# google-research/rigl

Hardware: AMD Instinct MI355X
Metric: images/sec/node, ResNet-50 80% ERK RigL step (higher is better)
Workload: dtype bf16

## Files before the change

include/rigl_hip.h:

```cpp
#ifndef RIGL_HIP_H_
#define RIGL_HIP_H_

#include <stddef.h>
#include <stdint.h>

#ifdef __cplusplus
extern "C" {
#endif

#define RIGL_ABI_VERSION 2

typedef void* rigl_stream_t;
typedef uint16_t rigl_bf16;

enum {
  RIGL_OK = 0,
  RIGL_EINVAL = -1,
  RIGL_ELAUNCH = -2,
  RIGL_EWORKSPACE = -3,
  RIGL_EUNSUPPORTED = -4
};

int rigl_version(void);
uint32_t rigl_crc32c(const void* data, size_t n, uint32_t crc);
// ... 41 lines not shown
                                         int32_t n_layers);
int rigl_prune_regrow(const RiglPruneRegrowLayer* layers ,
                      int32_t n_layers, const RiglPruneRegrowParams* params,
                      int32_t* out_counts ,
                      void* workspace , size_t workspace_bytes,
                      rigl_stream_t stream);

size_t rigl_prune_regrow_selections_workspace_bytes(int64_t n);
int rigl_prune_regrow_selections(const RiglPruneRegrowLayer* layer ,
                                 const RiglPruneRegrowParams* params,
                                 uint32_t* out_mask1_bits, uint32_t* out_mask2_bits,
                                 int32_t* out_idx1, int32_t* out_idx2,
                                 int32_t* out_counts ,
                                 void* workspace, size_t workspace_bytes,
                                 rigl_stream_t stream);

int rigl_prune_regrow_slots(const RiglPruneRegrowLayer* layers ,
                            float* const* momentum2 ,
                            int32_t n_layers, const RiglPruneRegrowParams* params,
                            int32_t* out_counts ,
                            void* workspace , size_t workspace_bytes,
                            rigl_stream_t stream);
int rigl_prune_regrow_selections_slots(const RiglPruneRegrowLayer* layer ,
                                       float* momentum2 ,
                                       const RiglPruneRegrowParams* params,
                                       uint32_t* out_mask1_bits, uint32_t* out_mask2_bits,
                                       int32_t* out_idx1, int32_t* out_idx2,
                                       int32_t* out_counts ,
                                       void* workspace, size_t workspace_bytes,
                                       rigl_stream_t stream);

int rigl_topk_mask(const float* score, int64_t n, int64_t n_keep,
                   uint32_t* mask_bits, void* workspace,
                   size_t workspace_bytes, rigl_stream_t stream);
typedef struct RiglTopkLayer {
  const float* score;
  int64_t n;
  int64_t n_keep;
  uint32_t* mask_bits;
} RiglTopkLayer;
int rigl_topk_mask_batched(const RiglTopkLayer* layers ,
                           int32_t n_layers, void* workspace,
                           size_t workspace_bytes, rigl_stream_t stream);

typedef struct RiglMagnitudePruneLayer {
  int64_t n;
  const float* w;
  uint32_t* mask_bits;
  float* threshold;
  int64_t k;
} RiglMagnitudePruneLayer;
size_t rigl_magnitude_prune_batched_workspace_bytes(int32_t n_layers);
#define RIGL_MAGPRUNE_COUNTS_PER_LAYER 4
int rigl_magnitude_prune_batched(const RiglMagnitudePruneLayer* layers ,
                                 int32_t n_layers, double threshold_decay,
                                 int32_t* out_counts, void* workspace,
                                 size_t workspace_bytes, rigl_stream_t stream);

int rigl_masked_sgd_momentum(int64_t n, float* w, float* momentum,
                             const float* dense_grad, const uint32_t* mask_bits,
                             float lr, float mu, float weight_decay,
                             float grad_scale, int32_t nesterov,
                             rigl_bf16* w_shadow, rigl_stream_t stream);

int rigl_masked_adam(int64_t n, float* w, float* m, float* v,
                     const float* dense_grad, const uint32_t* mask_bits,
                     const float* beta_powers , float lr,
                     float beta1, float beta2, float epsilon,
                     float weight_decay, float grad_scale,
                     rigl_bf16* w_shadow, rigl_stream_t stream);
int rigl_adam_advance(float* beta_powers , float beta1,
                      float beta2, rigl_stream_t stream);

#define RIGL_LR_MAX_SEGMENTS 32
#define RIGL_LR_DOMAIN_STEP 0
#define RIGL_LR_DOMAIN_EPOCH 1
#define RIGL_LR_CONST 0
#define RIGL_LR_WARMUP 1
#define RIGL_LR_COSINE 2
typedef struct RiglLrSegment {
  int32_t kind;
  int32_t start_step;
  float start;
  float c, d;
  float sum_r, len, m_fac;
} RiglLrSegment;
typedef struct RiglLrSchedule {
  int32_t n_seg;
  int32_t domain;
  float steps_per_epoch;
  int32_t reserved;
  RiglLrSegment seg[RIGL_LR_MAX_SEGMENTS];
} RiglLrSchedule;
int rigl_lr_schedule_step(const RiglLrSchedule* sched ,
                          int32_t* step ,
                          float* lr_out , rigl_stream_t stream);

int rigl_masked_sgd_momentum_dlr(int64_t n, float* w, float* momentum,
                                 const float* dense_grad,
                                 const uint32_t* mask_bits,
                                 const float* lr , float mu,
                                 float weight_decay, float grad_scale,
                                 int32_t nesterov, rigl_bf16* w_shadow,
                                 rigl_stream_t stream);
int rigl_masked_adam_dlr(int64_t n, float* w, float* m, float* v,
                         const float* dense_grad, const uint32_t* mask_bits,
                         const float* beta_powers ,
                         const float* lr , float beta1,
                         float beta2, float epsilon, float weight_decay,
                         float grad_scale, rigl_bf16* w_shadow,
                         rigl_stream_t stream);

int rigl_pack_weights(const float* w, const uint32_t* mask_bits ,
                      int32_t k, int32_t cout, rigl_bf16* hwio, rigl_bf16* ohwi,
                      rigl_stream_t stream);
typedef struct RiglPackLayer {
  const float* w;
  const uint32_t* mask_bits;
  rigl_bf16* hwio;
  rigl_bf16* ohwi;
  int32_t k, cout;
} RiglPackLayer;
int rigl_pack_weights_batched(const RiglPackLayer* layers, int32_t n_layers,
                              rigl_stream_t stream);

typedef struct RiglConvDesc {
  int32_t n, h, w, cin;
  int32_t ho, wo, cout;
  int32_t kh, kw;
  int32_t stride_h, stride_w;
  int32_t pad_top, pad_left;
} RiglConvDesc;

size_t rigl_conv2d_workspace_bytes(const RiglConvDesc* d, int32_t which );
int rigl_masked_conv2d_fwd(const RiglConvDesc* d, const rigl_bf16* x,
                           const rigl_bf16* w_ohwi, rigl_bf16* y,
                           void* workspace, size_t workspace_bytes,
                           rigl_stream_t stream);
int rigl_masked_conv2d_dgrad(const RiglConvDesc* d, const rigl_bf16* dy,
                             const rigl_bf16* w_hwio, rigl_bf16* dx,
                             void* workspace, size_t workspace_bytes,
                             rigl_stream_t stream);
int32_t rigl_conv2d_stats_parts(const RiglConvDesc* d);
int rigl_masked_conv2d_fwd_stats(const RiglConvDesc* d, const rigl_bf16* x,
                                 const rigl_bf16* w_ohwi, rigl_bf16* y,
                                 float* stats, size_t stats_floats,
                                 void* workspace, size_t workspace_bytes,
                                 rigl_stream_t stream);
int32_t rigl_conv2d_fwd_takes_bn_input(const RiglConvDesc* d);
int rigl_masked_conv2d_fwd_bnrelu(const RiglConvDesc* d, const rigl_bf16* x_pre,
                                  const float* scale_shift, rigl_bf16* a_out,
                                  const rigl_bf16* w_ohwi, rigl_bf16* y,
                                  float* stats , size_t stats_floats,
                                  void* workspace, size_t workspace_bytes,
                                  rigl_stream_t stream);
int rigl_masked_conv2d_dgrad_acc(const RiglConvDesc* d, const rigl_bf16* dy,
                                 const rigl_bf16* w_hwio, const rigl_bf16* addend,
                                 rigl_bf16* dx, void* workspace,
                                 size_t workspace_bytes, rigl_stream_t stream);
int rigl_masked_conv2d_wgrad(const RiglConvDesc* d, const rigl_bf16* x,
                             const rigl_bf16* dy, float* dw, void* workspace,
                             size_t workspace_bytes, rigl_stream_t stream);

int rigl_masked_conv2d_bwd(const RiglConvDesc* d, const rigl_bf16* x,
                           const rigl_bf16* dy, const rigl_bf16* w_hwio,
                           const rigl_bf16* addend , float* dw,
                           rigl_bf16* dx , void* workspace,
                           size_t workspace_bytes, rigl_stream_t stream);

int rigl_masked_conv2d_bwd_grid(const RiglConvDesc* d, const rigl_bf16* x,
                                const rigl_bf16* dy, const rigl_bf16* w_hwio,
                                float* dw, rigl_bf16* dx_grid, void* workspace,
                                size_t workspace_bytes, rigl_stream_t stream);
int rigl_masked_conv2d_bwd_sub(const RiglConvDesc* d, const rigl_bf16* x,
                               const rigl_bf16* dy, const rigl_bf16* w_hwio,
                               const rigl_bf16* addend, int32_t sub_h, int32_t sub_w,
                               float* dw, rigl_bf16* dx, void* workspace,
                               size_t workspace_bytes, rigl_stream_t stream);
int32_t rigl_conv2d_bwd_takes_masked_addend(const RiglConvDesc* d);
int rigl_masked_conv2d_bwd_masked(const RiglConvDesc* d, const rigl_bf16* x,
                                  const rigl_bf16* dy, const rigl_bf16* w_hwio,
                                  const rigl_bf16* addend, const uint8_t* addend_bits,
                                  float* dw, rigl_bf16* dx, void* workspace,
                                  size_t workspace_bytes, rigl_stream_t stream);

int32_t rigl_conv2d_bwd_takes_bn_apply(const RiglConvDesc* d);
int rigl_masked_conv2d_bwd_bnapply(const RiglConvDesc* d, const rigl_bf16* x,
                                   const rigl_bf16* dout, const rigl_bf16* w_hwio,
                                   const rigl_bf16* addend , float* dw,
                                   rigl_bf16* dx, void* workspace, size_t workspace_bytes,
                                   const rigl_bf16* y, const uint8_t* relu_bits,
                                   const float* mean, const float* invstd,
                                   const float* coef, rigl_stream_t stream);

typedef struct RiglBnReduceFuse {
  const rigl_bf16* x;
  const uint8_t* relu_bits;
  const float* params;
  int32_t relu;
  float* partial;
  size_t partial_floats;
} RiglBnReduceFuse;
int32_t rigl_conv2d_dgrad_stats_parts(const RiglConvDesc* d);
int rigl_masked_conv2d_bwd_bn(const RiglConvDesc* d, const rigl_bf16* x,
                              const rigl_bf16* dy, const rigl_bf16* w_hwio,
                              const rigl_bf16* addend, float* dw, rigl_bf16* dx,
                              void* workspace, size_t workspace_bytes,
                              const RiglBnReduceFuse* bn ,
                              rigl_stream_t stream);

size_t rigl_depthwise_conv2d_workspace_bytes(const RiglConvDesc* d);
int rigl_depthwise_conv2d_fwd(const RiglConvDesc* d, const rigl_bf16* x,
                              const float* w, rigl_bf16* y, rigl_stream_t stream);
int32_t rigl_depthwise_conv2d_stats_parts(const RiglConvDesc* d);
int rigl_depthwise_conv2d_fwd_stats(const RiglConvDesc* d, const rigl_bf16* x,
                                    const float* w, rigl_bf16* y, float* stats,
                                    size_t stats_floats, rigl_stream_t stream);
int rigl_depthwise_conv2d_dgrad(const RiglConvDesc* d, const rigl_bf16* dy,
                                const float* w, rigl_bf16* dx,
                                rigl_stream_t stream);
int rigl_depthwise_conv2d_wgrad(const RiglConvDesc* d, const rigl_bf16* x,
                                const rigl_bf16* dy, float* dw, void* workspace,
                                size_t workspace_bytes, rigl_stream_t stream);

int rigl_conv2d_fwd_ref(const RiglConvDesc* d, const rigl_bf16* x,
                        const rigl_bf16* w_ohwi, rigl_bf16* y,
                        rigl_stream_t stream);
int rigl_conv2d_dgrad_ref(const RiglConvDesc* d, const rigl_bf16* dy,
                          const rigl_bf16* w_hwio, rigl_bf16* dx,
                          rigl_stream_t stream);
int rigl_conv2d_wgrad_ref(const RiglConvDesc* d, const rigl_bf16* x,
                          const rigl_bf16* dy, float* dw, rigl_stream_t stream);

int rigl_masked_conv2d_fwd_f32(const RiglConvDesc* d, const float* x,
                               const float* w_hwio, const uint32_t* mask_bits ,
                               float* y, rigl_stream_t stream);
int rigl_masked_conv2d_dgrad_f32(const RiglConvDesc* d, const float* dy,
                                 const float* w_hwio, const uint32_t* mask_bits ,
                                 const float* addend ,
                                 float* dx, rigl_stream_t stream);
size_t rigl_conv2d_wgrad_f32_workspace_bytes(const RiglConvDesc* d);
int rigl_masked_conv2d_wgrad_f32(const RiglConvDesc* d, const float* x,
                                 const float* dy, float* dw, void* workspace,
                                 size_t workspace_bytes, rigl_stream_t stream);

size_t rigl_bn_workspace_bytes(int64_t m, int32_t c);
int rigl_bn_fwd(int64_t m, int32_t c, const rigl_bf16* x,
                const rigl_bf16* residual , const float* gamma,
                const float* beta, float* running_mean, float* running_var,
                float momentum, float eps, int32_t relu, rigl_bf16* y,
                float* save_mean, float* save_invstd, float* save_scale,
                float* save_shift, void* workspace, size_t workspace_bytes,
                rigl_stream_t stream);
int rigl_bn_fwd_stats(int64_t m, int32_t c, const rigl_bf16* x,
                      const rigl_bf16* residual ,
                      const float* gamma, const float* beta,
                      float* running_mean, float* running_var, float momentum,
                      float eps, int32_t relu, rigl_bf16* y, float* save_mean,
                      float* save_invstd, float* save_scale, float* save_shift,
                      const float* stats, int32_t stats_parts,
                      uint8_t* relu_bits ,
                      void* workspace, size_t workspace_bytes, rigl_stream_t stream);
int rigl_bn_bwd(int64_t m, int32_t c, const rigl_bf16* x,
                const rigl_bf16* y ,
                const uint8_t* relu_bits , const rigl_bf16* dy,
                const float* gamma, const float* save_mean,
                const float* save_invstd, const float* save_scale,
                const float* save_shift, int32_t relu, rigl_bf16* dx,
                rigl_bf16* dresidual , float* dgamma,
                float* dbeta, void* workspace, size_t workspace_bytes,
                rigl_stream_t stream);
int rigl_bn_bwd_reduce(int64_t m, int32_t c, const rigl_bf16* x,
                       const uint8_t* relu_bits ,
                       const rigl_bf16* dy, const float* gamma, const float* save_mean,
                       const float* save_invstd, int32_t relu, float* dgamma,
                       float* dbeta, float* coef, void* workspace,
                       size_t workspace_bytes, rigl_stream_t stream);
int rigl_bn_bwd_stats(int64_t m, int32_t c, const rigl_bf16* x,
                      const rigl_bf16* y ,
                      const uint8_t* relu_bits , const rigl_bf16* dy,
                      const float* gamma, const float* save_mean,
                      const float* save_invstd, const float* save_scale,
                      const float* save_shift, int32_t relu, rigl_bf16* dx,
                      rigl_bf16* dresidual , float* dgamma,
                      float* dbeta, const float* stats, int32_t stats_parts,
                      void* workspace, size_t workspace_bytes, rigl_stream_t stream);

int rigl_bn_add_bn_fwd(int64_t m, int32_t c, const rigl_bf16* x, const rigl_bf16* x2,
                       const float* scale2, const float* shift2,
                       const float* gamma, const float* beta, float* running_mean,
                       float* running_var, float momentum, float eps, int32_t relu,
                       rigl_bf16* y, float* save_mean, float* save_invstd,
                       float* save_scale, float* save_shift, const float* stats,
                       int32_t stats_parts, uint8_t* relu_bits ,
                       void* workspace, size_t workspace_bytes, rigl_stream_t stream);
size_t rigl_bn_add_bn_bwd_workspace_bytes(int64_t m, int32_t c);
int rigl_bn_add_bn_bwd(int64_t m, int32_t c, const rigl_bf16* x, const rigl_bf16* x2,
                       const uint8_t* relu_bits, const rigl_bf16* dy,
                       const float* gamma, const float* save_mean, const float* save_invstd,
                       const float* gamma2, const float* save_mean2, const float* save_invstd2,
                       rigl_bf16* dx, rigl_bf16* dx2, float* dgamma, float* dbeta,
                       float* dgamma2, float* dbeta2, void* workspace,
                       size_t workspace_bytes, rigl_stream_t stream);

int rigl_stateless_random(float* out, int64_t n, int32_t seed0, int32_t seed1,
                          int32_t dist, float scale, float shift,
                          rigl_stream_t stream);
typedef struct {
  float* out;
  int64_t n;
  int32_t seed0, seed1;
  int32_t dist;
  float scale, shift;
} RiglRandomItem;
int rigl_stateless_random_batched(const RiglRandomItem* items, int32_t n_items,
                                  rigl_stream_t stream);

int rigl_dropout_fwd(const void* x, void* y, uint8_t* keep_bits, int64_t n,
                     int32_t dtype, float rate, int32_t seed0,
                     const int32_t* step , rigl_stream_t stream);
int rigl_dropout_bwd(const void* dy, const uint8_t* keep_bits, void* dx,
                     int64_t n, int32_t dtype, float rate, rigl_stream_t stream);
int rigl_dropout_advance(int32_t* step , rigl_stream_t stream);

int rigl_cifar_batch(const uint8_t* images, const int32_t* labels,
                     int64_t n_images, int32_t batch, int32_t mode,
                     int32_t shard, int32_t n_shards, int32_t seed0,
                     const int32_t* step , void* out, int32_t dtype,
                     int32_t* out_labels, int32_t* out_index ,
                     rigl_stream_t stream);
int rigl_cifar_advance(int32_t* step , rigl_stream_t stream);

int rigl_maxpool_fwd(const RiglConvDesc* d, const rigl_bf16* x, rigl_bf16* y,
                     uint8_t* argmax, rigl_stream_t stream);
int rigl_maxpool_bwd(const RiglConvDesc* d, const rigl_bf16* dy,
                     const uint8_t* argmax, rigl_bf16* dx, rigl_stream_t stream);
int rigl_bn_fwd_statistics(int64_t m, int32_t c, const rigl_bf16* x ,
                           const float* gamma, const float* beta,
                           float* running_mean, float* running_var, float momentum,
                           float eps, float* save_mean, float* save_invstd,
                           float* save_scale, float* save_shift,
                           const float* stats, int32_t stats_parts,
                           void* workspace, size_t workspace_bytes, rigl_stream_t stream);
int rigl_bn_relu_maxpool_fwd(const RiglConvDesc* d, const rigl_bf16* x,
                             const float* scale, const float* shift, rigl_bf16* y,
                             uint8_t* argmax, rigl_stream_t stream);
size_t rigl_bn_relu_maxpool_bwd_workspace_bytes(const RiglConvDesc* d);
int rigl_bn_relu_maxpool_bwd(const RiglConvDesc* d, const rigl_bf16* x,
                             const rigl_bf16* dy, const uint8_t* argmax,
                             const float* gamma, const float* save_mean,
                             const float* save_invstd, const float* save_scale,
                             const float* save_shift, rigl_bf16* dx, float* dgamma,
                             float* dbeta, void* workspace, size_t workspace_bytes,
                             rigl_stream_t stream);

int rigl_global_avgpool_fwd(int32_t n, int32_t pixels, int32_t c, const rigl_bf16* x,
                            rigl_bf16* y, rigl_stream_t stream);
int rigl_global_avgpool_bwd(int32_t n, int32_t pixels, int32_t c, const rigl_bf16* dy,
                            rigl_bf16* dx, rigl_stream_t stream);
int rigl_global_avgpool_bwd_relu(int32_t n, int32_t pixels, int32_t c, const rigl_bf16* dy,
                                 const rigl_bf16* x, rigl_bf16* dx, rigl_stream_t stream);
int rigl_softmax_xent(int32_t rows, int32_t classes, const rigl_bf16* logits,
                      const int64_t* labels, float label_smoothing, float grad_scale,
                      float* row_loss, rigl_bf16* dlogits , rigl_stream_t stream);

int32_t rigl_conv2d_fwd_takes_relu_epilogue(const RiglConvDesc* d);
int32_t rigl_conv2d_bwd_takes_relu_epilogue(const RiglConvDesc* d);
int rigl_masked_conv2d_fwd_relu(const RiglConvDesc* d, const rigl_bf16* x,
                                const rigl_bf16* w_ohwi, rigl_bf16* y, void* workspace,
                                size_t workspace_bytes, rigl_stream_t stream);
int rigl_masked_conv2d_bwd_relu(const RiglConvDesc* d, const rigl_bf16* x,
                                const rigl_bf16* dy, const rigl_bf16* w_hwio, float* dw,
                                rigl_bf16* dx, void* workspace, size_t workspace_bytes,
                                rigl_stream_t stream);
int rigl_relu_fwd(int64_t n, const rigl_bf16* x, rigl_bf16* y, rigl_stream_t stream);
int rigl_relu_bwd(int64_t n, const rigl_bf16* dy, const rigl_bf16* x, rigl_bf16* dx,
                  rigl_stream_t stream);

typedef struct RiglBnInferItem {
  const float* gamma;
  const float* beta;
  const float* moving_mean;
  const float* moving_variance;
  float* scale_shift;
  int32_t c;
  float eps;
} RiglBnInferItem;
int rigl_bn_infer_params_batched(const RiglBnInferItem* items, int32_t n_items,
                                 rigl_stream_t stream);
int rigl_bn_apply(int64_t m, int32_t c, const rigl_bf16* x,
                  const rigl_bf16* residual , const float* scale_shift,
                  int32_t relu, rigl_bf16* y, rigl_stream_t stream);
int rigl_bn_apply_pair(int64_t m, int32_t c, const rigl_bf16* x, const rigl_bf16* x2,
                       const float* scale_shift, const float* scale_shift2,
                       int32_t relu, rigl_bf16* y, rigl_stream_t stream);
int rigl_bn_relu_maxpool_infer(const RiglConvDesc* d, const rigl_bf16* x,
                               const float* scale_shift, rigl_bf16* y,
                               rigl_stream_t stream);
int32_t rigl_conv2d_fwd_takes_bn_epilogue(const RiglConvDesc* d, int32_t bn_on_load,
                                          int32_t residual);
int rigl_masked_conv2d_fwd_bn_infer(const RiglConvDesc* d, const rigl_bf16* x,
                                    const float* in_scale_shift ,
                                    const rigl_bf16* w_ohwi,
                                    const float* scale_shift ,
                                    const rigl_bf16* residual ,
                                    int32_t relu, rigl_bf16* y, rigl_stream_t stream);
int rigl_eval_metrics(int32_t rows, int32_t classes, const rigl_bf16* logits,
                      const int64_t* labels, float label_smoothing, int32_t topk,
                      float* row_loss, int32_t* row_flags,
                      int64_t* counts , rigl_stream_t stream);

#define RIGL_PROF_KINDS 8
int rigl_prof_enable(int32_t on);
int rigl_prof_collect(double* ms_per_kind , int64_t* launches );
#define RIGL_PROF_KINDS_ALL 10
int rigl_prof_collect_kinds(double* ms_per_kind, int64_t* launches, int32_t n_kinds);
typedef struct RiglProfLaunch {
  int32_t kind;
  int32_t tag[6];
  float ms;
} RiglProfLaunch;
int rigl_prof_collect_launches(RiglProfLaunch* out , int64_t cap, int64_t* n_launches);

int rigl_probe_mfma_bf16(int32_t blocks, int32_t iters, float* sink, rigl_stream_t stream);

int rigl_tune_set(const char* key, int32_t value);
int32_t rigl_tune_get(const char* key, int32_t dflt);
int rigl_tune_unset(const char* key);
uint64_t rigl_tune_generation(void);
const volatile uint64_t* rigl_tune_generation_addr(void);

#ifdef __cplusplus
}
#endif
#endif
```

rigl_amd/_lib.py:

```python
import ctypes as C
import os

_HERE = os.path.dirname(os.path.abspath(__file__))
ABI_VERSION = 2
LIB_PATH = os.environ.get('RIGL_HIP_LIB') or os.path.join(_HERE, 'lib', 'librigl_hip.so')

RIGL_OK = 0
RIGL_EINVAL = -1
RIGL_ELAUNCH = -2
RIGL_EWORKSPACE = -3
RIGL_EUNSUPPORTED = -4
COUNTS_PER_LAYER = 8
MAGPRUNE_COUNTS_PER_LAYER = 4
PROF_KINDS = ('conv_fwd', 'conv_dgrad', 'conv_wgrad', 'prune_regrow',
              'sgd_momentum', 'pack_weights', 'conv_bwd', 'depthwise', 'masked_adam', 'magnitude_prune')

GROW_ZEROS, GROW_GRAD_SCALE, GROW_GRAD_SIGN, GROW_EXPLICIT = 0, 1, 2, 3
MOMRESET_ZEROS, MOMRESET_GRAD = 0, 1


class RiglError(RuntimeError):

  def __init__(self, code, msg):
    super().__init__('librigl_hip: error %d: %s' % (code, msg))
    self.code = code


class PruneRegrowLayer(C.Structure):
  _fields_ = [('n', C.c_int64), ('w', C.c_void_p), ('momentum', C.c_void_p),
              ('mask_bits', C.c_void_p), ('dense_grad', C.c_void_p),
              ('drop_noise', C.c_void_p), ('score_drop', C.c_void_p),
              ('score_grow', C.c_void_p), ('grow_values', C.c_void_p)]


class PruneRegrowParams(C.Structure):
  _fields_ = [('drop_fraction', C.c_float), ('grow_init_mode', C.c_int32),
              ('grow_init_div', C.c_float), ('momentum_reset_mode', C.c_int32),
              ('initial_acc_scale', C.c_float), ('reinit_when_same', C.c_int32)]


class TopkLayer(C.Structure):
  _fields_ = [('score', C.c_void_p), ('n', C.c_int64), ('n_keep', C.c_int64),
              ('mask_bits', C.c_void_p)]


class MagnitudePruneLayer(C.Structure):
  _fields_ = [('n', C.c_int64), ('w', C.c_void_p), ('mask_bits', C.c_void_p), ('threshold', C.c_void_p),
              ('k', C.c_int64)]


class PackLayer(C.Structure):
  _fields_ = [('w', C.c_void_p), ('mask_bits', C.c_void_p),
              ('hwio', C.c_void_p), ('ohwi', C.c_void_p), ('k', C.c_int32),
              ('cout', C.c_int32)]


class ConvDesc(C.Structure):
  _fields_ = [('n', C.c_int32), ('h', C.c_int32), ('w', C.c_int32),
              ('cin', C.c_int32), ('ho', C.c_int32), ('wo', C.c_int32),
              ('cout', C.c_int32), ('kh', C.c_int32), ('kw', C.c_int32),
              ('stride_h', C.c_int32), ('stride_w', C.c_int32),
              ('pad_top', C.c_int32), ('pad_left', C.c_int32)]


class BnReduceFuse(C.Structure):
  _fields_ = [('x', C.c_void_p), ('relu_bits', C.c_void_p), ('params', C.c_void_p), ('relu', C.c_int32),
              ('partial', C.c_void_p), ('partial_floats', C.c_size_t)]


class RandomItem(C.Structure):
  _fields_ = [('out', C.c_void_p), ('n', C.c_int64), ('seed0', C.c_int32), ('seed1', C.c_int32),
              ('dist', C.c_int32), ('scale', C.c_float), ('shift', C.c_float)]


class BnInferItem(C.Structure):
  _fields_ = [('gamma', C.c_void_p), ('beta', C.c_void_p), ('moving_mean', C.c_void_p), ('moving_variance', C.c_void_p),
              ('scale_shift', C.c_void_p), ('c', C.c_int32), ('eps', C.c_float)]


LR_MAX_SEGMENTS = 32
LR_DOMAIN_STEP, LR_DOMAIN_EPOCH = 0, 1
LR_CONST, LR_WARMUP, LR_COSINE = 0, 1, 2


class LrSegment(C.Structure):
  _fields_ = [('kind', C.c_int32), ('start_step', C.c_int32), ('start', C.c_float), ('c', C.c_float), ('d', C.c_float),
              ('sum_r', C.c_float), ('len', C.c_float), ('m_fac', C.c_float)]


class LrSchedule(C.Structure):
  _fields_ = [('n_seg', C.c_int32), ('domain', C.c_int32), ('steps_per_epoch', C.c_float), ('reserved', C.c_int32),
              ('seg', LrSegment * LR_MAX_SEGMENTS)]


class ProfLaunch(C.Structure):
  _fields_ = [('kind', C.c_int32), ('tag', C.c_int32 * 6), ('ms', C.c_float)]


_P, _I32, _I64, _F, _SZ = C.c_void_p, C.c_int32, C.c_int64, C.c_float, C.c_size_t
SIGNATURES = {
    'rigl_version': (C.c_int, []),
    'rigl_last_error': (C.c_char_p, []),
    'rigl_mask_pack': (C.c_int, [_P, _P, _I64, _P]),
    'rigl_mask_unpack': (C.c_int, [_P, _P, _I64, _P]),
    'rigl_prune_regrow_workspace_bytes': (_SZ, [C.POINTER(_I64), _I32]),
    'rigl_prune_regrow': (C.c_int, [C.POINTER(PruneRegrowLayer), _I32,
                                    C.POINTER(PruneRegrowParams), _P, _P, _SZ,
                                    _P]),
    'rigl_prune_regrow_slots': (C.c_int, [C.POINTER(PruneRegrowLayer), C.POINTER(_P), _I32,
                                          C.POINTER(PruneRegrowParams), _P, _P, _SZ, _P]),
    'rigl_prune_regrow_selections_workspace_bytes': (_SZ, [_I64]),
    'rigl_prune_regrow_selections': (C.c_int, [C.POINTER(PruneRegrowLayer), C.POINTER(PruneRegrowParams), _P, _P, _P, _P, _P,
                                               _P, _SZ, _P]),
    'rigl_prune_regrow_selections_slots': (C.c_int, [C.POINTER(PruneRegrowLayer), _P, C.POINTER(PruneRegrowParams), _P, _P,
                                                     _P, _P, _P, _P, _SZ, _P]),
    'rigl_topk_mask': (C.c_int, [_P, _I64, _I64, _P, _P, _SZ, _P]),
    'rigl_topk_mask_batched': (C.c_int, [C.POINTER(TopkLayer), _I32, _P, _SZ, _P]),
    'rigl_magnitude_prune_batched_workspace_bytes': (_SZ, [_I32]),
    'rigl_magnitude_prune_batched': (C.c_int, [C.POINTER(MagnitudePruneLayer), _I32, C.c_double, _P, _P, _SZ, _P]),
    'rigl_masked_sgd_momentum': (C.c_int, [_I64, _P, _P, _P, _P, _F, _F, _F, _F,
                                           _I32, _P, _P]),
    'rigl_masked_adam': (C.c_int, [_I64, _P, _P, _P, _P, _P, _P, _F, _F, _F, _F, _F, _F, _P, _P]),
    'rigl_adam_advance': (C.c_int, [_P, _F, _F, _P]),
    'rigl_lr_schedule_step': (C.c_int, [C.POINTER(LrSchedule), _P, _P, _P]),
    'rigl_masked_sgd_momentum_dlr': (C.c_int, [_I64, _P, _P, _P, _P, _P, _F, _F, _F, _I32, _P, _P]),
    'rigl_masked_adam_dlr': (C.c_int, [_I64, _P, _P, _P, _P, _P, _P, _P, _F, _F, _F, _F, _F, _P, _P]),
    'rigl_pack_weights': (C.c_int, [_P, _P, _I32, _I32, _P, _P, _P]),
    'rigl_pack_weights_batched': (C.c_int, [C.POINTER(PackLayer), _I32, _P]),
    'rigl_conv2d_workspace_bytes': (_SZ, [C.POINTER(ConvDesc), _I32]),
    'rigl_masked_conv2d_fwd': (C.c_int, [C.POINTER(ConvDesc), _P, _P, _P, _P,
                                         _SZ, _P]),
    'rigl_masked_conv2d_dgrad': (C.c_int, [C.POINTER(ConvDesc), _P, _P, _P, _P,
                                           _SZ, _P]),
    'rigl_conv2d_stats_parts': (_I32, [C.POINTER(ConvDesc)]),
    'rigl_masked_conv2d_fwd_stats': (C.c_int, [C.POINTER(ConvDesc), _P, _P, _P, _P,
                                               _SZ, _P, _SZ, _P]),
    'rigl_conv2d_fwd_takes_bn_input': (_I32, [C.POINTER(ConvDesc)]),
    'rigl_masked_conv2d_fwd_bnrelu': (C.c_int, [C.POINTER(ConvDesc), _P, _P, _P, _P, _P, _P, _SZ, _P, _SZ, _P]),
    'rigl_masked_conv2d_dgrad_acc': (C.c_int, [C.POINTER(ConvDesc), _P, _P, _P,
                                               _P, _P, _SZ, _P]),
    'rigl_conv2d_dgrad_stats_parts': (_I32, [C.POINTER(ConvDesc)]),
    'rigl_masked_conv2d_bwd_bn': (C.c_int, [C.POINTER(ConvDesc), _P, _P, _P, _P, _P, _P, _P, _SZ,
                                            C.POINTER(BnReduceFuse), _P]),
    'rigl_masked_conv2d_bwd': (C.c_int, [C.POINTER(ConvDesc), _P, _P, _P, _P, _P, _P, _P, _SZ, _P]),
    'rigl_masked_conv2d_bwd_masked': (C.c_int, [C.POINTER(ConvDesc), _P, _P, _P, _P, _P, _P, _P, _P, _SZ, _P]),
    'rigl_conv2d_bwd_takes_masked_addend': (_I32, [C.POINTER(ConvDesc)]),
    'rigl_conv2d_bwd_takes_bn_apply': (_I32, [C.POINTER(ConvDesc)]),
    'rigl_masked_conv2d_bwd_bnapply': (C.c_int, [C.POINTER(ConvDesc), _P, _P, _P, _P, _P, _P, _P, _SZ, _P, _P, _P, _P, _P, _P]),
    'rigl_masked_conv2d_bwd_grid': (C.c_int, [C.POINTER(ConvDesc), _P, _P, _P, _P, _P, _P, _SZ, _P]),
    'rigl_masked_conv2d_bwd_sub': (C.c_int, [C.POINTER(ConvDesc), _P, _P, _P, _P, _I32, _I32, _P, _P, _P, _SZ, _P]),
    'rigl_masked_conv2d_wgrad': (C.c_int, [C.POINTER(ConvDesc), _P, _P, _P, _P,
                                           _SZ, _P]),
    'rigl_conv2d_fwd_ref': (C.c_int, [C.POINTER(ConvDesc), _P, _P, _P, _P]),
    'rigl_conv2d_dgrad_ref': (C.c_int, [C.POINTER(ConvDesc), _P, _P, _P, _P]),
    'rigl_conv2d_wgrad_ref': (C.c_int, [C.POINTER(ConvDesc), _P, _P, _P, _P]),
    'rigl_masked_conv2d_fwd_f32': (C.c_int, [C.POINTER(ConvDesc), _P, _P, _P, _P, _P]),
    'rigl_masked_conv2d_dgrad_f32': (C.c_int, [C.POINTER(ConvDesc), _P, _P, _P, _P, _P, _P]),
    'rigl_conv2d_wgrad_f32_workspace_bytes': (_SZ, [C.POINTER(ConvDesc)]),
    'rigl_masked_conv2d_wgrad_f32': (C.c_int, [C.POINTER(ConvDesc), _P, _P, _P, _P, _SZ, _P]),
    'rigl_depthwise_conv2d_workspace_bytes': (_SZ, [C.POINTER(ConvDesc)]),
    'rigl_depthwise_conv2d_fwd': (C.c_int, [C.POINTER(ConvDesc), _P, _P, _P, _P]),
    'rigl_depthwise_conv2d_stats_parts': (_I32, [C.POINTER(ConvDesc)]),
    'rigl_depthwise_conv2d_fwd_stats': (C.c_int, [C.POINTER(ConvDesc), _P, _P, _P, _P, _SZ, _P]),
    'rigl_depthwise_conv2d_dgrad': (C.c_int, [C.POINTER(ConvDesc), _P, _P, _P, _P]),
    'rigl_depthwise_conv2d_wgrad': (C.c_int, [C.POINTER(ConvDesc), _P, _P, _P, _P, _SZ, _P]),
    'rigl_bn_workspace_bytes': (_SZ, [_I64, _I32]),
    'rigl_bn_fwd': (C.c_int, [_I64, _I32, _P, _P, _P, _P, _P, _P, _F, _F, _I32, _P, _P, _P, _P, _P, _P, _SZ, _P]),
    'rigl_bn_fwd_stats': (C.c_int, [_I64, _I32, _P, _P, _P, _P, _P, _P, _F, _F, _I32, _P, _P, _P, _P, _P, _P, _I32, _P, _P, _SZ, _P]),
    'rigl_bn_bwd': (C.c_int, [_I64, _I32, _P, _P, _P, _P, _P, _P, _P, _P, _P, _I32, _P, _P, _P, _P, _P, _SZ, _P]),
    'rigl_bn_bwd_stats': (C.c_int, [_I64, _I32, _P, _P, _P, _P, _P, _P, _P, _P, _P, _I32, _P, _P, _P, _P, _P, _I32, _P, _SZ, _P]),
    'rigl_bn_bwd_reduce': (C.c_int, [_I64, _I32, _P, _P, _P, _P, _P, _P, _I32, _P, _P, _P, _P, _SZ, _P]),
    'rigl_crc32c': (C.c_uint32, [_P, _SZ, C.c_uint32]),
    'rigl_stateless_random': (C.c_int, [_P, _I64, _I32, _I32, _I32, _F, _F, _P]),
    'rigl_stateless_random_batched': (C.c_int, [C.POINTER(RandomItem), _I32, _P]),
    'rigl_dropout_fwd': (C.c_int, [_P, _P, _P, _I64, _I32, _F, _I32, _P, _P]),
    'rigl_dropout_bwd': (C.c_int, [_P, _P, _P, _I64, _I32, _F, _P]),
    'rigl_dropout_advance': (C.c_int, [_P, _P]),
    'rigl_cifar_batch': (C.c_int, [_P, _P, _I64, _I32, _I32, _I32, _I32, _I32, _P, _P, _I32, _P, _P, _P]),
    'rigl_cifar_advance': (C.c_int, [_P, _P]),
    'rigl_maxpool_fwd': (C.c_int, [C.POINTER(ConvDesc), _P, _P, _P, _P]),
    'rigl_maxpool_bwd': (C.c_int, [C.POINTER(ConvDesc), _P, _P, _P, _P]),
    'rigl_bn_fwd_statistics': (C.c_int, [_I64, _I32, _P, _P, _P, _P, _P, _F, _F, _P, _P, _P, _P, _P, _I32, _P, _SZ, _P]),
    'rigl_bn_add_bn_fwd': (C.c_int, [_I64, _I32, _P, _P, _P, _P, _P, _P, _P, _P, _F, _F, _I32, _P, _P, _P, _P, _P, _P, _I32, _P, _P, _SZ, _P]),
    'rigl_bn_add_bn_bwd_workspace_bytes': (_SZ, [_I64, _I32]),
    'rigl_bn_add_bn_bwd': (C.c_int, [_I64, _I32, _P, _P, _P, _P, _P, _P, _P, _P, _P, _P, _P, _P, _P, _P, _P, _P, _P, _SZ, _P]),
    'rigl_bn_relu_maxpool_fwd': (C.c_int, [C.POINTER(ConvDesc), _P, _P, _P, _P, _P, _P]),
    'rigl_bn_relu_maxpool_bwd_workspace_bytes': (_SZ, [C.POINTER(ConvDesc)]),
    'rigl_bn_relu_maxpool_bwd': (C.c_int, [C.POINTER(ConvDesc), _P, _P, _P, _P, _P, _P, _P, _P, _P, _P, _P, _P, _SZ, _P]),
    'rigl_global_avgpool_fwd': (C.c_int, [_I32, _I32, _I32, _P, _P, _P]),
    'rigl_global_avgpool_bwd': (C.c_int, [_I32, _I32, _I32, _P, _P, _P]),
    'rigl_softmax_xent': (C.c_int, [_I32, _I32, _P, _P, _F, _F, _P, _P, _P]),
    'rigl_global_avgpool_bwd_relu': (C.c_int, [_I32, _I32, _I32, _P, _P, _P, _P]),
    'rigl_conv2d_fwd_takes_relu_epilogue': (C.c_int32, [C.POINTER(ConvDesc)]),
    'rigl_conv2d_bwd_takes_relu_epilogue': (C.c_int32, [C.POINTER(ConvDesc)]),
    'rigl_masked_conv2d_fwd_relu': (C.c_int, [C.POINTER(ConvDesc), _P, _P, _P, _P, _SZ, _P]),
    'rigl_masked_conv2d_bwd_relu': (C.c_int, [C.POINTER(ConvDesc), _P, _P, _P, _P, _P, _P, _SZ, _P]),
    'rigl_relu_fwd': (C.c_int, [_I64, _P, _P, _P]),
    'rigl_relu_bwd': (C.c_int, [_I64, _P, _P, _P, _P]),
    'rigl_bn_infer_params_batched': (C.c_int, [C.POINTER(BnInferItem), _I32, _P]),
    'rigl_bn_apply': (C.c_int, [_I64, _I32, _P, _P, _P, _I32, _P, _P]),
    'rigl_bn_apply_pair': (C.c_int, [_I64, _I32, _P, _P, _P, _P, _I32, _P, _P]),
    'rigl_bn_relu_maxpool_infer': (C.c_int, [C.POINTER(ConvDesc), _P, _P, _P, _P]),
    'rigl_conv2d_fwd_takes_bn_epilogue': (C.c_int32, [C.POINTER(ConvDesc), _I32, _I32]),
    'rigl_masked_conv2d_fwd_bn_infer': (C.c_int, [C.POINTER(ConvDesc), _P, _P, _P, _P, _P, _I32, _P, _P]),
    'rigl_eval_metrics': (C.c_int, [_I32, _I32, _P, _P, _F, _I32, _P, _P, _P, _P]),
    'rigl_prof_enable': (C.c_int, [_I32]),
    'rigl_prof_collect': (C.c_int, [C.POINTER(C.c_double), C.POINTER(_I64)]),
    'rigl_prof_collect_kinds': (C.c_int, [C.POINTER(C.c_double), C.POINTER(_I64), _I32]),
    'rigl_prof_collect_launches': (C.c_int, [C.POINTER(ProfLaunch), _I64, C.POINTER(_I64)]),
    'rigl_probe_mfma_bf16': (C.c_int, [_I32, _I32, _P, _P]),
    'rigl_tune_set': (C.c_int, [C.c_char_p, _I32]),
    'rigl_tune_get': (_I32, [C.c_char_p, _I32]),
    'rigl_tune_generation': (C.c_uint64, []),
    'rigl_tune_generation_addr': (C.c_void_p, []),
    'rigl_tune_unset': (C.c_int, [C.c_char_p]),
}

_lib = None


def load():
  global _lib
  if _lib is not None:
    return _lib
  if not os.path.exists(LIB_PATH):
    raise RiglError(
        RIGL_ELAUNCH, 'HIP extension not built: %s is missing; run '
        '`python -c "import __graft_entry__ as g; g.build()"` or '
        '`make -C rigl_amd/csrc`' % LIB_PATH)
  try:
    import torch
  except ImportError:
    pass
  lib = C.CDLL(LIB_PATH, mode=C.RTLD_GLOBAL)
  for name, (res, args) in SIGNATURES.items():
    fn = getattr(lib, name)
    fn.restype = res
    fn.argtypes = args
  if lib.rigl_version() != ABI_VERSION:
    raise RiglError(RIGL_EINVAL, 'ABI version mismatch')
  _lib = lib
  return lib


def check(rc):
  if rc != RIGL_OK:
    raise RiglError(rc, load().rigl_last_error().decode('utf-8', 'replace'))
```

rigl_amd/csrc/bn.hip:

```cpp
#include "common.hpp"

namespace rigl {
namespace kbn {

constexpr int THREADS = 256;
constexpr int MAX_PARTS = 512;

__device__ __forceinline__ float bf_lo(uint32_t w) { return __uint_as_float(w << 16); }
__device__ __forceinline__ float bf_hi(uint32_t w) { return __uint_as_float(w & 0xFFFF0000u); }
__device__ __forceinline__ uint32_t f2bf(float f) {
  uint32_t u = __float_as_uint(f);
  if ((u & 0x7FFFFFFFu) > 0x7F800000u) return (u >> 16) | 0x40u;
  u += 0x7FFFu + ((u >> 16) & 1u);
  return u >> 16;
}
typedef __attribute__((ext_vector_type(2))) __bf16 bf16x2_t;
typedef __attribute__((ext_vector_type(2))) float f32x2_t;
__device__ __forceinline__ uint32_t pack2(float a, float b) {
  const f32x2_t v = {a, b};
  return __builtin_bit_cast(uint32_t, __builtin_convertvector(v, bf16x2_t));
}
__device__ __forceinline__ void unpack8(const uint4& v, float f[8]) {
  f[0] = bf_lo(v.x); f[1] = bf_hi(v.x); f[2] = bf_lo(v.y); f[3] = bf_hi(v.y);
  f[4] = bf_lo(v.z); f[5] = bf_hi(v.z); f[6] = bf_lo(v.w); f[7] = bf_hi(v.w);
// ... 393 lines not shown
      float xv[8], x2v[8], dv[8];
      unpack8(*reinterpret_cast<const uint4*>(x + off), xv);
      unpack8(*reinterpret_cast<const uint4*>(x2 + off), x2v);
      unpack8(*reinterpret_cast<const uint4*>(dy + off), dv);
      const uint32_t mb = mbits[r * G.cg + cgi];
#pragma unroll
      for (int j = 0; j < 8; ++j) {
        const float dz = ((mb >> j) & 1u) != 0u ? dv[j] : 0.f;
        q0[j] += dz;
        q1[j] = fmaf(dz, (xv[j] - mu[j]) * is[j], q1[j]);
        q2[j] = fmaf(dz, (x2v[j] - mu2[j]) * is2[j], q2[j]);
      }
    }
  }
  float own[24];
#pragma unroll
  for (int j = 0; j < 8; ++j) {
    own[j] = q0[j]; own[8 + j] = q1[j]; own[16 + j] = q2[j];
    red[threadIdx.x][j] = q0[j]; red[threadIdx.x][8 + j] = q1[j]; red[threadIdx.x][16 + j] = q2[j];
  }
  __syncthreads();
  for (int s = G.rpb >> 1; s > 0; s >>= 1) {
    if (ty < s) {
      float oth[24];
#pragma unroll
      for (int j = 0; j < 24; ++j) oth[j] = red[threadIdx.x + s * G.tpr][j];
#pragma unroll
      for (int j = 0; j < 24; ++j) own[j] += oth[j];
      if (s > 1) {
#pragma unroll
        for (int j = 0; j < 24; ++j) red[threadIdx.x][j] = own[j];
      }
    }
    if (s > 1) __syncthreads();
  }
  if (ty == 0 && c_ok) {
    float* p = partial + ((int64_t)blockIdx.x * 2) * G.C + cgi * 8;
    float* p2 = partial2 + ((int64_t)blockIdx.x * 2) * G.C + cgi * 8;
#pragma unroll
    for (int j = 0; j < 8; ++j) {
      p[j] = own[j]; p[G.C + j] = own[8 + j];
      p2[j] = own[j]; p2[G.C + j] = own[16 + j];
    }
  }
}

struct FinSet { const float* partial; const float* gamma; const float* invstd; float* dgamma; float* dbeta; float* coef; };

template <int CL>
__global__ __launch_bounds__(THREADS) void k_bwd_finalize_pair(Geom G, FinSet s0, FinSet s1) {
  const FinSet& f = blockIdx.y == 0 ? s0 : s1;
  double a0, a1; int c; bool leader;
  sum_partials<CL>(G, f.partial, a0, a1, c, leader);
  if (!leader) return;
  f.dbeta[c] = (float)a0;
  f.dgamma[c] = (float)a1;
  f.coef[c] = f.gamma[c] * f.invstd[c];
  f.coef[G.C + c] = (float)(a0 / (double)G.M);
  f.coef[2 * G.C + c] = (float)(a1 / (double)G.M);
}

__global__ __launch_bounds__(THREADS) void k_bwd_apply_pair(Geom G, const uint16_t* __restrict__ x, const uint16_t* __restrict__ x2,
                                                             const uint8_t* __restrict__ mbits, const uint16_t* __restrict__ dy,
                                                             const float* __restrict__ mean, const float* __restrict__ invstd,
                                                             const float* __restrict__ mean2, const float* __restrict__ invstd2,
                                                             const float* __restrict__ coef, const float* __restrict__ coef2,
                                                             uint16_t* __restrict__ dx, uint16_t* __restrict__ dx2) {
  extern __shared__ __attribute__((aligned(16))) float prm[];
  const bool fixed = G.fixed != 0;
  float q[10][8];
  if (fixed) {
    const int c0 = (int)(((int64_t)blockIdx.x * THREADS + threadIdx.x) % G.cg) * 8;
    ld8f(mean + c0, q[0]); ld8f(invstd + c0, q[1]); ld8f(coef + c0, q[2]); ld8f(coef + G.C + c0, q[3]); ld8f(coef + 2 * G.C + c0, q[4]);
    ld8f(mean2 + c0, q[5]); ld8f(invstd2 + c0, q[6]); ld8f(coef2 + c0, q[7]); ld8f(coef2 + G.C + c0, q[8]); ld8f(coef2 + 2 * G.C + c0, q[9]);
  } else {
    for (int i = threadIdx.x; i < G.C; i += THREADS) {
      prm[i] = mean[i]; prm[G.C + i] = invstd[i];
      prm[2 * G.C + i] = coef[i]; prm[3 * G.C + i] = coef[G.C + i]; prm[4 * G.C + i] = coef[2 * G.C + i];
      prm[5 * G.C + i] = mean2[i]; prm[6 * G.C + i] = invstd2[i];
      prm[7 * G.C + i] = coef2[i]; prm[8 * G.C + i] = coef2[G.C + i]; prm[9 * G.C + i] = coef2[2 * G.C + i];
    }
    __syncthreads();
  }
  const int64_t total = G.M * G.cg;
  const int64_t stride = (int64_t)gridDim.x * THREADS;
  for (int64_t i = (int64_t)blockIdx.x * THREADS + threadIdx.x; i < total; i += stride) {
    if (!fixed) {
      const int c0 = (int)(i % G.cg) * 8;
#pragma unroll
      for (int k = 0; k < 10; ++k)
#pragma unroll
        for (int j = 0; j < 8; ++j) q[k][j] = prm[k * G.C + c0 + j];
    }
    float xv[8], x2v[8], dv[8];
    unpack8(ld16(x + i * 8, G.nt), xv);
    unpack8(ld16(x2 + i * 8, G.nt), x2v);
    unpack8(ld16(dy + i * 8, G.nt), dv);
    const uint32_t mb = mbits[i];
    float o[8], o2[8];
#pragma unroll
    for (int j = 0; j < 8; ++j) {
      const float dz = ((mb >> j) & 1u) != 0u ? dv[j] : 0.f;
      const float xh = (xv[j] - q[0][j]) * q[1][j];
      o[j] = q[2][j] * (dz - q[3][j] - xh * q[4][j]);
      const float xh2 = (x2v[j] - q[5][j]) * q[6][j];
      o2[j] = q[7][j] * (dz - q[8][j] - xh2 * q[9][j]);
    }
    uint4 out;
    out.x = pack2(o[0], o[1]); out.y = pack2(o[2], o[3]); out.z = pack2(o[4], o[5]); out.w = pack2(o[6], o[7]);
    st16(dx + i * 8, out, G.nt);
    out.x = pack2(o2[0], o2[1]); out.y = pack2(o2[2], o2[3]); out.z = pack2(o2[4], o2[5]); out.w = pack2(o2[6], o2[7]);
    st16(dx2 + i * 8, out, G.nt);
  }
}

constexpr int INFER_BATCH = 64;
struct InferBatch {
  RiglBnInferItem it[INFER_BATCH];
  int32_t blk_begin[INFER_BATCH + 1];
  int32_t count;
};
__global__ __launch_bounds__(THREADS) void k_infer_params(InferBatch B) {
  int i = 0;
  while (i + 1 < B.count && (int)blockIdx.x >= B.blk_begin[i + 1]) ++i;
  const RiglBnInferItem& t = B.it[i];
  const int c = ((int)blockIdx.x - B.blk_begin[i]) * THREADS + (int)threadIdx.x;
  if (c >= t.c) return;
  const float invstd = (float)(1.0 / sqrt((double)t.moving_variance[c] + (double)t.eps));
  const float sc = t.gamma[c] * invstd;
  t.scale_shift[c] = sc;
  t.scale_shift[t.c + c] = t.beta[c] - t.moving_mean[c] * sc;
}

static Geom make_geom(int64_t m, int c) {
  Geom g;
  g.nt = (int64_t)m * c * 2 >= (int64_t)RIGL_TUNE("bn_nt_mb", 0) * (1 << 20) ? RIGL_TUNE("bn_nt", 2) : 0;
  g.il = RIGL_TUNE("bn_il", 1);
  g.fixed = 0;
  g.M = m; g.C = c; g.cg = c / 8;
  int tpr = 1;
  while (tpr < g.cg && tpr < THREADS) tpr <<= 1;
  g.tpr = tpr; g.rpb = THREADS / tpr;
#ifndef RIGL_BN_ROWS_PER_LANE
#define RIGL_BN_ROWS_PER_LANE 8
#endif
  int64_t parts = (m + (int64_t)g.rpb * RIGL_BN_ROWS_PER_LANE - 1) / ((int64_t)g.rpb * RIGL_BN_ROWS_PER_LANE);
  const int64_t cap = RIGL_TUNE("bn_max_parts", MAX_PARTS);
  if (parts > cap) parts = cap;
  if (parts < 1) parts = 1;
  int64_t rpp = (m + parts - 1) / parts;
  rpp = (rpp + g.rpb - 1) / g.rpb * g.rpb;
  g.rows_per_part = rpp;
  g.parts = (int)((m + rpp - 1) / rpp);
  return g;
}

static unsigned apply_grid(Geom& g) {
#ifndef RIGL_BN_APPLY_PER_THREAD
#define RIGL_BN_APPLY_PER_THREAD 2
#endif
#ifndef RIGL_BN_APPLY_CAP
#define RIGL_BN_APPLY_CAP 16384
#endif
  int64_t b = (g.M * g.cg + THREADS * RIGL_BN_APPLY_PER_THREAD - 1) / (THREADS * RIGL_BN_APPLY_PER_THREAD);
  if (b > RIGL_BN_APPLY_CAP) b = RIGL_BN_APPLY_CAP;
  if (b < 1) b = 1;
  g.fixed = (RIGL_TUNE("bn_regs", 1) != 0 && (b * THREADS) % g.cg == 0) ? 1 : 0;
  return (unsigned)b;
}

void launch_bwd_finalize(int64_t m, int c, const float* partial, int parts, const float* gamma, const float* invstd,
                         float* dgamma, float* dbeta, float* coef, hipStream_t st) {
  Geom g = make_geom(m, c);
  g.parts = parts;
  if (parts > MAX_PARTS)
    hipLaunchKernelGGL(k_bwd_finalize<4>, dim3((unsigned)((c + 3) / 4)), dim3(THREADS), 0, st, g, partial, gamma, invstd,
                       dgamma, dbeta, coef);
  else
    hipLaunchKernelGGL(k_bwd_finalize<16>, dim3((unsigned)((c + 15) / 16)), dim3(THREADS), 0, st, g, partial, gamma, invstd,
                       dgamma, dbeta, coef);
}

static int fwd_statistics(Geom& g, int32_t c, const rigl_bf16* x, const float* gamma, const float* beta,
                          float* running_mean, float* running_var, float momentum, float eps, float* save_mean,
                          float* save_invstd, float* save_scale, float* save_shift, const float* stats,
                          int32_t stats_parts, void* workspace, size_t workspace_bytes, hipStream_t st) {
  const float* partial = stats;
  if (!stats) {
    const size_t need = rigl_bn_workspace_bytes(g.M, c);
    if (!workspace || workspace_bytes < need) return fail(RIGL_EWORKSPACE, "rigl_bn_fwd: workspace %zu < %zu", workspace_bytes, need);
    float* ws_partial = static_cast<float*>(workspace);
    dim3 rgrid((unsigned)g.parts, (unsigned)((g.cg + g.tpr - 1) / g.tpr));
    hipLaunchKernelGGL((k_reduce<0, false, 0>), rgrid, dim3(THREADS), 0, st, g, x, nullptr, nullptr, nullptr, nullptr, nullptr,
                       nullptr, nullptr, ws_partial);
    partial = ws_partial;
  } else {
    g.parts = stats_parts;
  }
  if (g.parts > 1024 && RIGL_TUNE("bn_fin1", 1) != 0)
    hipLaunchKernelGGL(k_fwd_finalize<1>, dim3((unsigned)c), dim3(THREADS), 0, st, g, partial, stats ? nullptr : reinterpret_cast<const uint16_t*>(x), gamma,
                       beta, running_mean, running_var, momentum, eps, save_mean, save_invstd, save_scale, save_shift);
  else if (g.parts > 256)
    hipLaunchKernelGGL(k_fwd_finalize<4>, dim3((unsigned)((c + 3) / 4)), dim3(THREADS), 0, st, g, partial, stats ? nullptr : reinterpret_cast<const uint16_t*>(x), gamma,
                       beta, running_mean, running_var, momentum, eps, save_mean, save_invstd, save_scale, save_shift);
  else
    hipLaunchKernelGGL(k_fwd_finalize<16>, dim3((unsigned)((c + 15) / 16)), dim3(THREADS), 0, st, g, partial, stats ? nullptr : reinterpret_cast<const uint16_t*>(x), gamma,
                       beta, running_mean, running_var, momentum, eps, save_mean, save_invstd, save_scale, save_shift);
  return RIGL_OK;
}

}
}

extern "C" {

size_t rigl_bn_workspace_bytes(int64_t m, int32_t c) {
  if (m <= 0 || c <= 0) return 0;
  rigl::kbn::Geom g = rigl::kbn::make_geom(m, c);
  return rigl::align_up((size_t)g.parts * 2 * c * 4, 256) + rigl::align_up((size_t)3 * c * 4, 256);
}

int rigl_bn_fwd_stats(int64_t m, int32_t c, const rigl_bf16* x, const rigl_bf16* residual, const float* gamma,
                      const float* beta, float* running_mean, float* running_var, float momentum, float eps,
                      int32_t relu, rigl_bf16* y, float* save_mean, float* save_invstd, float* save_scale,
                      float* save_shift, const float* stats, int32_t stats_parts, uint8_t* relu_bits,
                      void* workspace, size_t workspace_bytes, rigl_stream_t stream) {
  using namespace rigl;
  using namespace rigl::kbn;
  if (m <= 0 || c <= 0 || !x || !gamma || !beta || !y || !save_mean || !save_invstd || !save_scale || !save_shift)
    return fail(RIGL_EINVAL, "rigl_bn_fwd: bad arguments");
  if (c % 8) return fail(RIGL_EUNSUPPORTED, "rigl_bn_fwd: channels %% 8 != 0");
  if (2 * (size_t)c * 4 > 65536) return fail(RIGL_EUNSUPPORTED, "rigl_bn_fwd: too many channels for the LDS parameter cache");
  if (stats && stats_parts <= 0) return fail(RIGL_EINVAL, "rigl_bn_fwd_stats: stats_parts must be positive");
  hipStream_t st = as_stream(stream);
  Geom g = make_geom(m, c);
  int rc = fwd_statistics(g, c, x, gamma, beta, running_mean, running_var, momentum, eps, save_mean, save_invstd,
                          save_scale, save_shift, stats, stats_parts, workspace, workspace_bytes, st);
  if (rc) return rc;
  dim3 agrid(apply_grid(g));
  const size_t lds = g.fixed ? 0 : (size_t)2 * c * 4;
  if (relu && residual) hipLaunchKernelGGL((k_fwd_apply<true, true>), agrid, dim3(THREADS), lds, st, g, x, residual, save_scale, save_shift, y, relu_bits);
  else if (relu) hipLaunchKernelGGL((k_fwd_apply<true, false>), agrid, dim3(THREADS), lds, st, g, x, residual, save_scale, save_shift, y, relu_bits);
  else if (residual) hipLaunchKernelGGL((k_fwd_apply<false, true>), agrid, dim3(THREADS), lds, st, g, x, residual, save_scale, save_shift, y, nullptr);
  else hipLaunchKernelGGL((k_fwd_apply<false, false>), agrid, dim3(THREADS), lds, st, g, x, residual, save_scale, save_shift, y, nullptr);
  RIGL_CHECK_LAUNCH("rigl_bn_fwd");
  return RIGL_OK;
}

int rigl_bn_fwd(int64_t m, int32_t c, const rigl_bf16* x, const rigl_bf16* residual, const float* gamma,
                const float* beta, float* running_mean, float* running_var, float momentum, float eps, int32_t relu,
                rigl_bf16* y, float* save_mean, float* save_invstd, float* save_scale, float* save_shift,
                void* workspace, size_t workspace_bytes, rigl_stream_t stream) {
  return rigl_bn_fwd_stats(m, c, x, residual, gamma, beta, running_mean, running_var, momentum, eps, relu, y, save_mean,
                           save_invstd, save_scale, save_shift, nullptr, 0, nullptr, workspace, workspace_bytes, stream);
}

int rigl_bn_fwd_statistics(int64_t m, int32_t c, const rigl_bf16* x, const float* gamma, const float* beta,
                           float* running_mean, float* running_var, float momentum, float eps, float* save_mean,
                           float* save_invstd, float* save_scale, float* save_shift, const float* stats,
                           int32_t stats_parts, void* workspace, size_t workspace_bytes, rigl_stream_t stream) {
  using namespace rigl;
  using namespace rigl::kbn;
  if (m <= 0 || c <= 0 || (!x && !stats) || !gamma || !beta || !save_mean || !save_invstd || !save_scale || !save_shift)
    return fail(RIGL_EINVAL, "rigl_bn_fwd_statistics: bad arguments");
  if (c % 8) return fail(RIGL_EUNSUPPORTED, "rigl_bn_fwd_statistics: channels %% 8 != 0");
  if (stats && stats_parts <= 0) return fail(RIGL_EINVAL, "rigl_bn_fwd_statistics: stats_parts must be positive");
  Geom g = make_geom(m, c);
  int rc = fwd_statistics(g, c, x, gamma, beta, running_mean, running_var, momentum, eps, save_mean, save_invstd,
                          save_scale, save_shift, stats, stats_parts, workspace, workspace_bytes, as_stream(stream));
  if (rc) return rc;
  RIGL_CHECK_LAUNCH("rigl_bn_fwd_statistics");
  return RIGL_OK;
}

int rigl_bn_add_bn_fwd(int64_t m, int32_t c, const rigl_bf16* x, const rigl_bf16* x2, const float* scale2,
                       const float* shift2, const float* gamma, const float* beta, float* running_mean,
                       float* running_var, float momentum, float eps, int32_t relu, rigl_bf16* y, float* save_mean,
                       float* save_invstd, float* save_scale, float* save_shift, const float* stats,
                       int32_t stats_parts, uint8_t* relu_bits, void* workspace, size_t workspace_bytes,
                       rigl_stream_t stream) {
  using namespace rigl;
  using namespace rigl::kbn;
  if (m <= 0 || c <= 0 || !x || !x2 || !scale2 || !shift2 || !gamma || !beta || !y || !save_mean || !save_invstd ||
      !save_scale || !save_shift)
    return fail(RIGL_EINVAL, "rigl_bn_add_bn_fwd: bad arguments");
  if (c % 8) return fail(RIGL_EUNSUPPORTED, "rigl_bn_add_bn_fwd: channels %% 8 != 0");
  if (4 * (size_t)c * 4 > 65536) return fail(RIGL_EUNSUPPORTED, "rigl_bn_add_bn_fwd: too many channels for the LDS parameter cache");
  if (stats && stats_parts <= 0) return fail(RIGL_EINVAL, "rigl_bn_add_bn_fwd: stats_parts must be positive");
  hipStream_t st = as_stream(stream);
  Geom g = make_geom(m, c);
  int rc = fwd_statistics(g, c, x, gamma, beta, running_mean, running_var, momentum, eps, save_mean, save_invstd,
                          save_scale, save_shift, stats, stats_parts, workspace, workspace_bytes, st);
  if (rc) return rc;
  dim3 agrid(apply_grid(g));
  const size_t lds = g.fixed ? 0 : (size_t)4 * c * 4;
  if (relu) hipLaunchKernelGGL(k_fwd_apply_pair<true>, agrid, dim3(THREADS), lds, st, g, x, x2, save_scale, save_shift, scale2, shift2, y, relu_bits);
  else hipLaunchKernelGGL(k_fwd_apply_pair<false>, agrid, dim3(THREADS), lds, st, g, x, x2, save_scale, save_shift, scale2, shift2, y, nullptr);
  RIGL_CHECK_LAUNCH("rigl_bn_add_bn_fwd");
  return RIGL_OK;
}

size_t rigl_bn_add_bn_bwd_workspace_bytes(int64_t m, int32_t c) { return 2 * rigl_bn_workspace_bytes(m, c); }

int rigl_bn_add_bn_bwd(int64_t m, int32_t c, const rigl_bf16* x, const rigl_bf16* x2, const uint8_t* relu_bits,
                       const rigl_bf16* dy, const float* gamma, const float* save_mean, const float* save_invstd,
                       const float* gamma2, const float* save_mean2, const float* save_invstd2, rigl_bf16* dx,
                       rigl_bf16* dx2, float* dgamma, float* dbeta, float* dgamma2, float* dbeta2, void* workspace,
                       size_t workspace_bytes, rigl_stream_t stream) {
  using namespace rigl;
  using namespace rigl::kbn;
  if (m <= 0 || c <= 0 || !x || !x2 || !relu_bits || !dy || !gamma || !save_mean || !save_invstd || !gamma2 || !save_mean2 ||
      !save_invstd2 || !dx || !dx2 || !dgamma || !dbeta || !dgamma2 || !dbeta2)
    return fail(RIGL_EINVAL, "rigl_bn_add_bn_bwd: bad arguments");
  if (c % 8) return fail(RIGL_EUNSUPPORTED, "rigl_bn_add_bn_bwd: channels %% 8 != 0");
  const size_t lds = (size_t)10 * c * 4;
  if (lds > 160 * 1024 - 1024) return fail(RIGL_EUNSUPPORTED, "rigl_bn_add_bn_bwd: too many channels for the LDS parameter cache");
  const size_t need = rigl_bn_add_bn_bwd_workspace_bytes(m, c);
  if (!workspace || workspace_bytes < need) return fail(RIGL_EWORKSPACE, "rigl_bn_add_bn_bwd: workspace %zu < %zu", workspace_bytes, need);
  static const bool big_lds = hipFuncSetAttribute(reinterpret_cast<const void*>(&k_bwd_apply_pair),
                                                  hipFuncAttributeMaxDynamicSharedMemorySize, 159 * 1024) == hipSuccess;
  if (lds > 65536 && !big_lds) return fail(RIGL_ELAUNCH, "rigl_bn_add_bn_bwd: cannot raise the dynamic LDS limit");
  hipStream_t st = as_stream(stream);
  Geom g = make_geom(m, c);
  const size_t half = rigl_bn_workspace_bytes(m, c);
  const size_t part_bytes = align_up((size_t)g.parts * 2 * c * 4, 256);
  char* w0 = static_cast<char*>(workspace);
  float* partial = reinterpret_cast<float*>(w0);
  float* coef = reinterpret_cast<float*>(w0 + part_bytes);
  float* partial2 = reinterpret_cast<float*>(w0 + half);
  float* coef2 = reinterpret_cast<float*>(w0 + half + part_bytes);
  dim3 rgrid((unsigned)g.parts, (unsigned)((g.cg + g.tpr - 1) / g.tpr));
  hipLaunchKernelGGL(k_reduce_pair, rgrid, dim3(THREADS), 0, st, g, x, x2, relu_bits, dy, save_mean, save_invstd, save_mean2,
                     save_invstd2, partial, partial2);
  const FinSet f0 = {partial, gamma, save_invstd, dgamma, dbeta, coef};
  const FinSet f1 = {partial2, gamma2, save_invstd2, dgamma2, dbeta2, coef2};
  hipLaunchKernelGGL(k_bwd_finalize_pair<16>, dim3((unsigned)((c + 15) / 16), 2), dim3(THREADS), 0, st, g, f0, f1);
  const dim3 pgrid(apply_grid(g));
  hipLaunchKernelGGL(k_bwd_apply_pair, pgrid, dim3(THREADS), g.fixed ? 0 : lds, st, g, x, x2, relu_bits, dy, save_mean, save_invstd,
                     save_mean2, save_invstd2, coef, coef2, dx, dx2);
  RIGL_CHECK_LAUNCH("rigl_bn_add_bn_bwd");
  return RIGL_OK;
}

static int bn_bwd_impl(int64_t m, int32_t c, const rigl_bf16* x, const rigl_bf16* y, const uint8_t* relu_bits,
                       const rigl_bf16* dy, const float* gamma,
                       const float* save_mean, const float* save_invstd, const float* save_scale, const float* save_shift,
                       int32_t relu, rigl_bf16* dx, rigl_bf16* dresidual, float* dgamma, float* dbeta,
                       const float* stats, int32_t stats_parts, float* coef_out, void* workspace,
                       size_t workspace_bytes, rigl_stream_t stream) {
  using namespace rigl;
  using namespace rigl::kbn;
  if (m <= 0 || c <= 0 || !x || !dy || !gamma || !save_mean || !save_invstd || (!dx && !coef_out) || !dgamma || !dbeta)
    return fail(RIGL_EINVAL, "rigl_bn_bwd: bad arguments");
  if (c % 8) return fail(RIGL_EUNSUPPORTED, "rigl_bn_bwd: channels %% 8 != 0");
  if (relu && !y && !relu_bits && (!save_scale || !save_shift))
    return fail(RIGL_EINVAL, "rigl_bn_bwd: relu needs y, relu_bits or scale/shift");
  if (7 * (size_t)c * 4 > 65536) return fail(RIGL_EUNSUPPORTED, "rigl_bn_bwd: too many channels for the LDS parameter cache");
  if (stats && stats_parts <= 0) return fail(RIGL_EINVAL, "rigl_bn_bwd_stats: stats_parts must be positive");
  const size_t need = rigl_bn_workspace_bytes(m, c);
  if (!workspace || workspace_bytes < need) return fail(RIGL_EWORKSPACE, "rigl_bn_bwd: workspace %zu < %zu", workspace_bytes, need);
  hipStream_t st = as_stream(stream);
  Geom g = make_geom(m, c);
  float* partial = static_cast<float*>(workspace);
  float* coef = coef_out ? coef_out : reinterpret_cast<float*>(static_cast<char*>(workspace) + align_up((size_t)g.parts * 2 * c * 4, 256));
  dim3 rgrid((unsigned)g.parts, (unsigned)((g.cg + g.tpr - 1) / g.tpr));
  const int msk = relu_bits ? 2 : (y ? 1 : 0);
  const float* red = partial;
  if (stats) {
    red = stats;
    g.parts = stats_parts;
  } else {
#define RIGL_BWD_REDUCE(R, K) hipLaunchKernelGGL((k_reduce<1, R, K>), rgrid, dim3(THREADS), 0, st, g, x, y, relu_bits, dy, save_mean, save_invstd, save_scale, save_shift, partial)
    if (!relu) RIGL_BWD_REDUCE(false, 0);
    else if (msk == 2) RIGL_BWD_REDUCE(true, 2);
    else if (msk == 1) RIGL_BWD_REDUCE(true, 1);
    else RIGL_BWD_REDUCE(true, 0);
#undef RIGL_BWD_REDUCE
  }
  if (g.parts > MAX_PARTS)
    hipLaunchKernelGGL(k_bwd_finalize<4>, dim3((unsigned)((c + 3) / 4)), dim3(THREADS), 0, st, g, red, gamma,
                       save_invstd, dgamma, dbeta, coef);
  else
    hipLaunchKernelGGL(k_bwd_finalize<16>, dim3((unsigned)((c + 15) / 16)), dim3(THREADS), 0, st, g, red, gamma,
                       save_invstd, dgamma, dbeta, coef);
  if (coef_out) {
    RIGL_CHECK_LAUNCH("rigl_bn_bwd_reduce");
    return RIGL_OK;
  }
  dim3 agrid(apply_grid(g));
  const size_t lds = g.fixed ? 0 : (size_t)7 * c * 4;
#define RIGL_BWD_APPLY(R, K, D) hipLaunchKernelGGL((k_bwd_apply<R, K, D>), agrid, dim3(THREADS), lds, st, g, x, y, relu_bits, dy, save_mean, save_invstd, save_scale, save_shift, coef, dx, dresidual)
  const bool dres = dresidual != nullptr;
  if (!relu) { if (dres) RIGL_BWD_APPLY(false, 0, true); else RIGL_BWD_APPLY(false, 0, false); }
  else if (msk == 2) { if (dres) RIGL_BWD_APPLY(true, 2, true); else RIGL_BWD_APPLY(true, 2, false); }
  else if (msk == 1) { if (dres) RIGL_BWD_APPLY(true, 1, true); else RIGL_BWD_APPLY(true, 1, false); }
  else { if (dres) RIGL_BWD_APPLY(true, 0, true); else RIGL_BWD_APPLY(true, 0, false); }
#undef RIGL_BWD_APPLY
  RIGL_CHECK_LAUNCH("rigl_bn_bwd");
  return RIGL_OK;
}

int rigl_bn_bwd_stats(int64_t m, int32_t c, const rigl_bf16* x, const rigl_bf16* y, const uint8_t* relu_bits,
                      const rigl_bf16* dy, const float* gamma,
                      const float* save_mean, const float* save_invstd, const float* save_scale, const float* save_shift,
                      int32_t relu, rigl_bf16* dx, rigl_bf16* dresidual, float* dgamma, float* dbeta,
                      const float* stats, int32_t stats_parts, void* workspace,
                      size_t workspace_bytes, rigl_stream_t stream) {
  return bn_bwd_impl(m, c, x, y, relu_bits, dy, gamma, save_mean, save_invstd, save_scale, save_shift, relu, dx, dresidual, dgamma,
                     dbeta, stats, stats_parts, nullptr, workspace, workspace_bytes, stream);
}

int rigl_bn_bwd_reduce(int64_t m, int32_t c, const rigl_bf16* x, const uint8_t* relu_bits, const rigl_bf16* dy, const float* gamma,
                       const float* save_mean, const float* save_invstd, int32_t relu, float* dgamma, float* dbeta, float* coef,
                       void* workspace, size_t workspace_bytes, rigl_stream_t stream) {
  if (!coef) return rigl::fail(RIGL_EINVAL, "rigl_bn_bwd_reduce: coef is required");
  if (relu && !relu_bits) return rigl::fail(RIGL_EINVAL, "rigl_bn_bwd_reduce: relu needs relu_bits");
  return bn_bwd_impl(m, c, x, nullptr, relu ? relu_bits : nullptr, dy, gamma, save_mean, save_invstd, nullptr, nullptr, relu, nullptr,
                     nullptr, dgamma, dbeta, nullptr, 0, coef, workspace, workspace_bytes, stream);
}

int rigl_bn_bwd(int64_t m, int32_t c, const rigl_bf16* x, const rigl_bf16* y, const uint8_t* relu_bits,
                const rigl_bf16* dy, const float* gamma,
                const float* save_mean, const float* save_invstd, const float* save_scale, const float* save_shift,
                int32_t relu, rigl_bf16* dx, rigl_bf16* dresidual, float* dgamma, float* dbeta, void* workspace,
                size_t workspace_bytes, rigl_stream_t stream) {
  return rigl_bn_bwd_stats(m, c, x, y, relu_bits, dy, gamma, save_mean, save_invstd, save_scale, save_shift, relu, dx,
                           dresidual, dgamma, dbeta, nullptr, 0, workspace, workspace_bytes, stream);
}

int rigl_bn_infer_params_batched(const RiglBnInferItem* items, int32_t n_items, rigl_stream_t stream) {
  using namespace rigl;
  using namespace rigl::kbn;
  if (n_items < 0 || (n_items > 0 && !items)) return fail(RIGL_EINVAL, "rigl_bn_infer_params_batched: bad arguments");
  for (int i = 0; i < n_items; ++i) {
    const RiglBnInferItem& t = items[i];
    if (t.c < 0 || (t.c > 0 && (!t.gamma || !t.beta || !t.moving_mean || !t.moving_variance || !t.scale_shift)))
      return fail(RIGL_EINVAL, "rigl_bn_infer_params_batched: item %d: bad channels / NULL tensor", i);
  }
  hipStream_t st = as_stream(stream);
  for (int b = 0; b < n_items; b += INFER_BATCH) {
    InferBatch B;
    B.count = 0;
    int32_t blk = 0;
    for (int i = b; i < n_items && i < b + INFER_BATCH; ++i) {
      if (items[i].c == 0) continue;
      B.it[B.count] = items[i];
      B.blk_begin[B.count] = blk;
      blk += (items[i].c + THREADS - 1) / THREADS;
      ++B.count;
    }
    B.blk_begin[B.count] = blk;
    if (B.count) hipLaunchKernelGGL(k_infer_params, dim3((unsigned)blk), dim3(THREADS), 0, st, B);
  }
  RIGL_CHECK_LAUNCH("rigl_bn_infer_params_batched");
  return RIGL_OK;
}

int rigl_bn_apply(int64_t m, int32_t c, const rigl_bf16* x, const rigl_bf16* residual, const float* scale_shift, int32_t relu,
                  rigl_bf16* y, rigl_stream_t stream) {
  using namespace rigl;
  using namespace rigl::kbn;
  if (m <= 0 || c <= 0 || !x || !scale_shift || !y) return fail(RIGL_EINVAL, "rigl_bn_apply: bad arguments");
  if (c % 8) return fail(RIGL_EUNSUPPORTED, "rigl_bn_apply: channels %% 8 != 0");
  if (2 * (size_t)c * 4 > 65536) return fail(RIGL_EUNSUPPORTED, "rigl_bn_apply: too many channels for the LDS parameter cache");
  hipStream_t st = as_stream(stream);
  Geom g = make_geom(m, c);
  dim3 agrid(apply_grid(g));
  const size_t lds = g.fixed ? 0 : (size_t)2 * c * 4;
  const float* sc = scale_shift;
  const float* sh = scale_shift + c;
  if (relu && residual) hipLaunchKernelGGL((k_fwd_apply<true, true>), agrid, dim3(THREADS), lds, st, g, x, residual, sc, sh, y, nullptr);
  else if (relu) hipLaunchKernelGGL((k_fwd_apply<true, false>), agrid, dim3(THREADS), lds, st, g, x, residual, sc, sh, y, nullptr);
  else if (residual) hipLaunchKernelGGL((k_fwd_apply<false, true>), agrid, dim3(THREADS), lds, st, g, x, residual, sc, sh, y, nullptr);
  else hipLaunchKernelGGL((k_fwd_apply<false, false>), agrid, dim3(THREADS), lds, st, g, x, residual, sc, sh, y, nullptr);
  RIGL_CHECK_LAUNCH("rigl_bn_apply");
  return RIGL_OK;
}

int rigl_bn_apply_pair(int64_t m, int32_t c, const rigl_bf16* x, const rigl_bf16* x2, const float* scale_shift,
                       const float* scale_shift2, int32_t relu, rigl_bf16* y, rigl_stream_t stream) {
  using namespace rigl;
  using namespace rigl::kbn;
  if (m <= 0 || c <= 0 || !x || !x2 || !scale_shift || !scale_shift2 || !y) return fail(RIGL_EINVAL, "rigl_bn_apply_pair: bad arguments");
  if (c % 8) return fail(RIGL_EUNSUPPORTED, "rigl_bn_apply_pair: channels %% 8 != 0");
  if (4 * (size_t)c * 4 > 65536) return fail(RIGL_EUNSUPPORTED, "rigl_bn_apply_pair: too many channels for the LDS parameter cache");
  hipStream_t st = as_stream(stream);
  Geom g = make_geom(m, c);
  dim3 agrid(apply_grid(g));
  const size_t lds = g.fixed ? 0 : (size_t)4 * c * 4;
  if (relu) hipLaunchKernelGGL(k_fwd_apply_pair<true>, agrid, dim3(THREADS), lds, st, g, x, x2, scale_shift, scale_shift + c, scale_shift2, scale_shift2 + c, y, nullptr);
  else hipLaunchKernelGGL(k_fwd_apply_pair<false>, agrid, dim3(THREADS), lds, st, g, x, x2, scale_shift, scale_shift + c, scale_shift2, scale_shift2 + c, y, nullptr);
  RIGL_CHECK_LAUNCH("rigl_bn_apply_pair");
  return RIGL_OK;
}

}
```

rigl_amd/csrc/bwd1x1.hpp:

```cpp
#pragma once

struct Bwd1x1Args {
  const uint16_t* X;
  const uint16_t* DY;
  const uint16_t* W;
  const uint16_t* ADD;
  uint16_t* DX;
  float* SLAB;
  int M, splits, interleave;
  uint32_t x_bytes, dy_bytes;
  const uint16_t* Y3;
  const uint8_t* BITS;
  const float* MEAN;
  const float* INVSTD;
  const float* COEF;
};

template <int ROWB>
__device__ __forceinline__ int dual_swz(int row) {
  if (ROWB == 512) return ((row & 1) << 1) | (((row >> 1) & 1) << 2) | (((row ^ (row >> 2)) & 1) << 3);
  return (((row >> 1) & 1) << 1) | ((((row >> 1) ^ (row >> 2)) & 1) << 2);
}

typedef __attribute__((ext_vector_type(4))) float f32x4;

template <int CI, int CO, bool DO_W, int NST, bool BNA = false>
struct Bwd1x1Smem {
  static constexpr int BYTES = NST * (32 * ((DO_W ? CI : 0) + CO) * 2 + (BNA ? 32 * CO * 2 + 32 * (CO / 8) : 0)) + (CI <= 64 ? 2 : 1) * 32 * (CI * 2 + 16);
};
template <int CI, int CO, bool DO_W, int NST, bool BNA = false>
__global__ __launch_bounds__(THREADS) void k_bwd1x1(Bwd1x1Args P) {
  constexpr int PX = 32;
  constexpr int YROWB = CO * 2, XROWB = CI * 2;
  constexpr int Y_BYTES = PX * YROWB, X_BYTES = DO_W ? PX * XROWB : 0;
  constexpr int B_BYTES = BNA ? PX * (CO / 8) : 0;
  constexpr int Y3_OFF = Y_BYTES + X_BYTES, B_OFF = Y3_OFF + (BNA ? Y_BYTES : 0), STAGE = B_OFF + B_BYTES;
  static_assert(!BNA || (YROWB == 512 && B_BYTES == 4 * 256), "BNA: 256 output channels (a lane's pieces share one channel chunk)");
  constexpr int YI = YROWB / 32, XI = XROWB / 32;
  constexpr int YPW = YI / 4 > 0 ? YI / 4 : 1, XPW = XI / 4 > 0 ? XI / 4 : 1;
  static_assert(YI % 4 == 0 && XI % 4 == 0, "tiles are whole rounds of four waves");
  constexpr int L = YPW + (DO_W ? XPW : 0) + (BNA ? YPW + 1 : 0);
  constexpr int CF = CI / 16, CFW = CF / 2;
  constexpr int KSD = CO / 32;
  constexpr int NFI = CI / 32, NFO = CO / 32;
  constexpr bool WIDE_O = NFO >= NFI;
  constexpr int WF = NFI * NFO / 4 > 0 ? NFI * NFO / 4 : 1;
  static_assert(CFW * KSD * 4 <= 96, "W fragments stay in registers");
  constexpr bool DXDB = CI <= 64;
  constexpr int NDX = DXDB ? 2 : 1;
  constexpr int DXROWB = XROWB + 16, DX_BYTES = PX * DXROWB;
  static_assert(NST * STAGE + NDX * DX_BYTES == Bwd1x1Smem<CI, CO, DO_W, NST, BNA>::BYTES, "host and device agree on the LDS size");
  extern __shared__ __attribute__((aligned(1024))) unsigned char smem[];
  unsigned char* const dxs = smem + NST * STAGE;

  const int tid = threadIdx.x, lane = tid & 63;
  const int wave = __builtin_amdgcn_readfirstlane(tid >> 6);
  const int split = blockIdx.x;
  const int KT_all = (P.M + PX - 1) / PX;
  const int kt_begin = P.interleave ? split : (int)((int64_t)KT_all * split / P.splits);
  const int kt_step = P.interleave ? P.splits : 1;
  const int KT = P.interleave ? (split < KT_all ? (KT_all - split + P.splits - 1) / P.splits : 0)
                              : (int)((int64_t)KT_all * (split + 1) / P.splits) - kt_begin;
  const __amdgpu_buffer_rsrc_t rsrcY = make_rsrc(P.DY, P.dy_bytes), rsrcX = make_rsrc(P.X, P.x_bytes);
  const u32x4 rsrcY4 = make_rsrc4(P.DY, P.dy_bytes), rsrcX4 = make_rsrc4(P.X, P.x_bytes);
  (void)rsrcY4; (void)rsrcX4; (void)rsrcY; (void)rsrcX;
  const u32x4 rsrcZ4 = make_rsrc4(BNA ? P.Y3 : P.DY, BNA ? P.dy_bytes : 0u);
  const u32x4 rsrcB4 = make_rsrc4(BNA ? (const void*)P.BITS : (const void*)P.DY, BNA ? P.dy_bytes >> 4 : 0u);
  (void)rsrcZ4; (void)rsrcB4;

  int y_row[YPW], y_col[YPW], x_row[XPW], x_col[XPW];
#pragma unroll
  for (int q = 0; q < YPW; ++q) {
    const int i = q * 4 + wave, row = i * (1024 / YROWB) + lane / (YROWB / 16), slot = lane % (YROWB / 16);
    y_row[q] = row; y_col[q] = (slot ^ dual_swz<YROWB>(row)) * 8;
  }
#pragma unroll
  for (int q = 0; q < XPW; ++q) {
    const int i = q * 4 + wave, row = i * (1024 / XROWB) + lane / (XROWB / 16), slot = lane % (XROWB / 16);
    x_row[q] = row; x_col[q] = (slot ^ dual_swz<XROWB>(row)) * 8;
  }
  const int b_row = (((lane >> 4) * 4 + wave) << 1) | ((lane >> 3) & 1), b_col = (lane & 7) * 4;
  float pm[8], pis[8], pa[8], pb[8], pc[8];
  (void)pm; (void)pis; (void)pa; (void)pb; (void)pc; (void)b_row; (void)b_col;
  if constexpr (BNA) {
    const int c0 = y_col[0];
#pragma unroll
    for (int j = 0; j < 8; ++j) {
      pm[j] = P.MEAN[c0 + j]; pis[j] = P.INVSTD[c0 + j];
      pa[j] = P.COEF[c0 + j]; pb[j] = P.COEF[CO + c0 + j]; pc[j] = P.COEF[2 * CO + c0 + j];
    }
  }
#if !defined(RIGL_B1_NO_NT) && !defined(RIGL_DMA_BUILTIN)
#define B1_DMA16(r_, lds_, off_) lds_dma16_nt(r_##4, lds_, off_)
#else
#define B1_DMA16(r_, lds_, off_) RIGL_DMA16(r_, lds_, off_)
#endif
#define B1_ISSUE(kt_, stage_)                                                                            \
  {                                                                                                      \
    const int p0_ = (kt_begin + (kt_) * kt_step) * PX;                                                             \
    _Pragma("unroll") for (int q = 0; q < YPW; ++q) {                                                    \
      const int p_ = p0_ + y_row[q];                                                                     \
      const int off_ = p_ < P.M ? (int)((uint32_t)(p_ * CO + y_col[q]) * 2u) : (int)OOB;                 \
      B1_DMA16(rsrcY, smem + (stage_) * STAGE + (q * 4 + wave) * 1024, off_); \
      if (BNA) lds_dma16_nt(rsrcZ4, smem + (stage_) * STAGE + Y3_OFF + (q * 4 + wave) * 1024, off_);       \
    }                                                                                                    \
    if (BNA) {                                                                                           \
      const int p_ = p0_ + b_row;                                                                        \
      lds_dma4(rsrcB4, smem + (stage_) * STAGE + B_OFF + wave * 256, p_ < P.M ? p_ * (CO / 8) + b_col : (int)OOB); \
    }                                                                                                    \
    if (DO_W) {                                                                                          \
      _Pragma("unroll") for (int q = 0; q < XPW; ++q) {                                                  \
        const int p_ = p0_ + x_row[q];                                                                   \
        const int off_ = p_ < P.M ? (int)((uint32_t)(p_ * CI + x_col[q]) * 2u) : (int)OOB;               \
        B1_DMA16(rsrcX, smem + (stage_) * STAGE + Y_BYTES + (q * 4 + wave) * 1024, off_); \
      }                                                                                                  \
    }                                                                                                    \
  }

  const int pf = wave & 1, chalf = wave >> 1;
  bf16x8 wfr[CFW][KSD];
#pragma unroll
  for (int c = 0; c < CFW; ++c)
#pragma unroll
    for (int ks = 0; ks < KSD; ++ks) {
      const int ci = (chalf * CFW + c) * 16 + (lane & 15), co = ks * 32 + (lane >> 4) * 8;
      wfr[c][ks] = *reinterpret_cast<const bf16x8*>(P.W + (int64_t)ci * CO + co);
    }
  const int d_row = 16 * pf + (lane & 15);
  const int d_base = d_row * YROWB, d_swz = dual_swz<YROWB>(d_row), d_hi = lane >> 4;

  const int g = lane >> 4, j16 = lane & 15;
  const int t_row = 8 * (g >> 1) + (j16 >> 2);
  const int t_low = 2 * (g & 1) + ((j16 >> 1) & 1), t_half = (j16 & 1) * 8;
  f32x16 acc2[DO_W ? WF : 1];
  if (DO_W) {
#pragma unroll
    for (int f = 0; f < WF; ++f)
#pragma unroll
      for (int e = 0; e < 16; ++e) acc2[f][e] = 0.f;
  }
  const int w_fix = WIDE_O ? wave % NFI : wave % NFO;
  const int w_var0 = WIDE_O ? (wave / NFI) * WF : (wave / NFO) * WF;
#define B1_TR_OFF(ROWB_, chunk_, plus4_) \
  ((t_row + (plus4_)) * (ROWB_) + ((((chunk_) + t_low) ^ dual_swz<ROWB_>(t_row + (plus4_))) << 4) + t_half)

  constexpr int DXP = PX * (CI / 8) / THREADS;
  static_assert(PX * (CI / 8) % THREADS == 0, "whole pieces per thread");
  constexpr int W_N = L * (NST - 2), W_A = W_N + DXP * (NST - 1);
  uint4 addv[DXP];
#define B1_FLUSH(ktp_, second_barrier_)                                                                    \
  {                                                                                                        \
    const int p0_ = (kt_begin + (ktp_) * kt_step) * PX;                                                              \
    const unsigned char* src_ = dxs + ((ktp_) & (NDX - 1)) * DX_BYTES;                                     \
    uint4 v_[DXP];                                                                                         \
    _Pragma("unroll") for (int q = 0; q < DXP; ++q) {                                                      \
      const int idx = q * THREADS + tid, row = idx / (CI / 8), ch = idx % (CI / 8);                        \
      v_[q] = *reinterpret_cast<const uint4*>(src_ + row * DXROWB + ch * 16);                              \
    }                                                                                                      \
    if (second_barrier_) __syncthreads();                                                                  \
    _Pragma("unroll") for (int q = 0; q < DXP; ++q) {                                                      \
      const int idx = q * THREADS + tid, row = idx / (CI / 8), ch = idx % (CI / 8);                        \
      if (p0_ + row < P.M) {                                                                               \
        uint4 v = v_[q];                                                                                   \
        if (P.ADD) {                                                                                       \
          const uint4 a = addv[q];                                                                         \
          v.x = add_bf16x2(v.x, a.x); v.y = add_bf16x2(v.y, a.y); v.z = add_bf16x2(v.z, a.z); v.w = add_bf16x2(v.w, a.w); \
        }                                                                                                  \
        *reinterpret_cast<uint4*>(P.DX + (int64_t)(p0_ + row) * CI + ch * 8) = v;                          \
      }                                                                                                    \
    }                                                                                                      \
  }
  for (int t = 0; t < NST - 1; ++t)
    if (t < KT) B1_ISSUE(t, t);
  for (int kt = 0; kt < KT; ++kt) {
    if (kt + NST - 1 <= KT) {
      if (P.ADD && kt >= NST - 1) wait_vmcnt<W_A>();
      else wait_vmcnt<W_N>();
    } else {
      wait_vmcnt<0>();
    }
    if constexpr (BNA) {
      unsigned char* const Yw = smem + (kt % NST) * STAGE;
      const int p0 = (kt_begin + kt * kt_step) * PX;
#pragma unroll
      for (int q = 0; q < YPW; ++q) {
        unsigned char* const pd = Yw + (q * 4 + wave) * 1024 + lane * 16;
        const uint4 d4 = *reinterpret_cast<const uint4*>(pd), x4 = *reinterpret_cast<const uint4*>(pd + Y3_OFF);
        const uint32_t mb = Yw[B_OFF + wave * 256 + (2 * q + (lane >> 5)) * 32 + (y_col[q] >> 3)];
        const bool rowok = p0 + y_row[q] < P.M;
        uint32_t o4[4];
#pragma unroll
        for (int dd = 0; dd < 4; ++dd) {
          const uint32_t dw_ = dword_of(d4, dd), xw_ = dword_of(x4, dd);
          const float dz0 = (mb >> (2 * dd)) & 1u ? __uint_as_float(dw_ << 16) : 0.f;
          const float dz1 = (mb >> (2 * dd + 1)) & 1u ? __uint_as_float(dw_ & 0xFFFF0000u) : 0.f;
          const f32x2 o = {bn_bwd_dx(dz0, __uint_as_float(xw_ << 16), pm[2 * dd], pis[2 * dd], pa[2 * dd], pb[2 * dd], pc[2 * dd]),
                           bn_bwd_dx(dz1, __uint_as_float(xw_ & 0xFFFF0000u), pm[2 * dd + 1], pis[2 * dd + 1], pa[2 * dd + 1],
                                     pb[2 * dd + 1], pc[2 * dd + 1])};
          o4[dd] = rowok ? __builtin_bit_cast(uint32_t, __builtin_convertvector(o, bf16x2)) : 0u;
        }
        *reinterpret_cast<uint4*>(pd) = make_uint4(o4[0], o4[1], o4[2], o4[3]);
      }
    }
    asm volatile("s_waitcnt lgkmcnt(0)" ::: "memory");
    __builtin_amdgcn_s_barrier();
    asm volatile("" ::: "memory");
    if (kt + NST - 1 < KT) B1_ISSUE(kt + NST - 1, (kt + NST - 1) % NST);
    asm volatile("" ::: "memory");
    __builtin_amdgcn_sched_barrier(0);
    if (kt > 0) B1_FLUSH(kt - 1, !DXDB);
    asm volatile("" ::: "memory");
    __builtin_amdgcn_sched_barrier(0);
    const unsigned char* Ys = smem + (kt % NST) * STAGE;
    const unsigned char* Xs = Ys + Y_BYTES;
    if (P.ADD) {
      const int p0 = (kt_begin + kt * kt_step) * PX;
#pragma unroll
      for (int q = 0; q < DXP; ++q) {
        const int idx = q * THREADS + tid, row = idx / (CI / 8), ch = idx % (CI / 8);
        addv[q] = p0 + row < P.M ? *reinterpret_cast<const uint4*>(P.ADD + (int64_t)(p0 + row) * CI + ch * 8) : make_uint4(0u, 0u, 0u, 0u);
      }
    }
    asm volatile("" ::: "memory");
    __builtin_amdgcn_sched_barrier(0);
    f32x4 acc1[CFW];
#pragma unroll
    for (int c = 0; c < CFW; ++c) acc1[c] = (f32x4){0.f, 0.f, 0.f, 0.f};
#pragma unroll
    for (int ks = 0; ks < KSD; ++ks) {
      const bf16x8 yf = *reinterpret_cast<const bf16x8*>(Ys + d_base + (((4 * ks + d_hi) ^ d_swz) << 4));
#pragma unroll
      for (int c = 0; c < CFW; ++c) acc1[c] = __builtin_amdgcn_mfma_f32_16x16x32_bf16(wfr[c][ks], yf, acc1[c], 0, 0, 0);
    }
    if (DO_W) {
#pragma unroll
      for (int k2 = 0; k2 < 2; ++k2) {
        bf16x8 fa[WIDE_O ? 1 : WF], fb[WIDE_O ? WF : 1];
        if (WIDE_O) {
          fa[0] = lds_read_tr_pair(Xs + k2 * 16 * XROWB + B1_TR_OFF(XROWB, w_fix * 4, 0), Xs + k2 * 16 * XROWB + B1_TR_OFF(XROWB, w_fix * 4, 4));
#pragma unroll
          for (int f = 0; f < WF; ++f)
            fb[f] = lds_read_tr_pair(Ys + k2 * 16 * YROWB + B1_TR_OFF(YROWB, (w_var0 + f) * 4, 0),
                                     Ys + k2 * 16 * YROWB + B1_TR_OFF(YROWB, (w_var0 + f) * 4, 4));
#pragma unroll
          for (int f = 0; f < WF; ++f) acc2[f] = __builtin_amdgcn_mfma_f32_32x32x16_bf16(fa[0], fb[f], acc2[f], 0, 0, 0);
        } else {
          fb[0] = lds_read_tr_pair(Ys + k2 * 16 * YROWB + B1_TR_OFF(YROWB, w_fix * 4, 0), Ys + k2 * 16 * YROWB + B1_TR_OFF(YROWB, w_fix * 4, 4));
#pragma unroll
          for (int f = 0; f < WF; ++f)
            fa[f] = lds_read_tr_pair(Xs + k2 * 16 * XROWB + B1_TR_OFF(XROWB, (w_var0 + f) * 4, 0),
                                     Xs + k2 * 16 * XROWB + B1_TR_OFF(XROWB, (w_var0 + f) * 4, 4));
#pragma unroll
          for (int f = 0; f < WF; ++f) acc2[f] = __builtin_amdgcn_mfma_f32_32x32x16_bf16(fa[f], fb[0], acc2[f], 0, 0, 0);
        }
      }
    }
    {
      const int prow = 16 * pf + (lane & 15);
      unsigned char* const dst = dxs + (kt & (NDX - 1)) * DX_BYTES;
#pragma unroll
      for (int c = 0; c < CFW; ++c) {
        const f32x2 lo = {acc1[c][0], acc1[c][1]}, hi2 = {acc1[c][2], acc1[c][3]};
        uint2 pk;
        pk.x = __builtin_bit_cast(uint32_t, __builtin_convertvector(lo, bf16x2));
        pk.y = __builtin_bit_cast(uint32_t, __builtin_convertvector(hi2, bf16x2));
        *reinterpret_cast<uint2*>(dst + prow * DXROWB + ((chalf * CFW + c) * 16 + (lane >> 4) * 4) * 2) = pk;
      }
    }
  }
  if (KT > 0) {
    __syncthreads();
    B1_FLUSH(KT - 1, false);
  }
#undef B1_FLUSH
#undef B1_ISSUE
#undef B1_TR_OFF
  if (DO_W) {
    float* const out = P.SLAB + (int64_t)split * CI * CO;
#pragma unroll
    for (int f = 0; f < WF; ++f) {
      const int fi = WIDE_O ? w_fix : w_var0 + f, fo = WIDE_O ? w_var0 + f : w_fix;
#pragma unroll
      for (int e = 0; e < 16; ++e) {
        const int ci = fi * 32 + (e & 3) + 8 * (e >> 2) + 4 * (lane >> 5), co = fo * 32 + (lane & 31);
        out[(int64_t)ci * CO + co] = acc2[f][e];
      }
    }
  }
}

static inline int bwd1x1_kind(const RiglConvDesc* d) {
  if (d->kh != 1 || d->kw != 1 || d->stride_h != 1 || d->stride_w != 1 || d->pad_top || d->pad_left) return 0;
  if (d->ho != d->h || d->wo != d->w) return 0;
  const int knob = RIGL_TUNE("bwd1x1", 1);
  if (knob == 0 || (int64_t)d->n * d->h * d->w < (knob == 2 ? 8192 : 65536)) return 0;
  if (d->cin == 64 && d->cout == 256) return 1;
  if (d->cin == 64 && d->cout == 64) return 3;
  return 0;
}
static inline int bwd1x1_splits() { return 2 * num_cus(); }
static inline size_t bwd1x1_workspace(const RiglConvDesc* d) {
  return bwd1x1_kind(d) ? (size_t)2 * num_cus() * d->cin * d->cout * 4 : 0;
}
template <int CI, int CO, bool DO_W, int NST>
static bool bwd1x1_ready_i() {
  constexpr int SMEM = Bwd1x1Smem<CI, CO, DO_W, NST>::BYTES;
  static_assert(SMEM <= 160 * 1024 / 2, "the rings of the two workgroups resident on a CU fit its LDS");
  static const bool ready = hipFuncSetAttribute(reinterpret_cast<const void*>(&k_bwd1x1<CI, CO, DO_W, NST>),
                                                hipFuncAttributeMaxDynamicSharedMemorySize, SMEM) == hipSuccess;
  return ready;
}
static bool bwd1x1_ready(const RiglConvDesc* d) {
  switch (bwd1x1_kind(d)) {
    case 1: return bwd1x1_ready_i<64, 256, true, 3>();
    case 3: return bwd1x1_ready_i<64, 64, true, 3>();
    default: return false;
  }
}
template <int CI, int CO, bool DO_W, int NST>
static bool launch_bwd1x1_i(const Bwd1x1Args& a, hipStream_t st) {
  constexpr int SMEM = Bwd1x1Smem<CI, CO, DO_W, NST>::BYTES;
  if (!bwd1x1_ready_i<CI, CO, DO_W, NST>()) return false;
  RIGL_K_LAUNCH((k_bwd1x1<CI, CO, DO_W, NST>), dim3((unsigned)a.splits), dim3(THREADS), SMEM, st, a);
  return true;
}
template <int CI, int CO>
static bool launch_bwd1x1_t(const Bwd1x1Args& a, bool w, hipStream_t st) {
  return w ? launch_bwd1x1_i<CI, CO, true, 3>(a, st) : launch_bwd1x1_i<CI, CO, false, 3>(a, st);
}
static bool launch_bwd1x1(const RiglConvDesc* d, const rigl_bf16* x, const rigl_bf16* dy, const rigl_bf16* w_hwio,
                          const rigl_bf16* addend, rigl_bf16* dx, float* slab, hipStream_t st) {
  Bwd1x1Args a = {};
  a.X = x; a.DY = dy; a.W = w_hwio; a.ADD = addend; a.DX = dx; a.SLAB = slab;
  a.M = d->n * d->h * d->w; a.splits = bwd1x1_splits(); a.interleave = RIGL_TUNE("bwd1x1_il", 1);
  a.x_bytes = (uint32_t)((size_t)a.M * d->cin * 2); a.dy_bytes = (uint32_t)((size_t)a.M * d->cout * 2);
  const bool w = slab != nullptr;
  switch (bwd1x1_kind(d)) {
    case 1: return launch_bwd1x1_t<64, 256>(a, w, st);
    case 3: return launch_bwd1x1_t<64, 64>(a, w, st);
    default: return false;
  }
}

static bool bwd1x1_bna_ready(const RiglConvDesc* d) {
  if (!RIGL_TUNE("bn_bwd_on_load", 1) || bwd1x1_kind(d) != 1 || !bwd1x1_ready(d)) return false;
  constexpr int SMEM = Bwd1x1Smem<64, 256, true, 4, true>::BYTES;
  static_assert(SMEM <= 160 * 1024, "the ring fits a CU's LDS");
  static const bool ready = hipFuncSetAttribute(reinterpret_cast<const void*>(&k_bwd1x1<64, 256, true, 4, true>),
                                                hipFuncAttributeMaxDynamicSharedMemorySize, SMEM) == hipSuccess;
  return ready;
}
static bool launch_bwd1x1_bna(const RiglConvDesc* d, const rigl_bf16* x, const rigl_bf16* dout, const rigl_bf16* w_hwio,
                              const rigl_bf16* addend, rigl_bf16* dx, float* slab, const rigl_bf16* y3, const uint8_t* bits,
                              const float* mean, const float* invstd, const float* coef, hipStream_t st) {
  if (!bwd1x1_bna_ready(d)) return false;
  Bwd1x1Args a = {};
  a.X = x; a.DY = dout; a.W = w_hwio; a.ADD = addend; a.DX = dx; a.SLAB = slab;
  a.M = d->n * d->h * d->w; a.splits = bwd1x1_splits(); a.interleave = RIGL_TUNE("bwd1x1_il", 1);
  a.x_bytes = (uint32_t)((size_t)a.M * d->cin * 2); a.dy_bytes = (uint32_t)((size_t)a.M * d->cout * 2);
  a.Y3 = y3; a.BITS = bits; a.MEAN = mean; a.INVSTD = invstd; a.COEF = coef;
  RIGL_K_LAUNCH((k_bwd1x1<64, 256, true, 4, true>), dim3((unsigned)a.splits), dim3(THREADS),
                (Bwd1x1Smem<64, 256, true, 4, true>::BYTES), st, a);
  return true;
}
```

rigl_amd/ops.py:

```python
import ctypes as C
import os

import torch

from rigl_amd import _lib
from rigl_amd._lib import (ConvDesc, PackLayer, PruneRegrowLayer,
                           PruneRegrowParams, RiglError, check)

_workspaces = {}


_raw_stream = getattr(torch._C, '_cuda_getCurrentRawStream', None)
_cur_device = getattr(torch._C, '_cuda_getDevice', None)


def _stream():
  if _raw_stream is not None and _cur_device is not None:
    return C.c_void_p(_raw_stream(_cur_device()))
  return C.c_void_p(torch.cuda.current_stream().cuda_stream)


def _ptr(t):
  return C.c_void_p(t.data_ptr()) if t is not None else C.c_void_p(0)

# ... 218 lines not shown
      _ptr(w_shadow), _stream()))


def masked_adam(w, grad, m, v, beta_powers, lr=None, beta1=0.9, beta2=0.999, epsilon=1e-8, mask_bits=None,
                weight_decay=0.0, grad_scale=1.0, w_shadow=None, lr_device=None):
  _lr_device(lr, lr_device)
  _req(w, torch.float32, 'w')
  _req(grad, torch.float32, 'grad')
  _req(m, torch.float32, 'm')
  _req(v, torch.float32, 'v')
  _req(beta_powers, torch.float32, 'beta_powers')
  _req(mask_bits, torch.int32, 'mask_bits', allow_none=True)
  _req(w_shadow, torch.bfloat16, 'w_shadow', allow_none=True)
  n = w.numel()
  if grad.numel() != n or m.numel() != n or v.numel() != n or beta_powers.numel() != 2:
    raise ValueError('size mismatch')
  if mask_bits is not None and mask_bits.numel() < n_mask_words(n):
    raise ValueError('mask_bits too small')
  if w_shadow is not None and w_shadow.numel() != n:
    raise ValueError('w_shadow size mismatch')
  if lr_device is not None:
    check(_lib.load().rigl_masked_adam_dlr(
        n, _ptr(w), _ptr(m), _ptr(v), _ptr(grad), _ptr(mask_bits), _ptr(beta_powers), _ptr(lr_device), float(beta1),
        float(beta2), float(epsilon), float(weight_decay), float(grad_scale), _ptr(w_shadow), _stream()))
    return
  check(_lib.load().rigl_masked_adam(
      n, _ptr(w), _ptr(m), _ptr(v), _ptr(grad), _ptr(mask_bits), _ptr(beta_powers), float(lr), float(beta1),
      float(beta2), float(epsilon), float(weight_decay), float(grad_scale), _ptr(w_shadow), _stream()))


def adam_advance(beta_powers, beta1=0.9, beta2=0.999):
  _req(beta_powers, torch.float32, 'beta_powers')
  if beta_powers.numel() != 2:
    raise ValueError('beta_powers must hold 2 floats')
  check(_lib.load().rigl_adam_advance(_ptr(beta_powers), float(beta1), float(beta2), _stream()))


def lr_schedule_step(sched, step, lr_out):
  if not isinstance(sched, _lib.LrSchedule):
    raise TypeError('sched: expected an LrSchedule descriptor, got %s' % type(sched).__name__)
  _req(step, torch.int32, 'step')
  _req(lr_out, torch.float32, 'lr_out')
  if step.numel() != 1 or lr_out.numel() != 1:
    raise ValueError('step and lr_out must hold 1 element each')
  check(_lib.load().rigl_lr_schedule_step(C.byref(sched), _ptr(step), _ptr(lr_out), _stream()))


def pack_weights_batched(layers):
  nl = len(layers)
  if nl == 0:
    return
  arr = (PackLayer * nl)()
  for i, (w, bits, k, cout, hwio, ohwi) in enumerate(layers):
    _req(w, torch.float32, 'w')
    _req(bits, torch.int32, 'mask_bits', allow_none=True)
    _req(hwio, torch.bfloat16, 'hwio', allow_none=True)
    _req(ohwi, torch.bfloat16, 'ohwi', allow_none=True)
    if w.numel() != k * cout:
      raise ValueError('pack_weights: w has %d elements, k*cout=%d' %
                       (w.numel(), k * cout))
    arr[i].w = w.data_ptr()
    arr[i].mask_bits = bits.data_ptr() if bits is not None else None
    arr[i].hwio = hwio.data_ptr() if hwio is not None else None
    arr[i].ohwi = ohwi.data_ptr() if ohwi is not None else None
    arr[i].k = k
    arr[i].cout = cout
  check(_lib.load().rigl_pack_weights_batched(arr, nl, _stream()))


def pack_weights(w, mask_bits, k, cout, hwio=None, ohwi=None):
  pack_weights_batched([(w, mask_bits, k, cout, hwio, ohwi)])


WORK = {'fwd_macs': 0, 'dgrad_macs': 0, 'wgrad_macs': 0, 'depthwise_bytes': 0}
_work_on = False


def work_count(on=True):
  global _work_on
  _work_on = bool(on)
  if on:
    for k in WORK:
      WORK[k] = 0


def _count_macs(kind, d):
  if _work_on:
    WORK[kind] += d.n * d.ho * d.wo * d.kh * d.kw * d.cin * d.cout


def _count_depthwise(d):
  if _work_on:
    WORK['depthwise_bytes'] += 2 * d.n * (d.h * d.w + d.ho * d.wo) * d.cin




_GEN_WORD = None


def _plan_cached(d, name, fn):
  global _GEN_WORD
  if _GEN_WORD is None:
    _GEN_WORD = C.c_uint64.from_address(_lib.load().rigl_tune_generation_addr())
  gen = _GEN_WORD.value
  c = getattr(d, '_plan', None)
  if c is None or c[0] != gen:
    c = (gen, {})
    d._plan = c
  v = c[1].get(name)
  if v is None:
    v = c[1][name] = fn()
  return v


def conv_desc(n, h, w, cin, cout, kh, kw, stride, pad_top, pad_left, ho, wo):
  sh, sw = (stride, stride) if isinstance(stride, int) else stride
  return ConvDesc(n, h, w, cin, ho, wo, cout, kh, kw, sh, sw, pad_top,
                  pad_left)


def mfma_supported(d):
  return d.cout % 8 == 0


def mfma_dgrad_supported(d):
  return d.cout % 8 == 0 and d.cin % 8 == 0


def conv_fwd(d, x, w_ohwi, y=None, force_ref=False, stats=False, *, scale_shift=None, residual=None, relu=False, part=None):
  if scale_shift is not None or residual is not None or relu:
    if scale_shift is None or stats or force_ref:
      raise ValueError('conv_fwd: residual / relu need scale_shift, and the eval epilogue leaves no statistics')
    return _conv_fwd_infer(d, x, None, w_ohwi, scale_shift, residual, relu, y)
  _req(x, torch.bfloat16, 'x')
  _req(w_ohwi, torch.bfloat16, 'w_ohwi')
  _count_macs('fwd_macs', d)
  y = _out(y, (d.n, d.ho, d.wo, d.cout), torch.bfloat16, x.device, 'y')
  lib = _lib.load()
  if force_ref or not mfma_supported(d):
    check(lib.rigl_conv2d_fwd_ref(C.byref(d), _ptr(x), _ptr(w_ohwi), _ptr(y),
                                  _stream()))
    return (y, None) if stats else y
  need = _plan_cached(d, 'ws_fwd', lambda: lib.rigl_conv2d_workspace_bytes(C.byref(d), 0))
  d._stats_parts = _plan_cached(d, 'stats_parts', lambda: lib.rigl_conv2d_stats_parts(C.byref(d)))
  ws = workspace(need, x.device) if need else None
  if stats:
    part = _stats_out(part, d._stats_parts, d.cout, x.device)
  else:
    part = None
  check(lib.rigl_masked_conv2d_fwd_stats(
      C.byref(d), _ptr(x), _ptr(w_ohwi), _ptr(y), _ptr(part),
      part.numel() if part is not None else 0, _ptr(ws),
      ws.numel() if ws is not None else 0, _stream()))
  return (y, part) if stats else y


def _stats_out(part, parts, c, device):
  if part is None:
    return torch.empty((parts, 2, c), dtype=torch.float32, device=device)
  _req(part, torch.float32, 'part')
  if tuple(part.shape) != (parts, 2, c):
    raise ValueError('part must be [%d, 2, %d]' % (parts, c))
  return part


def _out(t, shape, dtype, device, name):
  if t is None:
    return torch.empty(shape, dtype=dtype, device=device)
  _req(t, dtype, name)
  n = 1
  for s in shape:
    n *= s
  if t.numel() != n:
    raise ValueError('%s must hold %d elements (%s)' % (name, n, 'x'.join(map(str, shape))))
  return t


def conv_fwd_takes_bn_input(d):
  if not mfma_supported(d):
    return False
  return bool(_plan_cached(d, 'fwd_bn_input', lambda: int(_lib.load().rigl_conv2d_fwd_takes_bn_input(C.byref(d)))))


def conv_fwd_bnrelu(d, x_pre, saved, w_ohwi, a_out, y=None, stats=False, *, scale_shift=None, residual=None, relu=False, part=None):
  if a_out is None:
    if stats:
      raise ValueError('conv_fwd_bnrelu: the eval form leaves no statistics')
    if scale_shift is None and (residual is not None or relu):
      raise ValueError('conv_fwd_bnrelu: residual / relu need scale_shift')
    return _conv_fwd_infer(d, x_pre, saved, w_ohwi, scale_shift, residual, relu, y)
  if scale_shift is not None or residual is not None or relu:
    raise ValueError('conv_fwd_bnrelu: the epilogue arguments belong to the eval form (a_out None)')
  _req(x_pre, torch.bfloat16, 'x_pre')
  _req(a_out, torch.bfloat16, 'a_out')
  _req(w_ohwi, torch.bfloat16, 'w_ohwi')
  _req(saved, torch.float32, 'saved')
  if saved.numel() != 4 * d.cin or a_out.numel() != x_pre.numel() or x_pre.numel() != d.n * d.h * d.w * d.cin:
    raise ValueError('saved must be [4, Cin]; x_pre and a_out [n, h, w, Cin]')
  _count_macs('fwd_macs', d)
  y = _out(y, (d.n, d.ho, d.wo, d.cout), torch.bfloat16, x_pre.device, 'y')
  lib = _lib.load()
  if stats:
    parts = _plan_cached(d, 'stats_parts', lambda: lib.rigl_conv2d_stats_parts(C.byref(d)))
    part = _stats_out(part, parts, d.cout, x_pre.device)
  else:
    part = None
  check(lib.rigl_masked_conv2d_fwd_bnrelu(C.byref(d), _ptr(x_pre), _ptr(saved[2]), _ptr(a_out), _ptr(w_ohwi), _ptr(y), _ptr(part),
                                          part.numel() if part is not None else 0, None, 0, _stream()))
  return (y, part) if stats else y


def conv_fwd_takes_bn_epilogue(d, bn_on_load=False, residual=False):
  if not mfma_supported(d):
    return False
  a, r = int(bool(bn_on_load)), int(bool(residual))
  return bool(_plan_cached(d, 'fwd_bn_epilogue%d%d' % (a, r),
                           lambda: int(_lib.load().rigl_conv2d_fwd_takes_bn_epilogue(C.byref(d), a, r))))


def _conv_fwd_infer(d, x, in_ss, w_ohwi, ss, residual, relu, y):
  _req(x, torch.bfloat16, 'x')
  _req(w_ohwi, torch.bfloat16, 'w_ohwi')
  for t, nm, c in ((in_ss, 'in_scale_shift', d.cin), (ss, 'scale_shift', d.cout)):
    if t is not None:
      _req(t, torch.float32, nm)
      if t.dim() != 2 or t.shape[0] not in (2, 4) or t.shape[1] != c:
        raise ValueError('%s must be [2, %d] (or a [4, %d] saved block)' % (nm, c, c))
  if x.numel() != d.n * d.h * d.w * d.cin:
    raise ValueError('x must be [n, h, w, Cin] of the descriptor')
  _req(residual, torch.bfloat16, 'residual', allow_none=True)
  if residual is not None and residual.numel() != d.n * d.ho * d.wo * d.cout:
    raise ValueError('residual must have the shape of the output')
  y = _out(y, (d.n, d.ho, d.wo, d.cout), torch.bfloat16, x.device, 'y')
  if conv_fwd_takes_bn_epilogue(d, in_ss is not None, residual is not None):
    _count_macs('fwd_macs', d)
    check(_lib.load().rigl_masked_conv2d_fwd_bn_infer(
        C.byref(d), _ptr(x), _ptr(in_ss[-2] if in_ss is not None else None), _ptr(w_ohwi),
        _ptr(ss[-2] if ss is not None else None), _ptr(residual), int(bool(relu)), _ptr(y), _stream()))
    return y
  if in_ss is not None:
    x = bn_apply(x, in_ss, relu=True)
    if ss is not None and conv_fwd_takes_bn_epilogue(d, False, residual is not None):
      return _conv_fwd_infer(d, x, None, w_ohwi, ss, residual, relu, y)
  if ss is None:
    return conv_fwd(d, x, w_ohwi, y)
  return bn_apply(conv_fwd(d, x, w_ohwi), ss, relu=relu, residual=residual, y=y)


def conv_dgrad(d, dy, w_hwio, dx=None, force_ref=False, addend=None):
  _count_macs('dgrad_macs', d)
  _req(dy, torch.bfloat16, 'dy')
  _req(w_hwio, torch.bfloat16, 'w_hwio')
  dx = _out(dx, (d.n, d.h, d.w, d.cin), torch.bfloat16, dy.device, 'dx')
  if addend is not None:
    _req(addend, torch.bfloat16, 'addend')
    if addend.numel() != dx.numel():
      raise ValueError('addend must have the shape of dx')
  lib = _lib.load()
  if force_ref or not mfma_dgrad_supported(d):
    check(lib.rigl_conv2d_dgrad_ref(C.byref(d), _ptr(dy), _ptr(w_hwio),
                                    _ptr(dx), _stream()))
    if addend is not None:
      dx += addend.view_as(dx)
    return dx
  check(lib.rigl_masked_conv2d_dgrad_acc(C.byref(d), _ptr(dy), _ptr(w_hwio),
                                         _ptr(addend), _ptr(dx), None, 0,
                                         _stream()))
  return dx


def conv_wgrad(d, x, dy, dw=None, force_ref=False):
  _count_macs('wgrad_macs', d)
  _req(x, torch.bfloat16, 'x')
  _req(dy, torch.bfloat16, 'dy')
  dw = _out(dw, (d.kh * d.kw * d.cin * d.cout,), torch.float32, x.device, 'dw')
  lib = _lib.load()
  if force_ref or not mfma_supported(d):
    check(lib.rigl_conv2d_wgrad_ref(C.byref(d), _ptr(x), _ptr(dy), _ptr(dw),
                                    _stream()))
    return dw
  need = _plan_cached(d, 'ws_wgrad', lambda: lib.rigl_conv2d_workspace_bytes(C.byref(d), 2))
  ws = workspace(need, x.device) if need else None
  check(lib.rigl_masked_conv2d_wgrad(C.byref(d), _ptr(x), _ptr(dy), _ptr(dw),
                                     _ptr(ws),
                                     ws.numel() if ws is not None else 0,
                                     _stream()))
  return dw


def dgrad_stats_parts(d):
  v = _plan_cached(d, 'dgrad_parts', lambda: int(_lib.load().rigl_conv2d_dgrad_stats_parts(C.byref(d))))
  return v


def conv_bwd_takes_masked_addend(d):
  return bool(_plan_cached(d, 'masked_addend', lambda: int(_lib.load().rigl_conv2d_bwd_takes_masked_addend(C.byref(d)))))


def conv_bwd_takes_bn_apply(d):
  if not (mfma_supported(d) and mfma_dgrad_supported(d)):
    return False
  return bool(_plan_cached(d, 'bwd_bn_apply', lambda: int(_lib.load().rigl_conv2d_bwd_takes_bn_apply(C.byref(d)))))


def _conv_bwd(d, x, dy, w_hwio, dw, dx, on_dw_ready, launch, need_dx=True, dx_shape=None, dgrad_desc=None, f32=False):
  act = torch.float32 if f32 else torch.bfloat16
  _req(x, act, 'x')
  _req(dy, act, 'dy')
  _req(dw, torch.float32, 'dw')
  lib = _lib.load()
  _count_macs('wgrad_macs', d)
  if f32:
    need = _plan_cached(d, 'ws_wgrad_f32', lambda: lib.rigl_conv2d_wgrad_f32_workspace_bytes(C.byref(d)))
  else:
    need = _plan_cached(d, 'ws_wgrad', lambda: lib.rigl_conv2d_workspace_bytes(C.byref(d), 2))
  ws = workspace(need, x.device, 'wg32' if f32 else 'wg') if need else None
  if need_dx:
    _req(w_hwio, act, 'w_hwio')
    _count_macs('dgrad_macs', dgrad_desc if dgrad_desc is not None else d)
    dx = _out(dx, dx_shape or (d.n, d.h, d.w, d.cin), act, dy.device, 'dx')
  else:
    dx = None
  check(launch(lib, _ptr(dx), _ptr(ws), ws.numel() if ws is not None else 0))
  if on_dw_ready is not None:
    on_dw_ready()
  return dx


def conv_bwd_bnapply(d, x, dout, w_hwio, dw, y, relu_bits, saved, coef, addend=None, on_dw_ready=None, dx=None):
  if not conv_bwd_takes_bn_apply(d):
    raise ValueError('this layer\'s backward does not take the batch-norm apply (conv_bwd_takes_bn_apply)')
  _req(dout, torch.bfloat16, 'dout')
  _req(y, torch.bfloat16, 'y')
  _req(addend, torch.bfloat16, 'addend', allow_none=True)
  _req(saved, torch.float32, 'saved'); _req(coef, torch.float32, 'coef')
  _req(relu_bits, torch.uint8, 'relu_bits')
  n_out = d.n * d.ho * d.wo * d.cout
  if dout.numel() != n_out or y.numel() != n_out or relu_bits.numel() * 8 != n_out:
    raise ValueError('dout and y must have the shape of the conv output and relu_bits one bit per element of it')
  if saved.numel() != 4 * d.cout or coef.numel() != 3 * d.cout:
    raise ValueError('saved must be [4, Cout] and coef [3, Cout]')
  if addend is not None and addend.numel() != d.n * d.h * d.w * d.cin:
    raise ValueError('addend must have the shape of dx')
  return _conv_bwd(d, x, dout, w_hwio, dw, dx, on_dw_ready, lambda lib, pdx, ws, nws: lib.rigl_masked_conv2d_bwd_bnapply(
      C.byref(d), _ptr(x), _ptr(dout), _ptr(w_hwio), _ptr(addend), _ptr(dw), pdx, ws, nws, _ptr(y), _ptr(relu_bits),
      _ptr(saved[0]), _ptr(saved[1]), _ptr(coef), _stream()))


def conv_bwd(d, x, dy, w_hwio, dw, need_dx=True, addend=None, on_dw_ready=None, bn_fuse=None, addend_sub=None,
             addend_bits=None, dx=None):
  if addend_sub is not None and tuple(addend_sub) == (1, 1):
    addend_sub = None
  n_in = d.n * d.h * d.w * d.cin
  both = mfma_supported(d) and mfma_dgrad_supported(d)
  if addend_bits is not None:
    if addend is None or not need_dx or bn_fuse is not None or addend_sub is not None:
      raise ValueError('addend_bits needs an addend and dX, and combines with neither bn_fuse nor addend_sub')
    _req(addend, torch.bfloat16, 'addend'); _req(addend_bits, torch.uint8, 'addend_bits')
    if addend.numel() != n_in or addend_bits.numel() * 8 != n_in:
      raise ValueError('addend must have the shape of dx and addend_bits one bit per element of it')
    return _conv_bwd(d, x, dy, w_hwio, dw, dx, on_dw_ready, lambda lib, pdx, ws, nws: lib.rigl_masked_conv2d_bwd_masked(
        C.byref(d), _ptr(x), _ptr(dy), _ptr(w_hwio), _ptr(addend), _ptr(addend_bits), _ptr(dw), pdx, ws, nws, _stream()))
  if addend_sub is not None:
    if addend is None or not need_dx or bn_fuse is not None:
      raise ValueError('addend_sub needs an addend and dX, and does not combine with bn_fuse')
    if not both:
      raise ValueError('addend_sub needs cin % 8 == cout % 8 == 0')
  if bn_fuse is not None:
    bn_fuse.pop('partials', None)
    if not (need_dx and both and dgrad_stats_parts(d) > 0):
      bn_fuse = None
  if not (mfma_supported(d) and (not need_dx or mfma_dgrad_supported(d))):
    conv_wgrad(d, x, dy, dw)
    if on_dw_ready is not None:
      on_dw_ready()
    return conv_dgrad(d, dy, w_hwio, dx=dx, addend=addend) if need_dx else None
  _req(addend, torch.bfloat16, 'addend', allow_none=True)
  if addend_sub is not None:
    sh, sw = addend_sub
    if addend.numel() != d.n * (-(-d.h // sh)) * (-(-d.w // sw)) * d.cin:
      raise ValueError('addend must be [n, ceil(h / sh), ceil(w / sw), cin]')
    return _conv_bwd(d, x, dy, w_hwio, dw, dx, on_dw_ready, lambda lib, pdx, ws, nws: lib.rigl_masked_conv2d_bwd_sub(
        C.byref(d), _ptr(x), _ptr(dy), _ptr(w_hwio), _ptr(addend), int(sh), int(sw), _ptr(dw), pdx, ws, nws, _stream()))
  if need_dx and addend is not None and addend.numel() != n_in:
    raise ValueError('addend must have the shape of dx')
  bn = None
  if bn_fuse is not None:
    bx, saved = bn_fuse['x'], bn_fuse['saved']
    _req(bx, torch.bfloat16, 'bn x')
    _req(saved, torch.float32, 'bn saved')
    bits = bn_fuse.get('relu_bits')
    _req(bits, torch.uint8, 'bn relu_bits', allow_none=True)
    if bx.numel() != n_in or saved.numel() != 4 * d.cin:
      raise ValueError('bn_fuse: x must have the shape of dx and saved must be [4, Cin]')
    part = torch.empty((dgrad_stats_parts(d), 2, d.cin), dtype=torch.float32, device=dy.device)
    bn = C.byref(_lib.BnReduceFuse(bx.data_ptr(), bits.data_ptr() if bits is not None else None, saved.data_ptr(),
                                   int(bool(bn_fuse['relu'])), part.data_ptr(), part.numel()))
    bn_fuse['partials'] = part
  return _conv_bwd(d, x, dy, w_hwio, dw, dx, on_dw_ready, lambda lib, pdx, ws, nws: lib.rigl_masked_conv2d_bwd_bn(
      C.byref(d), _ptr(x), _ptr(dy), _ptr(w_hwio), _ptr(addend), _ptr(dw), pdx, ws, nws, bn, _stream()), need_dx=need_dx)


def conv_bwd_grid(d, x, dy, w_hwio, dw, on_dw_ready=None, dx=None):
  grid = ConvDesc(d.n, d.ho, d.wo, d.cin, d.ho, d.wo, d.cout, 1, 1, 1, 1, 0, 0)
  return _conv_bwd(d, x, dy, w_hwio, dw, dx, on_dw_ready, lambda lib, pdx, ws, nws: lib.rigl_masked_conv2d_bwd_grid(
      C.byref(d), _ptr(x), _ptr(dy), _ptr(w_hwio), _ptr(dw), pdx, ws, nws, _stream()),
                   dx_shape=(d.n, d.ho, d.wo, d.cin), dgrad_desc=grid)


def conv_fwd_takes_relu_epilogue(d):
  return bool(_plan_cached(d, 'fwd_relu_epi', lambda: int(_lib.load().rigl_conv2d_fwd_takes_relu_epilogue(C.byref(d)))))


def conv_bwd_takes_relu_epilogue(d):
  return bool(_plan_cached(d, 'bwd_relu_epi', lambda: int(_lib.load().rigl_conv2d_bwd_takes_relu_epilogue(C.byref(d)))))


def conv_fwd_relu(d, x, w_ohwi, y=None):
  _req(x, torch.bfloat16, 'x')
  _req(w_ohwi, torch.bfloat16, 'w_ohwi')
  if x.numel() != d.n * d.h * d.w * d.cin:
    raise ValueError('x must be [n, h, w, Cin] of the descriptor')
  _count_macs('fwd_macs', d)
  y = _out(y, (d.n, d.ho, d.wo, d.cout), torch.bfloat16, x.device, 'y')
  lib = _lib.load()
  need = _plan_cached(d, 'ws_fwd', lambda: lib.rigl_conv2d_workspace_bytes(C.byref(d), 0))
  ws = workspace(need, x.device) if need else None
  check(lib.rigl_masked_conv2d_fwd_relu(C.byref(d), _ptr(x), _ptr(w_ohwi), _ptr(y), _ptr(ws),
                                        ws.numel() if ws is not None else 0, _stream()))
  return y


def conv_bwd_relu(d, x, dy, w_hwio, dw, on_dw_ready=None, dx=None):
  _req(x, torch.bfloat16, 'x')
  _req(dy, torch.bfloat16, 'dy')
  if x.numel() != d.n * d.h * d.w * d.cin or dy.numel() != d.n * d.ho * d.wo * d.cout:
    raise ValueError('x / dy must have the shapes of the descriptor')
  return _conv_bwd(d, x, dy, w_hwio, dw, dx, on_dw_ready, lambda lib, pdx, ws, nws: lib.rigl_masked_conv2d_bwd_relu(
      C.byref(d), _ptr(x), _ptr(dy), _ptr(w_hwio), _ptr(dw), pdx, ws, nws, _stream()))


def relu_fwd(x, y=None):
  _req(x, torch.bfloat16, 'x')
  if y is None:
    y = torch.empty_like(x)
  _req(y, torch.bfloat16, 'y')
  if y.numel() != x.numel():
    raise ValueError('y must have the shape of x')
  check(_lib.load().rigl_relu_fwd(x.numel(), _ptr(x), _ptr(y), _stream()))
  return y


def relu_bwd(dy, x, dx=None):
  _req(dy, torch.bfloat16, 'dy')
  _req(x, torch.bfloat16, 'x')
  if dx is None:
    dx = torch.empty_like(dy)
  _req(dx, torch.bfloat16, 'dx')
  if not dy.numel() == x.numel() == dx.numel():
    raise ValueError('dy, x and dx must have one shape')
  check(_lib.load().rigl_relu_bwd(dy.numel(), _ptr(dy), _ptr(x), _ptr(dx), _stream()))
  return dx


def conv_fwd_f32(d, x, w_hwio, mask_bits=None, y=None):
  _req(x, torch.float32, 'x')
  _req(w_hwio, torch.float32, 'w_hwio')
  _req(mask_bits, torch.int32, 'mask_bits', allow_none=True)
  _count_macs('fwd_macs', d)
  if y is None:
    y = torch.empty((d.n, d.ho, d.wo, d.cout), dtype=torch.float32, device=x.device)
  _req(y, torch.float32, 'y')
  check(_lib.load().rigl_masked_conv2d_fwd_f32(C.byref(d), _ptr(x), _ptr(w_hwio), _ptr(mask_bits), _ptr(y), _stream()))
  return y


def conv_bwd_f32(d, x, dy, w_hwio, mask_bits, dw, need_dx=True, addend=None, on_dw_ready=None, dx=None):
  _req(addend, torch.float32, 'addend', allow_none=True)
  _req(mask_bits, torch.int32, 'mask_bits', allow_none=True)
  if need_dx and addend is not None and addend.numel() != d.n * d.h * d.w * d.cin:
    raise ValueError('addend must have the shape of dx')
  dx = _conv_bwd(d, x, dy, w_hwio, dw, dx, on_dw_ready, lambda lib, pdx, ws, nws: lib.rigl_masked_conv2d_wgrad_f32(
      C.byref(d), _ptr(x), _ptr(dy), _ptr(dw), ws, nws, _stream()), need_dx=need_dx, f32=True)
  if need_dx:
    check(_lib.load().rigl_masked_conv2d_dgrad_f32(C.byref(d), _ptr(dy), _ptr(w_hwio), _ptr(mask_bits), _ptr(addend), _ptr(dx),
                                                   _stream()))
  return dx


def depthwise_fwd(d, x, w, stats=False, y=None, part=None):
  _count_depthwise(d)
  _req(x, torch.bfloat16, 'x')
  _req(w, torch.float32, 'w')
  y = _out(y, (d.n, d.ho, d.wo, d.cout), torch.bfloat16, x.device, 'y')
  lib = _lib.load()
  if stats:
    parts = _plan_cached(d, 'dw_parts', lambda: int(lib.rigl_depthwise_conv2d_stats_parts(C.byref(d))))
    if parts > 0:
      part = _stats_out(part, parts, d.cout, x.device)
      check(lib.rigl_depthwise_conv2d_fwd_stats(C.byref(d), _ptr(x), _ptr(w), _ptr(y), _ptr(part), part.numel(), _stream()))
      return y, part
  check(lib.rigl_depthwise_conv2d_fwd(C.byref(d), _ptr(x), _ptr(w), _ptr(y), _stream()))
  return (y, None) if stats else y


def depthwise_dgrad(d, dy, w, dx=None):
  _count_depthwise(d)
  _req(dy, torch.bfloat16, 'dy')
  _req(w, torch.float32, 'w')
  dx = _out(dx, (d.n, d.h, d.w, d.cin), torch.bfloat16, dy.device, 'dx')
  check(_lib.load().rigl_depthwise_conv2d_dgrad(C.byref(d), _ptr(dy), _ptr(w), _ptr(dx), _stream()))
  return dx


def depthwise_wgrad(d, x, dy, dw):
  _count_depthwise(d)
  _req(x, torch.bfloat16, 'x')
  _req(dy, torch.bfloat16, 'dy')
  _req(dw, torch.float32, 'dw')
  lib = _lib.load()
  ws = workspace(lib.rigl_depthwise_conv2d_workspace_bytes(C.byref(d)), x.device)
  check(lib.rigl_depthwise_conv2d_wgrad(C.byref(d), _ptr(x), _ptr(dy), _ptr(dw), _ptr(ws), ws.numel(), _stream()))
  return dw


def _bn_plan(x, partials=None, need_ws=False):
  _req(x, torch.bfloat16, 'x')
  c = x.shape[-1]
  m = x.numel() // c
  parts = 0
  if partials is not None:
    _req(partials, torch.float32, 'partials')
    if partials.dim() != 3 or partials.shape[1] != 2 or partials.shape[2] != c:
      raise ValueError('partials must be [parts, 2, %d]' % c)
    parts = partials.shape[0]
  ws = workspace(_lib.load().rigl_bn_workspace_bytes(m, c), x.device) if (need_ws or partials is None) else None
  return m, c, ws, parts


def bn_fwd(x, gamma, beta, running_mean, running_var, momentum, eps, relu,
           residual=None, partials=None, want_relu_bits=False):
  _req(residual, torch.bfloat16, 'residual', allow_none=True)
  for t, nm in ((gamma, 'gamma'), (beta, 'beta')):
    _req(t, torch.float32, nm)
  m, c, ws, parts = _bn_plan(x, partials)
  y = torch.empty_like(x)
  saved = torch.empty((4, c), dtype=torch.float32, device=x.device)
  bits = torch.empty(x.numel() // 8, dtype=torch.uint8, device=x.device) \
      if (want_relu_bits and relu) else None
  check(_lib.load().rigl_bn_fwd_stats(
      m, c, _ptr(x), _ptr(residual), _ptr(gamma), _ptr(beta),
      _ptr(running_mean), _ptr(running_var), float(momentum), float(eps),
      int(bool(relu)), _ptr(y), _ptr(saved[0]), _ptr(saved[1]), _ptr(saved[2]),
      _ptr(saved[3]), _ptr(partials), parts, _ptr(bits), _ptr(ws),
      ws.numel() if ws is not None else 0, _stream()))
  return (y, saved, bits) if want_relu_bits else (y, saved)


def bn_bwd(x, y, dy, gamma, saved, relu, dgamma, dbeta, want_dres=False,
           relu_bits=None, partials=None):
  _req(relu_bits, torch.uint8, 'relu_bits', allow_none=True)
  _req(dy, torch.bfloat16, 'dy')
  _req(y, torch.bfloat16, 'y', allow_none=True)
  m, c, ws, parts = _bn_plan(x, partials, need_ws=True)
  dx = torch.empty_like(x)
  dres = torch.empty_like(x) if want_dres else None
  check(_lib.load().rigl_bn_bwd_stats(m, c, _ptr(x), _ptr(y), _ptr(relu_bits), _ptr(dy), _ptr(gamma),
                                      _ptr(saved[0]), _ptr(saved[1]), _ptr(saved[2]),
                                      _ptr(saved[3]), int(bool(relu)), _ptr(dx), _ptr(dres),
                                      _ptr(dgamma), _ptr(dbeta), _ptr(partials), parts, _ptr(ws), ws.numel(),
                                      _stream()))
  return dx, dres


def bn_bwd_reduce(x, dy, gamma, saved, relu, relu_bits, dgamma, dbeta):
  _req(dy, torch.bfloat16, 'dy')
  _req(relu_bits, torch.uint8, 'relu_bits', allow_none=not relu)
  m, c, ws, _ = _bn_plan(x)
  if dy.numel() != x.numel() or (relu and relu_bits.numel() * 8 != x.numel()):
    raise ValueError('dy must have the shape of x and relu_bits one bit per element of it')
  coef = torch.empty((3, c), dtype=torch.float32, device=x.device)
  check(_lib.load().rigl_bn_bwd_reduce(m, c, _ptr(x), _ptr(relu_bits) if relu else None, _ptr(dy), _ptr(gamma), _ptr(saved[0]),
                                       _ptr(saved[1]), int(bool(relu)), _ptr(dgamma), _ptr(dbeta), _ptr(coef), _ptr(ws),
                                       ws.numel(), _stream()))
  return coef


def _i32(v):
  v = int(v) & 0xFFFFFFFF
  return v - (1 << 32) if v >= 1 << 31 else v


def stateless_random(n, seed0, seed1, dist, scale=1.0, shift=0.0, device=None,
                     out=None):
  if dist not in ('uniform', 'normal'):
    raise ValueError('dist must be "uniform" or "normal"')
  if out is None:
    out = torch.empty(int(n), dtype=torch.float32, device=device)
  _req(out, torch.float32, 'out')
  check(_lib.load().rigl_stateless_random(_ptr(out), out.numel(), _i32(seed0), _i32(seed1),
                                          1 if dist == 'normal' else 0,
                                          float(scale), float(shift), _stream()))
  return out


def stateless_random_batched(items, device):
  if not items:
    return []
  offs, total = [], 0
  for it in items:
    offs.append(total)
    total += (int(it[0]) + 63) // 64 * 64
  buf = torch.empty(max(total, 1), dtype=torch.float32, device=device)
  arr = (_lib.RandomItem * len(items))()
  outs = []
  for i, (n, s0, s1, dist, scale, shift) in enumerate(items):
    if dist not in ('uniform', 'normal'):
      raise ValueError('dist must be "uniform" or "normal"')
    t = buf[offs[i]:offs[i] + int(n)]
    outs.append(t)
    arr[i].out = t.data_ptr() if int(n) else None
    arr[i].n = int(n)
    arr[i].seed0, arr[i].seed1 = _i32(s0), _i32(s1)
    arr[i].dist = 1 if dist == 'normal' else 0
    arr[i].scale, arr[i].shift = float(scale), float(shift)
  check(_lib.load().rigl_stateless_random_batched(arr, len(items), _stream()))
  return outs


_DROPOUT_DTYPES = {torch.bfloat16: 0, torch.float32: 1}


def _dropout_dtype(t, name):
  _req(t, getattr(t, 'dtype', None), name)
  if t.dtype not in _DROPOUT_DTYPES:
    raise TypeError('%s: expected bfloat16 or float32, got %s' % (name, t.dtype))
  return _DROPOUT_DTYPES[t.dtype]


def dropout_fwd(x, rate, seed0, step, y=None, bits=None):
  dt = _dropout_dtype(x, 'x')
  _req(step, torch.int32, 'step')
  if step.numel() != 1:
    raise ValueError('step must hold one int32')
  n = x.numel()
  if y is None:
    y = torch.empty_like(x)
  if bits is None:
    bits = torch.empty((n + 7) // 8, dtype=torch.uint8, device=x.device)
  _req(y, x.dtype, 'y')
  _req(bits, torch.uint8, 'bits')
  if y.numel() != n or bits.numel() < (n + 7) // 8:
    raise ValueError('y must have the shape of x and bits ceil(n / 8) bytes')
  check(_lib.load().rigl_dropout_fwd(_ptr(x), _ptr(y), _ptr(bits), n, dt, float(rate), _i32(seed0), _ptr(step), _stream()))
  return y, bits


def dropout_bwd(dy, bits, rate, dx=None):
  dt = _dropout_dtype(dy, 'dy')
  _req(bits, torch.uint8, 'bits')
  n = dy.numel()
  if dx is None:
    dx = torch.empty_like(dy)
  _req(dx, dy.dtype, 'dx')
  if dx.numel() != n or bits.numel() < (n + 7) // 8:
    raise ValueError('dx must have the shape of dy and bits ceil(n / 8) bytes')
  check(_lib.load().rigl_dropout_bwd(_ptr(dy), _ptr(bits), _ptr(dx), n, dt, float(rate), _stream()))
  return dx


def dropout_advance(step):
  _req(step, torch.int32, 'step')
  if step.numel() != 1:
    raise ValueError('step must hold one int32')
  check(_lib.load().rigl_dropout_advance(_ptr(step), _stream()))


def cifar_batch(images, labels, batch, step, out, out_labels, out_index=None, train=True, seed0=0, shard=0, n_shards=1):
  _req(images, torch.uint8, 'images')
  _req(labels, torch.int32, 'labels')
  _req(step, torch.int32, 'step')
  dt = _dropout_dtype(out, 'out')
  _req(out_labels, torch.int32, 'out_labels')
  _req(out_index, torch.int32, 'out_index', allow_none=True)
  if step.numel() != 1:
    raise ValueError('step must hold one int32')
  if images.dim() != 4 or tuple(images.shape[1:]) != (32, 32, 3):
    raise ValueError('images must be [N, 32, 32, 3] uint8 (HWC), got %s' % (tuple(images.shape),))
  n = images.shape[0]
  batch = int(batch)
  if labels.numel() != n:
    raise ValueError('labels must hold one int32 per image')
  if batch > 0 and (out.numel() != batch * 3072 or out_labels.numel() != batch or
                    (out_index is not None and out_index.numel() != batch)):
    raise ValueError('out must be [batch, 32, 32, 3] and out_labels / out_index [batch]')
  check(_lib.load().rigl_cifar_batch(_ptr(images), _ptr(labels), n, batch, 0 if train else 1, int(shard), int(n_shards),
                                     _i32(seed0), _ptr(step), _ptr(out), dt, _ptr(out_labels), _ptr(out_index), _stream()))


def cifar_advance(step):
  _req(step, torch.int32, 'step')
  if step.numel() != 1:
    raise ValueError('step must hold one int32')
  check(_lib.load().rigl_cifar_advance(_ptr(step), _stream()))


def maxpool_fwd(d, x):
  _req(x, torch.bfloat16, 'x')
  y = torch.empty((d.n, d.ho, d.wo, d.cout), dtype=torch.bfloat16, device=x.device)
  arg = torch.empty((d.n, d.ho, d.wo, d.cout), dtype=torch.uint8, device=x.device)
  check(_lib.load().rigl_maxpool_fwd(C.byref(d), _ptr(x), _ptr(y), _ptr(arg), _stream()))
  return y, arg


def maxpool_bwd(d, dy, arg):
  _req(dy, torch.bfloat16, 'dy')
  _req(arg, torch.uint8, 'argmax')
  dx = torch.empty((d.n, d.h, d.w, d.cin), dtype=torch.bfloat16, device=dy.device)
  check(_lib.load().rigl_maxpool_bwd(C.byref(d), _ptr(dy), _ptr(arg), _ptr(dx), _stream()))
  return dx


def bn_statistics(x, gamma, beta, running_mean, running_var, momentum, eps, partials=None):
  m, c, ws, parts = _bn_plan(x, partials)
  saved = torch.empty((4, c), dtype=torch.float32, device=x.device)
  check(_lib.load().rigl_bn_fwd_statistics(
      m, c, _ptr(x), _ptr(gamma), _ptr(beta), _ptr(running_mean), _ptr(running_var), float(momentum), float(eps),
      _ptr(saved[0]), _ptr(saved[1]), _ptr(saved[2]), _ptr(saved[3]), _ptr(partials), parts, _ptr(ws),
      ws.numel() if ws is not None else 0, _stream()))
  return saved


def bn_add_bn_fwd(x, x2, saved2, gamma, beta, running_mean, running_var, momentum, eps, relu, partials=None):
  _req(x2, torch.bfloat16, 'x2')
  if x2.shape != x.shape:
    raise ValueError('x2 must have the shape of x')
  m, c, ws, parts = _bn_plan(x, partials)
  y = torch.empty_like(x)
  saved = torch.empty((4, c), dtype=torch.float32, device=x.device)
  bits = torch.empty(x.numel() // 8, dtype=torch.uint8, device=x.device) if relu else None
  check(_lib.load().rigl_bn_add_bn_fwd(
      m, c, _ptr(x), _ptr(x2), _ptr(saved2[2]), _ptr(saved2[3]), _ptr(gamma), _ptr(beta), _ptr(running_mean),
      _ptr(running_var), float(momentum), float(eps), int(bool(relu)), _ptr(y), _ptr(saved[0]), _ptr(saved[1]),
      _ptr(saved[2]), _ptr(saved[3]), _ptr(partials), parts, _ptr(bits),
      _ptr(ws), ws.numel() if ws is not None else 0, _stream()))
  return y, saved, bits


def bn_add_bn_bwd(x, x2, relu_bits, dy, gamma, saved, gamma2, saved2, dgamma, dbeta, dgamma2, dbeta2):
  _req(x, torch.bfloat16, 'x')
  _req(x2, torch.bfloat16, 'x2')
  _req(dy, torch.bfloat16, 'dy')
  _req(relu_bits, torch.uint8, 'relu_bits')
  c = x.shape[-1]
  m = x.numel() // c
  lib = _lib.load()
  ws = workspace(lib.rigl_bn_add_bn_bwd_workspace_bytes(m, c), x.device)
  dx, dx2 = torch.empty_like(x), torch.empty_like(x2)
  check(lib.rigl_bn_add_bn_bwd(m, c, _ptr(x), _ptr(x2), _ptr(relu_bits), _ptr(dy), _ptr(gamma), _ptr(saved[0]), _ptr(saved[1]),
                               _ptr(gamma2), _ptr(saved2[0]), _ptr(saved2[1]), _ptr(dx), _ptr(dx2), _ptr(dgamma), _ptr(dbeta),
                               _ptr(dgamma2), _ptr(dbeta2), _ptr(ws), ws.numel(), _stream()))
  return dx, dx2


def bn_relu_maxpool_fwd(d, x, gamma, beta, running_mean, running_var, momentum, eps, partials=None):
  saved = bn_statistics(x, gamma, beta, running_mean, running_var, momentum, eps, partials=partials)
  lib = _lib.load()
  y = torch.empty((d.n, d.ho, d.wo, d.cout), dtype=torch.bfloat16, device=x.device)
  arg = torch.empty((d.n, d.ho, d.wo, d.cout), dtype=torch.uint8, device=x.device)
  check(lib.rigl_bn_relu_maxpool_fwd(C.byref(d), _ptr(x), _ptr(saved[2]), _ptr(saved[3]), _ptr(y), _ptr(arg), _stream()))
  return y, arg, saved


def bn_relu_maxpool_bwd(d, x, dy, arg, gamma, saved, dgamma, dbeta):
  _req(x, torch.bfloat16, 'x')
  _req(dy, torch.bfloat16, 'dy')
  _req(arg, torch.uint8, 'argmax')
  lib = _lib.load()
  ws = workspace(lib.rigl_bn_relu_maxpool_bwd_workspace_bytes(C.byref(d)), x.device)
  dx = torch.empty_like(x)
  check(lib.rigl_bn_relu_maxpool_bwd(C.byref(d), _ptr(x), _ptr(dy), _ptr(arg), _ptr(gamma), _ptr(saved[0]), _ptr(saved[1]),
                                     _ptr(saved[2]), _ptr(saved[3]), _ptr(dx), _ptr(dgamma), _ptr(dbeta), _ptr(ws),
                                     ws.numel(), _stream()))
  return dx


def global_avgpool_fwd(x):
  _req(x, torch.bfloat16, 'x')
  n, h, w, c = x.shape
  y = torch.empty((n, c), dtype=torch.bfloat16, device=x.device)
  check(_lib.load().rigl_global_avgpool_fwd(n, h * w, c, _ptr(x), _ptr(y), _stream()))
  return y


def global_avgpool_bwd(dy, h, w):
  _req(dy, torch.bfloat16, 'dy')
  n, c = dy.shape
  dx = torch.empty((n, h, w, c), dtype=torch.bfloat16, device=dy.device)
  check(_lib.load().rigl_global_avgpool_bwd(n, h * w, c, _ptr(dy), _ptr(dx), _stream()))
  return dx


def global_avgpool_bwd_relu(dy, x):
  _req(dy, torch.bfloat16, 'dy')
  _req(x, torch.bfloat16, 'x')
  n, h, w, c = x.shape
  if tuple(dy.shape) != (n, c):
    raise ValueError('dy must be [N, C] of x')
  dx = torch.empty_like(x)
  check(_lib.load().rigl_global_avgpool_bwd_relu(n, h * w, c, _ptr(dy), _ptr(x), _ptr(dx), _stream()))
  return dx


def softmax_xent(logits, labels, label_smoothing=0.0, grad_scale=None, want_grad=True):
  _req(logits, torch.bfloat16, 'logits')
  _req(labels, torch.int64, 'labels')
  rows, k = logits.shape
  if labels.numel() != rows:
    raise ValueError('softmax_xent: %d labels for %d rows' % (labels.numel(), rows))
  loss = torch.empty(rows, dtype=torch.float32, device=logits.device)
  dz = torch.empty_like(logits) if want_grad else None
  check(_lib.load().rigl_softmax_xent(rows, k, _ptr(logits), _ptr(labels), float(label_smoothing),
                                      1.0 / rows if grad_scale is None else float(grad_scale), _ptr(loss), _ptr(dz),
                                      _stream()))
  return loss, dz


def bn_infer_params(bns, out=None):
  bns = list(bns)
  if not bns:
    return []
  total = sum(2 * b.moving_mean.numel() for b in bns)
  dev = bns[0].moving_mean.device
  if out is None:
    out = torch.empty(total, dtype=torch.float32, device=dev)
  _req(out, torch.float32, 'out')
  if out.numel() < total:
    raise ValueError('bn_infer_params: out holds %d floats < %d' % (out.numel(), total))
  arr = (_lib.BnInferItem * len(bns))()
  views, off = [], 0
  for i, b in enumerate(bns):
    c = b.moving_mean.numel()
    for t, nm in ((b.gamma.data, 'gamma'), (b.beta.data, 'beta'), (b.moving_mean, 'moving_mean'),
                  (b.moving_variance, 'moving_variance')):
      _req(t, torch.float32, nm)
      if t.numel() != c:
        raise ValueError('bn_infer_params: %s has %d channels, not %d' % (nm, t.numel(), c))
    v = out[off:off + 2 * c].view(2, c)
    arr[i] = _lib.BnInferItem(b.gamma.data.data_ptr(), b.beta.data.data_ptr(), b.moving_mean.data_ptr(),
                              b.moving_variance.data_ptr(), v.data_ptr(), c, float(b.eps))
    views.append(v)
    off += 2 * c
  check(_lib.load().rigl_bn_infer_params_batched(arr, len(bns), _stream()))
  return views


def _req_ss(ss, c, name='scale_shift'):
  _req(ss, torch.float32, name)
  if ss.dim() != 2 or ss.shape[0] not in (2, 4) or ss.shape[1] != c:
    raise ValueError('%s must be [2, %d] (or a [4, %d] saved block)' % (name, c, c))
  return ss[-2]


def bn_apply(x, scale_shift, relu=False, residual=None, y=None):
  _req(x, torch.bfloat16, 'x')
  _req(residual, torch.bfloat16, 'residual', allow_none=True)
  c = x.shape[-1]
  row = _req_ss(scale_shift, c)
  if residual is not None and residual.shape != x.shape:
    raise ValueError('residual must have the shape of x')
  if y is None:
    y = torch.empty_like(x)
  _req(y, torch.bfloat16, 'y')
  check(_lib.load().rigl_bn_apply(x.numel() // c, c, _ptr(x), _ptr(residual), _ptr(row), int(bool(relu)), _ptr(y), _stream()))
  return y


def bn_apply_pair(x, x2, scale_shift, scale_shift2, relu=True):
  _req(x, torch.bfloat16, 'x')
  _req(x2, torch.bfloat16, 'x2')
  if x2.shape != x.shape:
    raise ValueError('x2 must have the shape of x')
  c = x.shape[-1]
  r1, r2 = _req_ss(scale_shift, c), _req_ss(scale_shift2, c, 'scale_shift2')
  y = torch.empty_like(x)
  check(_lib.load().rigl_bn_apply_pair(x.numel() // c, c, _ptr(x), _ptr(x2), _ptr(r1), _ptr(r2), int(bool(relu)), _ptr(y),
                                       _stream()))
  return y


def bn_relu_maxpool_infer(d, x, scale_shift):
  _req(x, torch.bfloat16, 'x')
  row = _req_ss(scale_shift, d.cin)
  y = torch.empty((d.n, d.ho, d.wo, d.cout), dtype=torch.bfloat16, device=x.device)
  check(_lib.load().rigl_bn_relu_maxpool_infer(C.byref(d), _ptr(x), _ptr(row), _ptr(y), _stream()))
  return y


def eval_metrics(logits, labels, label_smoothing=0.0, topk=5, counts=None):
  _req(logits, torch.bfloat16, 'logits')
  _req(labels, torch.int64, 'labels')
  _req(counts, torch.int64, 'counts', allow_none=True)
  if counts is not None and counts.numel() != 3:
    raise ValueError('counts must be int64 [3]')
  rows, k = logits.shape
  if labels.numel() != rows:
    raise ValueError('eval_metrics: %d labels for %d rows' % (labels.numel(), rows))
  loss = torch.empty(rows, dtype=torch.float32, device=logits.device)
  flags = torch.empty(rows, dtype=torch.int32, device=logits.device)
  check(_lib.load().rigl_eval_metrics(rows, k, _ptr(logits), _ptr(labels), float(label_smoothing), int(topk), _ptr(loss),
                                      _ptr(flags), _ptr(counts), _stream()))
  return loss, flags


def tune_set(key, value):
  check(_lib.load().rigl_tune_set(key.encode(), int(value)))


def tune_unset(key):
  check(_lib.load().rigl_tune_unset(key.encode()))


def tune_get(key, default=-1):
  return int(_lib.load().rigl_tune_get(key.encode(), int(default)))


def mfma_peak_probe(device='cuda:0', blocks=2048, iters=2000, reps=5):
  lib = _lib.load()
  sink = torch.zeros(blocks * 256, dtype=torch.float32, device=device)
  best = 0.0
  for r in range(reps + 1):
    s, e = torch.cuda.Event(enable_timing=True), torch.cuda.Event(enable_timing=True)
    s.record()
    check(lib.rigl_probe_mfma_bf16(blocks, iters, _ptr(sink), _stream()))
    e.record()
    e.synchronize()
    if r:
      best = max(best, blocks * 4 * iters * 8 * 32768.0 / (s.elapsed_time(e) * 1e-3) / 1e12)
  return best


def prof_enable(on=True):
  check(_lib.load().rigl_prof_enable(int(bool(on))))


def prof_collect_launches(cap=1 << 16):
  arr = (_lib.ProfLaunch * cap)()
  n = C.c_int64(0)
  check(_lib.load().rigl_prof_collect_launches(arr, cap, C.byref(n)))
  if n.value > cap:
    raise RuntimeError('prof_collect_launches: %d timed dispatches, room for %d (the rest were consumed and dropped): '
                       'collect more often or pass a larger cap' % (n.value, cap))
  return [(_lib.PROF_KINDS[arr[i].kind], tuple(arr[i].tag), float(arr[i].ms)) for i in range(min(n.value, cap))]


def prof_collect():
  ms = (C.c_double * len(_lib.PROF_KINDS))()
  cnt = (C.c_int64 * len(_lib.PROF_KINDS))()
  check(_lib.load().rigl_prof_collect_kinds(ms, cnt, len(_lib.PROF_KINDS)))
  return {k: (ms[i], cnt[i]) for i, k in enumerate(_lib.PROF_KINDS)}
```

rigl_amd/pruning_layers.py:

```python
import math
import os

import numpy as np
import torch

from rigl_amd import ops
from rigl_amd import variables as V


def _same_pad(size, k, stride):
  out = -(-size // stride)
  total = max((out - 1) * stride + k - size, 0)
  return out, total // 2


def _valid_out(size, k, stride):
  return (size - k) // stride + 1


_BN_FUSE_BWD = os.environ.get('RIGL_BN_FUSE_BWD', '0') == '1'
_CONV_PAIR = os.environ.get('RIGL_CONV_PAIR', '1') != '0'
_BN_FUSE_MAX_BYTES = float(os.environ.get('RIGL_BN_FUSE_MAX_MB', '1e9')) * 1e6


def _bn_source(x):
  h = getattr(x, 'bn_ctx', None) if _BN_FUSE_BWD else None
  if h is not None:
    h.attached += 1
  return h


def _bn_fuse_request(holder, need_dx):
  if holder is None or not need_dx or holder.attached != 1 or holder.x is None:
    return None
  if holder.x.numel() * 2 > _BN_FUSE_MAX_BYTES:
    return None
  return dict(x=holder.x, saved=holder.saved, relu=holder.relu, relu_bits=holder.bits)


def _bn_fuse_publish(holder, req, dx):
  if req is not None and req.get('partials') is not None and dx is not None:
    holder.partials, holder.dx_ptr = req['partials'], dx.data_ptr()


class _HandOver:
  __slots__ = ('armed', 'grad', 'payload')
  knob = did = None

  def __init__(self):
    self.armed = False
    self.grad = self.payload = None

  def fill(self, grad, *payload):
    self.grad, self.payload = grad, payload

  def take(self, grad):
    filled, payload = self.grad, self.payload
    self.grad = self.payload = None
    if self.armed != (filled is not None):
      raise RuntimeError('%s: the batch norm %s but the forward had decided otherwise' % (self.knob, self.did[filled is None]))
    if filled is None:
      return None
    if grad is not filled and (grad is None or grad.data_ptr() != filled.data_ptr() or grad.shape != filled.shape
                               or not grad.is_contiguous()):
      raise RuntimeError('%s: the gradient that reached the conv is not the one the batch norm handed over' % self.knob)
    return payload


class BnApplyHolder(_HandOver):
  __slots__ = ()
  knob, did = 'bn_bwd_on_load', ('skipped its apply pass', 'ran its apply pass')


class MaskedAddendHolder(_HandOver):
  __slots__ = ()
  knob, did = 'lazy_res_grad', ('handed the shortcut gradient over unmasked', 'wrote the masked shortcut gradient')


def _conv_forward(lv, desc, x, want_stats):
  if x.dtype == torch.float32:
    return ops.conv_fwd_f32(desc, x, lv.weights.data.view(-1), _mask_bits(lv)), None
  return ops.conv_fwd(desc, x, lv.ohwi, stats=True) if want_stats else (ops.conv_fwd(desc, x, lv.ohwi), None)


def stats_outputs(ctx, want_stats, outs, parts, device):
  if not want_stats:
    return outs if len(outs) > 1 else outs[0]
  parts = tuple(p if p is not None else torch.empty(0, device=device) for p in parts)
  ctx.mark_non_differentiable(*parts)
  ctx.set_materialize_grads(False)
  return outs + parts


def _dw_ready(lv):
  sync = getattr(lv.weights.graph, 'grad_sync', None)
  return (lambda: sync.notify_layer_grad_ready(lv.weights)) if sync is not None else None


def _dy_or_zeros(dy, d, x):
  if dy is None:
    return torch.zeros((d.n, d.ho, d.wo, d.cout), dtype=x.dtype, device=x.device)
  return dy.contiguous()


def _mask_bits(lv):
  return lv.mask.bits if lv.mask is not None else None


class _MaskedConvFn(torch.autograd.Function):

  @staticmethod
  def forward(ctx, x, lv, desc, need_dx, want_stats=False, bn_holder=None, pending=None, apply_holder=None):
    ctx.lv, ctx.desc, ctx.need_dx = lv, desc, need_dx
    ctx.bn_holder, ctx.apply_holder = bn_holder, apply_holder
    ctx.save_for_backward(x)
    if pending is not None:
      out = ops.conv_fwd_bnrelu(desc, pending.x, pending.saved, lv.ohwi, x, stats=want_stats)
      y, part = out if want_stats else (out, None)
    else:
      y, part = _conv_forward(lv, desc, x, want_stats)
    return stats_outputs(ctx, want_stats, (y,), (part,), x.device)

  @staticmethod
  def backward(ctx, dy, _dpart=None):
    (x,) = ctx.saved_tensors
    lv, d = ctx.lv, ctx.desc
    dy = _dy_or_zeros(dy, d, x)
    ready = _dw_ready(lv)
    if x.dtype == torch.float32:
      dx = ops.conv_bwd_f32(d, x, dy, lv.weights.data.view(-1), _mask_bits(lv), lv.weights.grad.view(-1),
                            need_dx=ctx.need_dx, on_dw_ready=ready)
      return (dx,) + (None,) * 7
    got = ctx.apply_holder.take(dy) if ctx.apply_holder is not None else None
    if got is not None:
      dx = ops.conv_bwd_bnapply(d, x, dy, lv.hwio, lv.weights.grad.view(-1), *got, on_dw_ready=ready)
      return (dx,) + (None,) * 7
    req = _bn_fuse_request(ctx.bn_holder, ctx.need_dx)
    dx = ops.conv_bwd(d, x, dy, lv.hwio, lv.weights.grad.view(-1), need_dx=ctx.need_dx, on_dw_ready=ready, bn_fuse=req)
    _bn_fuse_publish(ctx.bn_holder, req, dx)
    return (dx,) + (None,) * 7


class _MaskedConvReluFn(torch.autograd.Function):

  @staticmethod
  def forward(ctx, x, lv, desc, need_dx, gate_input):
    ctx.lv, ctx.desc, ctx.need_dx, ctx.gate_input = lv, desc, need_dx, gate_input
    ctx.save_for_backward(x)
    return ops.conv_fwd_relu(desc, x, lv.ohwi)

  @staticmethod
  def backward(ctx, dy):
    (x,) = ctx.saved_tensors
    lv, d = ctx.lv, ctx.desc
    dy, ready = _dy_or_zeros(dy, d, x), _dw_ready(lv)
    if ctx.need_dx and ctx.gate_input:
      dx = ops.conv_bwd_relu(d, x, dy, lv.hwio, lv.weights.grad.view(-1), on_dw_ready=ready)
    else:
      dx = ops.conv_bwd(d, x, dy, lv.hwio, lv.weights.grad.view(-1), need_dx=ctx.need_dx, on_dw_ready=ready)
    return dx, None, None, None, None


class _MaskedConvForkFn(torch.autograd.Function):

  @staticmethod
  def forward(ctx, x, lv, desc, want_stats=False, bn_holder=None, addend_holder=None):
    ctx.lv, ctx.desc = lv, desc
    ctx.bn_holder, ctx.addend_holder = bn_holder, addend_holder
    ctx.save_for_backward(x)
    y, part = _conv_forward(lv, desc, x, want_stats)
    return stats_outputs(ctx, want_stats, (y, x.view_as(x)), (part,), x.device)

  @staticmethod
  def backward(ctx, dy, dalias, _dpart=None):
    (x,) = ctx.saved_tensors
    lv, d = ctx.lv, ctx.desc
    dy, ready = _dy_or_zeros(dy, d, x), _dw_ready(lv)
    if dalias is not None:
      dalias = dalias.contiguous()
    if x.dtype == torch.float32:
      dx = ops.conv_bwd_f32(d, x, dy, lv.weights.data.view(-1), _mask_bits(lv), lv.weights.grad.view(-1),
                            need_dx=True, addend=dalias, on_dw_ready=ready)
      return (dx,) + (None,) * 5
    got = ctx.addend_holder.take(dalias) if ctx.addend_holder is not None else None
    if got is not None:
      dx = ops.conv_bwd(d, x, dy, lv.hwio, lv.weights.grad.view(-1), need_dx=True, addend=dalias, addend_bits=got[0],
                        on_dw_ready=ready)
      return (dx,) + (None,) * 5
    req = _bn_fuse_request(ctx.bn_holder, True)
    dx = ops.conv_bwd(d, x, dy, lv.hwio, lv.weights.grad.view(-1), need_dx=True, addend=dalias, on_dw_ready=ready, bn_fuse=req)
    _bn_fuse_publish(ctx.bn_holder, req, dx)
    return (dx,) + (None,) * 5


class _MaskedConvPairFn(torch.autograd.Function):

  @staticmethod
  def forward(ctx, x, lv_s, d_s, lv_m, d_m, want_stats):
    ctx.lv_s, ctx.d_s, ctx.lv_m, ctx.d_m = lv_s, d_s, lv_m, d_m
    ctx.save_for_backward(x)
    ys, ps = _conv_forward(lv_s, d_s, x, want_stats)
    ym, pm = _conv_forward(lv_m, d_m, x, want_stats)
    return stats_outputs(ctx, want_stats, (ys, ym), (ps, pm), x.device)

  @staticmethod
  def backward(ctx, dys, dym, _dps=None, _dpm=None):
    (x,) = ctx.saved_tensors
    lv_s, d_s, lv_m, d_m = ctx.lv_s, ctx.d_s, ctx.lv_m, ctx.d_m
    dys, dym = _dy_or_zeros(dys, d_s, x), _dy_or_zeros(dym, d_m, x)
    dxs = ops.conv_bwd_grid(d_s, x, dys, lv_s.hwio, lv_s.weights.grad.view(-1), on_dw_ready=_dw_ready(lv_s))
    dx = ops.conv_bwd(d_m, x, dym, lv_m.hwio, lv_m.weights.grad.view(-1), need_dx=True, addend=dxs,
                      addend_sub=(d_s.stride_h, d_s.stride_w), on_dw_ready=_dw_ready(lv_m))
    return dx, None, None, None, None, None


def conv_pair(conv_sub, conv_main, x, bn_stats=False):
  n, h, w, c = x.shape
  ok = (x.dtype == torch.bfloat16 and x.requires_grad and conv_sub.need_input_grad and conv_main.need_input_grad
        and conv_sub.kh == conv_sub.kw == 1 and max(conv_sub.strides) > 1
        and conv_sub.cin % 8 == 0 and conv_sub.units % 8 == 0 and conv_main.units % 8 == 0
        and _CONV_PAIR and not (_BN_FUSE_BWD and getattr(x, 'bn_ctx', None) is not None))
  d_s = conv_sub.desc_for(n, h, w) if ok else None
  if ok and (d_s.pad_top or d_s.pad_left or d_s.ho != -(-h // d_s.stride_h) or d_s.wo != -(-w // d_s.stride_w)):
    ok = False
  if not ok:
    ys, alias = conv_sub.fork(x, bn_stats)
    return ys, conv_main(alias, bn_stats)
  if c != conv_sub.cin or c != conv_main.cin:
    raise ValueError('expected [N,H,W,%d], got %s' % (conv_sub.cin, tuple(x.shape)))
  conv_sub.graph.refresh_shadows()
  d_m = conv_main.desc_for(n, h, w)
  if not bn_stats:
    return _MaskedConvPairFn.apply(x.contiguous(), conv_sub.vars, d_s, conv_main.vars, d_m, False)
  ys, ym, ps, pm = _MaskedConvPairFn.apply(x.contiguous(), conv_sub.vars, d_s, conv_main.vars, d_m, True)
  if ps.numel():
    ys.bn_partials = ps
  if pm.numel():
    ym.bn_partials = pm
  return ys, ym


class _Layer:

  def __init__(self, graph, scope, shape, sparsity_technique, weight_decay,
               kernel_initializer):
    if sparsity_technique not in ('threshold', 'baseline'):
      raise ValueError(
          'Unsupported sparsity technique {}'.format(sparsity_technique))
    self.graph = graph
    self.scope = scope
    self.masked = sparsity_technique == 'threshold'
    init = kernel_initializer(shape) if kernel_initializer is not None else \
        variance_scaling_initializer()(shape)
    self.vars = graph.add_masked_layer(scope, shape, self.masked, weight_decay,
                                       init)
    self.bias = None

  @property
  def weights(self):
    return self.vars.weights

  @property
  def mask(self):
    return self.vars.mask


class MaskedConv2d(_Layer):

  def __init__(self, graph, scope, cin, units, kernel_size, strides=(1, 1),
               padding='SAME', sparsity_technique='baseline', weight_decay=0.0,
               kernel_initializer=None, need_input_grad=True):
    kh, kw = kernel_size
    super().__init__(graph, scope, (kh, kw, cin, units), sparsity_technique,
                     weight_decay, kernel_initializer)
    if padding not in ('SAME', 'VALID'):
      raise ValueError('padding must be SAME or VALID')
    self.cin, self.units, self.kh, self.kw = cin, units, kh, kw
    self.strides = tuple(strides)
    self.padding = padding
    self.need_input_grad = need_input_grad
    self._descs = {}

  def desc_for(self, n, h, w):
    key = (n, h, w)
    d = self._descs.get(key)
    if d is None:
      sh, sw = self.strides
      if self.padding == 'SAME':
        ho, pt = _same_pad(h, self.kh, sh)
        wo, pl = _same_pad(w, self.kw, sw)
      else:
        ho, pt = _valid_out(h, self.kh, sh), 0
        wo, pl = _valid_out(w, self.kw, sw), 0
      d = ops.conv_desc(n, h, w, self.cin, self.units, self.kh, self.kw,
                        (sh, sw), pt, pl, ho, wo)
      self._descs[key] = d
    return d

  def __call__(self, x, bn_stats=False):
    if x.dim() != 4:
      raise ValueError('Rank not supported {}'.format(x.dim()))
    if x.shape[-1] != self.cin:
      raise ValueError('expected %d input channels, got %d' %
                       (self.cin, x.shape[-1]))
    self.graph.refresh_shadows()
    n, h, w, _ = x.shape
    d = self.desc_for(n, h, w)
    need_dx = self.need_input_grad and x.requires_grad
    holder = _bn_source(x) if need_dx else None
    pending = getattr(x, 'bn_pending', None)
    if pending is not None and (pending.x is None or not x.is_contiguous()):
      raise RuntimeError('a deferred batch-norm output must reach its consumer conv as it was returned')
    if not x.requires_grad:
      x = x.detach().requires_grad_(True)
    apply_holder = BnApplyHolder() if (need_dx and x.dtype == torch.bfloat16 and x.is_cuda and ops.conv_bwd_takes_bn_apply(d)) else None
    if not bn_stats:
      y = _MaskedConvFn.apply(x.contiguous(), self.vars, d, need_dx, False, holder, pending, apply_holder)
    else:
      y, part = _MaskedConvFn.apply(x.contiguous(), self.vars, d, need_dx, True, holder, pending, apply_holder)
      if part.numel():
        y.bn_partials = part
    if apply_holder is not None and y.grad_fn is not None:
      y.bn_apply = apply_holder
    return y

  def conv_relu(self, x, gate_input=True):
    if x.dim() != 4 or x.shape[-1] != self.cin:
      raise ValueError('expected [N,H,W,%d], got %s' % (self.cin, tuple(x.shape)))
    if x.dtype != torch.bfloat16:
      raise NotImplementedError('conv_relu: bf16 activations only')
    self.graph.refresh_shadows()
    n, h, w, _ = x.shape
    d = self.desc_for(n, h, w)
    need_dx = self.need_input_grad and x.requires_grad
    if not x.requires_grad:
      x = x.detach().requires_grad_(True)
    return _MaskedConvReluFn.apply(x.contiguous(), self.vars, d, need_dx, bool(gate_input))

  def takes_bn_input(self, x):
    if not (x.is_cuda and x.dtype == torch.bfloat16 and x.dim() == 4 and x.shape[-1] == self.cin):
      return False
    n, h, w, _ = x.shape
    return ops.conv_fwd_takes_bn_input(self.desc_for(n, h, w))

  def takes_masked_addend(self, x):
    if not (self.need_input_grad and x.requires_grad and x.dtype == torch.bfloat16 and x.dim() == 4) or _BN_FUSE_BWD:
      return False
    n, h, w, _ = x.shape
    return ops.conv_bwd_takes_masked_addend(self.desc_for(n, h, w))

  def fork(self, x, bn_stats=False):
    if x.dim() != 4 or x.shape[-1] != self.cin:
      raise ValueError('expected [N,H,W,%d], got %s' % (self.cin, tuple(x.shape)))
    if not (self.need_input_grad and x.requires_grad):
      return self(x, bn_stats), x
    self.graph.refresh_shadows()
    n, h, w, _ = x.shape
    holder = _bn_source(x)
    addend_holder = MaskedAddendHolder() if self.takes_masked_addend(x) else None
    y, alias, *part = _MaskedConvForkFn.apply(x.contiguous(), self.vars, self.desc_for(n, h, w), bn_stats, holder, addend_holder)
    if part and part[0].numel():
      y.bn_partials = part[0]
    if addend_holder is not None:
      alias.masked_addend = addend_holder
    return y, alias


class MaskedDense(_Layer):

  def __init__(self, graph, scope, n_in, units, use_bias=True,
               sparsity_technique='baseline', weight_decay=0.0,
               kernel_initializer=None, activation=None):
    super().__init__(graph, scope, (n_in, units), sparsity_technique,
                     weight_decay, kernel_initializer)
    self.n_in, self.units = n_in, units
    self.activation = activation
    self._descs = {}
    if use_bias:
      self.bias = graph.add_variable(scope + '/biases', (units,), V.KIND_OTHER, 0.0)

  def __call__(self, x):
    if x.shape[-1] != self.n_in:
      raise ValueError('expected %d inputs, got %d' % (self.n_in, x.shape[-1]))
    self.graph.refresh_shadows()
    lead = x.shape[:-1]
    x2 = x.reshape(-1, 1, 1, self.n_in)
    b = x2.shape[0]
    d = self._descs.get(b)
    if d is None:
      d = ops.conv_desc(b, 1, 1, self.n_in, self.units, 1, 1, 1, 0, 0, 1, 1)
      self._descs[b] = d
    need_dx = x2.requires_grad
    if not x2.requires_grad:
      x2 = x2.detach().requires_grad_(True)
    y = _MaskedConvFn.apply(x2.contiguous(), self.vars, d, need_dx)
    y = y.reshape(*lead, self.units)
    if self.bias is not None:
      y = y + bias_tensor(self.bias).to(y.dtype)
    if self.activation is not None:
      y = self.activation(y)
    return y


def bias_tensor(var):
  leaf = getattr(var, '_leaf', None)
  if leaf is None or leaf.data_ptr() != var.data.data_ptr():
    leaf = var.data.detach().requires_grad_(True)
    var._leaf = leaf
  if leaf.grad is None or leaf.grad.data_ptr() != var.grad.data_ptr():
    leaf.grad = var.grad
  return leaf


_init_rng = np.random.RandomState(0)


def set_init_seed(seed):
  global _init_rng
  _init_rng = np.random.RandomState(seed)


def variance_scaling_initializer(scale=1.0):

  def init(shape):
    fan_in = int(np.prod(shape[:-1]))
    std = math.sqrt(scale / max(1.0, fan_in)) / .87962566103423978
    v = _init_rng.randn(*shape)
    bad = np.abs(v) > 2
    while bad.any():
      v[bad] = _init_rng.randn(int(bad.sum()))
      bad = np.abs(v) > 2
    return (v * std).astype(np.float32)

  return init


def random_normal_initializer(stddev=0.01):
  return lambda shape: (_init_rng.randn(*shape) * stddev).astype(np.float32)


def _regularizer_scale(reg):
  if reg is None:
    return 0.0
  if isinstance(reg, (int, float)):
    return float(reg)
  return float(getattr(reg, 'scale'))


class l2_regularizer:

  def __init__(self, scale):
    self.scale = float(scale)


def sparse_conv2d(x, units, kernel_size, activation=None, use_bias=False,
                  kernel_initializer=None, kernel_regularizer=None,
                  bias_initializer=None, biases_regularizer=None,
                  sparsity_technique='baseline', normalizer_fn=None,
                  strides=(1, 1), padding='SAME', data_format='channels_last',
                  name=None, graph=None):
  del bias_initializer, biases_regularizer
  if data_format == 'channels_last':
    pass
  elif data_format == 'channels_first':
    raise ValueError('channels_first is not supported by the NHWC kernels')
  else:
    raise ValueError('Not a valid channel string:', data_format)
  if x.dim() != 4:
    raise ValueError('Rank not supported {}'.format(x.dim()))
  if sparsity_technique not in ('threshold', 'baseline'):
    raise ValueError(
        'Unsupported sparsity technique {}'.format(sparsity_technique))
  if use_bias:
    raise ValueError('use_bias=True is not used by the reference models')
  g = graph or V.get_default_graph()
  key = name
  layer = g.modules.get(key) if key is not None else None
  if layer is None:
    scope = g.unique_scope(name, 'Conv')
    layer = MaskedConv2d(g, scope, x.shape[-1], units, tuple(kernel_size),
                         tuple(strides), padding, sparsity_technique,
                         _regularizer_scale(kernel_regularizer),
                         kernel_initializer)
    g.modules[scope] = layer
  y = layer(x)
  if normalizer_fn is not None:
    y = normalizer_fn(y)
  if activation is not None:
    y = activation(y)
  return y


def sparse_fully_connected(x, units, activation=None, use_bias=True,
                           kernel_initializer=None, kernel_regularizer=None,
                           bias_initializer=None, biases_regularizer=None,
                           sparsity_technique='baseline', name=None,
                           graph=None):
  del bias_initializer, biases_regularizer
  if sparsity_technique not in ('threshold', 'baseline'):
    raise ValueError(
        'Unsupported sparsity technique {}'.format(sparsity_technique))
  g = graph or V.get_default_graph()
  layer = g.modules.get(name) if name is not None else None
  if layer is None:
    scope = g.unique_scope(name, 'Dense')
    layer = MaskedDense(g, scope, x.shape[-1], units, use_bias,
                        sparsity_technique,
                        _regularizer_scale(kernel_regularizer),
                        kernel_initializer, activation)
    g.modules[scope] = layer
  return layer(x)
```

rigl_amd/workloads/nn.py:

```python
import os

import torch
import torch.nn.functional as F

from rigl_amd import variables as V
from rigl_amd.pruning_layers import bias_tensor, stats_outputs

BATCH_NORM_DECAY = 0.9
BATCH_NORM_EPSILON = 1e-5
_DW_STATS = os.environ.get('RIGL_DW_STATS', '1') != '0'


def activation_dtype(precision=None):
  if precision is None:
    from rigl_amd import ops
    precision = 'float32' if ops.tune_get('k1_fp32', 0) == 1 else 'bfloat16'
  if precision not in ('bfloat16', 'float32'):
    raise ValueError('precision must be bfloat16 or float32, got %r' % (precision,))
  return torch.float32 if precision == 'float32' else torch.bfloat16


def nchw_view(x):
  return x.permute(0, 3, 1, 2)


def nhwc_view(x):
  return x.permute(0, 2, 3, 1)


class _BnBwdHolder:
  __slots__ = ('x', 'saved', 'bits', 'relu', 'attached', 'partials', 'dx_ptr')

  def __init__(self, relu):
    self.x = self.saved = self.bits = self.partials = self.dx_ptr = None
    self.relu = relu
    self.attached = 0


_LAZY_RES_GRAD = os.environ.get('RIGL_LAZY_RES_GRAD', '1') != '0'
_BN_ON_LOAD = os.environ.get('RIGL_BN_ON_LOAD', '0') == '1'


class _FusedBNFn(torch.autograd.Function):

  @staticmethod
  def forward(ctx, x, residual, bn, relu, partials=None, holder=None, addend_holder=None, defer=False, apply_holder=None):
    from rigl_amd import ops
    x_in = x
    x = x.contiguous()
    res = residual.contiguous() if residual is not None else None
    ctx.bn, ctx.relu, ctx.has_res = bn, relu, res is not None
    ctx.holder = holder
    ctx.addend_holder = addend_holder if (_LAZY_RES_GRAD and relu and res is not None and ctx.needs_input_grad[1]) else None
    if ctx.addend_holder is not None:
      addend_holder.armed = True
    ctx.apply_holder = None
    if apply_holder is not None and ctx.addend_holder is not None and not defer and x is x_in and ctx.needs_input_grad[0]:
      ctx.apply_holder = apply_holder
      apply_holder.armed = True
    if defer:
      saved = ops.bn_statistics(x, bn.gamma.data, bn.beta.data, bn.moving_mean, bn.moving_variance, 1.0 - bn.decay, bn.eps,
                                partials=partials)
      ctx.save_for_backward(x, saved)
      holder.x, holder.saved, holder.bits = x, saved, None
      return torch.empty_like(x)
    if relu and res is not None:
      y, saved, bits = ops.bn_fwd(x, bn.gamma.data, bn.beta.data, bn.moving_mean,
                                  bn.moving_variance, 1.0 - bn.decay, bn.eps, relu, res,
                                  partials=partials, want_relu_bits=True)
      ctx.save_for_backward(x, saved, bits)
    else:
      bits = None
      y, saved = ops.bn_fwd(x, bn.gamma.data, bn.beta.data, bn.moving_mean,
                            bn.moving_variance, 1.0 - bn.decay, bn.eps, relu, res,
                            partials=partials)
      ctx.save_for_backward(x, saved)
    if holder is not None:
      holder.x, holder.saved, holder.bits = x, saved, bits
    return y

  @staticmethod
  def backward(ctx, dy):
    from rigl_amd import ops
    bn = ctx.bn
    if ctx.relu and ctx.has_res:
      x, saved, bits = ctx.saved_tensors
    else:
      (x, saved), bits = ctx.saved_tensors, None
    dy = dy.contiguous()
    h, part = ctx.holder, None
    if h is not None:
      if h.partials is not None and h.dx_ptr == dy.data_ptr():
        part = h.partials
      h.partials = h.x = h.saved = h.bits = None
    if ctx.apply_holder is not None:
      coef = ops.bn_bwd_reduce(x, dy, bn.gamma.data, saved, True, bits, bn.gamma.grad, bn.beta.grad)
      ctx.apply_holder.fill(dy, x, bits, saved, coef)
      ctx.addend_holder.fill(dy, bits)
      return dy, dy, None, None, None, None, None, None, None
    if ctx.addend_holder is not None:
      dx, _ = ops.bn_bwd(x, None, dy, bn.gamma.data, saved, ctx.relu, bn.gamma.grad, bn.beta.grad, want_dres=False,
                         relu_bits=bits, partials=part)
      ctx.addend_holder.fill(dy, bits)
      return dx, dy, None, None, None, None, None, None, None
    dx, dres = ops.bn_bwd(x, None, dy, bn.gamma.data, saved, ctx.relu,
                          bn.gamma.grad, bn.beta.grad,
                          want_dres=ctx.has_res and ctx.needs_input_grad[1],
                          relu_bits=bits, partials=part)
    return dx, dres, None, None, None, None, None, None, None


class _BnAddBnFn(torch.autograd.Function):

  @staticmethod
  def forward(ctx, x, x2, bn, bn2, partials, partials2):
    from rigl_amd import ops
    x, x2 = x.contiguous(), x2.contiguous()
    saved2 = ops.bn_statistics(x2, bn2.gamma.data, bn2.beta.data, bn2.moving_mean, bn2.moving_variance,
                               1.0 - bn2.decay, bn2.eps, partials=partials2)
    y, saved, bits = ops.bn_add_bn_fwd(x, x2, saved2, bn.gamma.data, bn.beta.data, bn.moving_mean, bn.moving_variance,
                                       1.0 - bn.decay, bn.eps, True, partials=partials)
    ctx.bn, ctx.bn2 = bn, bn2
    ctx.save_for_backward(x, x2, saved, saved2, bits)
    return y

  @staticmethod
  def backward(ctx, dy):
    from rigl_amd import ops
    x, x2, saved, saved2, bits = ctx.saved_tensors
    bn, bn2 = ctx.bn, ctx.bn2
    dx, dx2 = ops.bn_add_bn_bwd(x, x2, bits, dy.contiguous(), bn.gamma.data, saved, bn2.gamma.data, saved2,
                                bn.gamma.grad, bn.beta.grad, bn2.gamma.grad, bn2.beta.grad)
    return dx, dx2, None, None, None, None


_BN_PAIR_FUSED = os.environ.get('RIGL_BN_PAIR', '1') != '0'


def bn_add_bn_relu(bn, x, bn2, x2, is_training=True):
  c = x.shape[-1]
  if (_BN_PAIR_FUSED and bn.fused and bn2.fused and is_training and x.is_cuda and x.dtype == torch.bfloat16
      and x2.dtype == torch.bfloat16 and x2.shape == x.shape and c % 8 == 0 and c <= 3968):
    px, px2 = getattr(x, 'bn_partials', None), getattr(x2, 'bn_partials', None)
    if not x.requires_grad:
      x = x.detach().requires_grad_(True)
    if not x2.requires_grad:
      x2 = x2.detach().requires_grad_(True)
    return _BnAddBnFn.apply(x, x2, bn, bn2, px, px2)
  return bn(x, is_training, relu=True, residual=bn2(x2, is_training, relu=False))


class BatchNorm:

  def __init__(self, graph, scope, channels, init_zero=False,
               decay=BATCH_NORM_DECAY, eps=BATCH_NORM_EPSILON, fused=True):
    self.gamma = graph.add_variable(scope + '/gamma', (channels,), V.KIND_OTHER,
                                    0.0, init=None)
    if not init_zero:
      self.gamma.data.fill_(1.0)
    self.beta = graph.add_variable(scope + '/beta', (channels,), V.KIND_OTHER)
    self.moving_mean = torch.zeros(channels, device=graph.device)
    self.moving_variance = torch.ones(channels, device=graph.device)
    self.decay, self.eps = decay, eps
    self.channels = channels
    self.fused = fused
    self.scope = scope
    graph.modules[scope] = self

  def __call__(self, x, is_training=True, relu=False, residual=None, consumer=None):
    if (self.fused and is_training and x.is_cuda and self.channels % 8 == 0
        and x.dtype == torch.bfloat16):
      partials = getattr(x, 'bn_partials', None)
      if not x.requires_grad:
        x = x.detach().requires_grad_(True)
      holder = _BnBwdHolder(relu)
      defer = bool(_BN_ON_LOAD and consumer is not None and relu and residual is None and consumer.takes_bn_input(x))
      apply_holder = getattr(x, 'bn_apply', None)
      addend_holder = getattr(residual, 'masked_addend', None)
      y = _FusedBNFn.apply(x, residual, self, relu, partials, holder, addend_holder, defer, apply_holder)
      y.bn_ctx = holder
      if defer:
        y.bn_pending = holder
      return y
    y = F.batch_norm(nchw_view(x), self.moving_mean, self.moving_variance,
                     bias_tensor(self.gamma), bias_tensor(self.beta),
                     is_training, 1.0 - self.decay, self.eps)
    y = nhwc_view(y)
    if residual is not None:
      y = y + residual
    if relu:
      y = F.relu(y)
    return y


class DropoutState:

  def __init__(self, device):
    self.step = torch.zeros(1, dtype=torch.int32, device=device)
    self.bits_hook = None


class _DropoutFn(torch.autograd.Function):

  @staticmethod
  def forward(ctx, x, rate, seed0, state):
    from rigl_amd import ops
    y, bits = ops.dropout_fwd(x.contiguous(), rate, seed0, state.step)
    ctx.rate = rate
    ctx.save_for_backward(bits)
    if state.bits_hook is not None:
      state.bits_hook(seed0, bits)
    return y

  @staticmethod
  def backward(ctx, dy):
    from rigl_amd import ops
    (bits,) = ctx.saved_tensors
    return ops.dropout_bwd(dy.contiguous(), bits, ctx.rate), None, None, None


def dropout(x, rate, seed0, state, is_training=True):
  if not is_training or rate == 0:
    return x
  if not 0.0 < rate < 1.0:
    raise ValueError('dropout: rate must be in [0, 1), got %r' % (rate,))
  return _DropoutFn.apply(x, float(rate), int(seed0), state)


def eval_fused():
  from rigl_amd import ops
  return ops.tune_get('eval_fuse', 1) != 0


def infer_params(graph):
  from rigl_amd import ops
  bns = [m for m in graph.modules.values() if isinstance(m, BatchNorm)]
  return dict(zip(bns, ops.bn_infer_params(bns)))


def conv_infer(conv, x, desc=None, **epilogue):
  from rigl_amd import ops
  n, h, w, _ = x.shape
  d = desc if desc is not None else conv.desc_for(n, h, w)
  return ops.conv_fwd(d, x.contiguous(), conv.vars.ohwi, **epilogue)


def conv_bn_infer(conv, x, bn_in, **epilogue):
  from rigl_amd import ops
  n, h, w, _ = x.shape
  return ops.conv_fwd_bnrelu(conv.desc_for(n, h, w), x.contiguous(), bn_in, conv.vars.ohwi, None, **epilogue)


def dense_infer(layer, x):
  from rigl_amd import ops
  lead = x.shape[:-1]
  x2 = x.reshape(-1, 1, 1, layer.n_in).contiguous()
  b = x2.shape[0]
  d = layer._descs.get(b)
  if d is None:
    d = ops.conv_desc(b, 1, 1, layer.n_in, layer.units, 1, 1, 1, 0, 0, 1, 1)
    layer._descs[b] = d
  y = ops.conv_fwd(d, x2, layer.vars.ohwi).reshape(*lead, layer.units)
  if layer.bias is not None:
    y = y + layer.bias.data.to(y.dtype)
  if layer.activation is not None:
    y = layer.activation(y)
  return y


def bn_relu_max_pool_infer(x, scale_shift):
  from rigl_amd import ops
  if eval_fused():
    return ops.bn_relu_maxpool_infer(_pool_desc(x), x.contiguous(), scale_shift)
  return max_pool_3x3_s2_same(ops.bn_apply(x.contiguous(), scale_shift, relu=True))


class _DepthwiseFn(torch.autograd.Function):

  @staticmethod
  def forward(ctx, x, layer, desc, want_stats=False):
    from rigl_amd import ops
    x = x.contiguous()
    ctx.layer, ctx.desc = layer, desc
    ctx.save_for_backward(x)
    out = ops.depthwise_fwd(desc, x, layer.weights.data.view(-1), stats=want_stats)
    y, part = out if want_stats else (out, None)
    return stats_outputs(ctx, want_stats, (y,), (part,), x.device)

  @staticmethod
  def backward(ctx, dy, _dpart=None):
    from rigl_amd import ops
    (x,) = ctx.saved_tensors
    dy = dy.contiguous()
    w = ctx.layer.weights
    ops.depthwise_wgrad(ctx.desc, x, dy, w.grad.view(-1))
    return ops.depthwise_dgrad(ctx.desc, dy, w.data.view(-1)), None, None, None


class DepthwiseConv2d:

  def __init__(self, graph, scope, channels, kernel_size=3, stride=1):
    from rigl_amd import pruning_layers as PL
    self.k, self.stride, self.channels = kernel_size, stride, channels
    init = PL.variance_scaling_initializer()((kernel_size, kernel_size, channels, 1))
    self.weights = graph.add_variable(scope + '/depthwise_weights', (kernel_size, kernel_size, channels, 1),
                                      V.KIND_OTHER, 0.0, init)
    self._descs = {}

  def _desc(self, x):
    from rigl_amd import ops
    n, h, w, c = x.shape
    d = self._descs.get((n, h, w))
    if d is None:
      pad = (self.k - 1) // 2
      ho, wo = (h - 1) // self.stride + 1, (w - 1) // self.stride + 1
      d = ops.conv_desc(n, h, w, c, c, self.k, self.k, self.stride, pad, pad, ho, wo)
      self._descs[(n, h, w)] = d
    return d

  def infer(self, x):
    from rigl_amd import ops
    return ops.depthwise_fwd(self._desc(x), x.contiguous(), self.weights.data.view(-1))

  def __call__(self, x, bn_stats=False):
    d = self._desc(x)
    if not x.requires_grad:
      x = x.detach().requires_grad_(True)
    if not (bn_stats and _DW_STATS):
      return _DepthwiseFn.apply(x, self, d)
    y, part = _DepthwiseFn.apply(x, self, d, True)
    if part.numel():
      y.bn_partials = part
    return y


class _MaxPoolFn(torch.autograd.Function):

  @staticmethod
  def forward(ctx, x, desc):
    from rigl_amd import ops
    y, arg = ops.maxpool_fwd(desc, x.contiguous())
    ctx.desc = desc
    ctx.save_for_backward(arg)
    return y

  @staticmethod
  def backward(ctx, dy):
    from rigl_amd import ops
    (arg,) = ctx.saved_tensors
    return ops.maxpool_bwd(ctx.desc, dy.contiguous(), arg), None


class _BnReluMaxPoolFn(torch.autograd.Function):

  @staticmethod
  def forward(ctx, x, bn, desc, partials=None):
    from rigl_amd import ops
    x = x.contiguous()
    y, arg, saved = ops.bn_relu_maxpool_fwd(desc, x, bn.gamma.data, bn.beta.data, bn.moving_mean, bn.moving_variance,
                                            1.0 - bn.decay, bn.eps, partials=partials)
    ctx.bn, ctx.desc = bn, desc
    ctx.save_for_backward(x, arg, saved)
    return y

  @staticmethod
  def backward(ctx, dy):
    from rigl_amd import ops
    x, arg, saved = ctx.saved_tensors
    bn = ctx.bn
    dx = ops.bn_relu_maxpool_bwd(ctx.desc, x, dy.contiguous(), arg, bn.gamma.data, saved, bn.gamma.grad, bn.beta.grad)
    return dx, None, None, None


_STEM_TAIL_FUSED = os.environ.get('RIGL_STEM_TAIL', '1') != '0'


def _pool_desc(x):
  from rigl_amd import ops
  n, h, w, c = x.shape
  key = (n, h, w, c)
  d = _POOL_DESCS.get(key)
  if d is None:
    ho, wo = -(-h // 2), -(-w // 2)
    ph = max((ho - 1) * 2 + 3 - h, 0)
    pw = max((wo - 1) * 2 + 3 - w, 0)
    d = ops.conv_desc(n, h, w, c, c, 3, 3, 2, ph // 2, pw // 2, ho, wo)
    _POOL_DESCS[key] = d
  return d


def bn_relu_max_pool_3x3_s2_same(bn, x, is_training=True):
  c = x.shape[-1]
  if (_STEM_TAIL_FUSED and bn.fused and is_training and x.is_cuda and x.dtype == torch.bfloat16 and x.dim() == 4
      and c % 8 == 0 and c <= 256 and 64 % (c // 4) == 0 and x.numel() // 4 < (1 << 31)):
    partials = getattr(x, 'bn_partials', None)
    if not x.requires_grad:
      x = x.detach().requires_grad_(True)
    return _BnReluMaxPoolFn.apply(x, bn, _pool_desc(x), partials)
  return max_pool_3x3_s2_same(bn(x, is_training, relu=True))


_POOL_DESCS = {}


def max_pool_3x3_s2_same(x):
  if x.is_cuda and x.dtype == torch.bfloat16 and x.dim() == 4 and x.shape[-1] % 8 == 0:
    return _MaxPoolFn.apply(x, _pool_desc(x))
  xn = nchw_view(x)
  h, w = xn.shape[2], xn.shape[3]
  if h % 2 == 0 and w % 2 == 0:
    return nhwc_view(F.max_pool2d(xn, 3, 2, padding=0, ceil_mode=True))
  ph = max((-(-h // 2) - 1) * 2 + 3 - h, 0)
  pw = max((-(-w // 2) - 1) * 2 + 3 - w, 0)
  xn = F.pad(xn, (pw // 2, pw - pw // 2, ph // 2, ph - ph // 2),
             value=float('-inf'))
  return nhwc_view(F.max_pool2d(xn, 3, 2))


_HEAD_KERNELS = os.environ.get('RIGL_HEAD_TORCH', '0') != '1'


class _GlobalAvgPoolFn(torch.autograd.Function):

  @staticmethod
  def forward(ctx, x):
    from rigl_amd import ops
    ctx.hw = (x.shape[1], x.shape[2])
    return ops.global_avgpool_fwd(x.contiguous())

  @staticmethod
  def backward(ctx, dy):
    from rigl_amd import ops
    return ops.global_avgpool_bwd(dy.contiguous(), *ctx.hw)


def global_avg_pool(x):
  if _HEAD_KERNELS and x.is_cuda and x.dtype == torch.bfloat16 and x.shape[-1] % 2 == 0:
    return _GlobalAvgPoolFn.apply(x)
  return x.float().mean(dim=(1, 2)).to(x.dtype)


class _GlobalAvgPoolReluFn(torch.autograd.Function):

  @staticmethod
  def forward(ctx, x):
    from rigl_amd import ops
    ctx.save_for_backward(x)
    return ops.global_avgpool_fwd(x)

  @staticmethod
  def backward(ctx, dy):
# ... 37 lines not shown
```

Baseline: 13110.

## Fuse paired BN-add-BN backward apply into downstream 1x1 conv backward loads

Splits the paired BN+add+BN backward into a reduce-only entry that produces per-channel coefficients. The elementwise BN apply is then deferred into the fused 1x1 conv backward (bn-apply-on-load) for both the main and shortcut convolutions, which skips writing and re-reading dx/dx2. The 1x1 backward kernel also gains an ADDL variant that stages the residual addend through LDS via DMA instead of register loads. The bn_bwd_on_load default is raised to 2 to enable the pair path. This adds holder plumbing complexity and more LDS use per block.

```diff
diff --git a/include/rigl_hip.h b/include/rigl_hip.h
--- a/include/rigl_hip.h
+++ b/include/rigl_hip.h
@@ -367,6 +367,13 @@
                        rigl_bf16* dx, rigl_bf16* dx2, float* dgamma, float* dbeta,
                        float* dgamma2, float* dbeta2, void* workspace,
                        size_t workspace_bytes, rigl_stream_t stream);
+int rigl_bn_add_bn_bwd_reduce(int64_t m, int32_t c, const rigl_bf16* x, const rigl_bf16* x2,
+                              const uint8_t* relu_bits, const rigl_bf16* dy,
+                              const float* gamma, const float* save_mean, const float* save_invstd,
+                              const float* gamma2, const float* save_mean2, const float* save_invstd2,
+                              float* dgamma, float* dbeta, float* dgamma2, float* dbeta2,
+                              float* coef, float* coef2, void* workspace,
+                              size_t workspace_size, rigl_stream_t stream);
 
 int rigl_stateless_random(float* out, int64_t n, int32_t seed0, int32_t seed1,
                           int32_t dist, float scale, float shift,
diff --git a/rigl_amd/_lib.py b/rigl_amd/_lib.py
--- a/rigl_amd/_lib.py
+++ b/rigl_amd/_lib.py
@@ -184,6 +184,7 @@
     'rigl_bn_add_bn_fwd': (C.c_int, [_I64, _I32, _P, _P, _P, _P, _P, _P, _P, _P, _F, _F, _I32, _P, _P, _P, _P, _P, _P, _I32, _P, _P, _SZ, _P]),
     'rigl_bn_add_bn_bwd_workspace_bytes': (_SZ, [_I64, _I32]),
     'rigl_bn_add_bn_bwd': (C.c_int, [_I64, _I32, _P, _P, _P, _P, _P, _P, _P, _P, _P, _P, _P, _P, _P, _P, _P, _P, _P, _SZ, _P]),
+    'rigl_bn_add_bn_bwd_reduce': (C.c_int, [_I64, _I32, _P, _P, _P, _P, _P, _P, _P, _P, _P, _P, _P, _P, _P, _P, _P, _P, _P, _SZ, _P]),
     'rigl_bn_relu_maxpool_fwd': (C.c_int, [C.POINTER(ConvDesc), _P, _P, _P, _P, _P, _P]),
     'rigl_bn_relu_maxpool_bwd_workspace_bytes': (_SZ, [C.POINTER(ConvDesc)]),
     'rigl_bn_relu_maxpool_bwd': (C.c_int, [C.POINTER(ConvDesc), _P, _P, _P, _P, _P, _P, _P, _P, _P, _P, _P, _P, _SZ, _P]),
diff --git a/rigl_amd/csrc/bn.hip b/rigl_amd/csrc/bn.hip
--- a/rigl_amd/csrc/bn.hip
+++ b/rigl_amd/csrc/bn.hip
@@ -719,44 +719,72 @@
 
 size_t rigl_bn_add_bn_bwd_workspace_bytes(int64_t m, int32_t c) { return 2 * rigl_bn_workspace_bytes(m, c); }
 
-int rigl_bn_add_bn_bwd(int64_t m, int32_t c, const rigl_bf16* x, const rigl_bf16* x2, const uint8_t* relu_bits,
-                       const rigl_bf16* dy, const float* gamma, const float* save_mean, const float* save_invstd,
-                       const float* gamma2, const float* save_mean2, const float* save_invstd2, rigl_bf16* dx,
-                       rigl_bf16* dx2, float* dgamma, float* dbeta, float* dgamma2, float* dbeta2, void* workspace,
-                       size_t workspace_bytes, rigl_stream_t stream) {
+static int bn_add_bn_bwd_impl(const char* who, int64_t m, int32_t c, const rigl_bf16* x, const rigl_bf16* x2, const uint8_t* relu_bits,
+                              const rigl_bf16* dy, const float* gamma, const float* save_mean, const float* save_invstd,
+                              const float* gamma2, const float* save_mean2, const float* save_invstd2, rigl_bf16* dx,
+                              rigl_bf16* dx2, float* dgamma, float* dbeta, float* dgamma2, float* dbeta2, float* coef_out,
+                              float* coef2_out, void* workspace, size_t workspace_bytes, rigl_stream_t stream) {
   using namespace rigl;
   using namespace rigl::kbn;
+  const bool reduce_only = coef_out != nullptr;
   if (m <= 0 || c <= 0 || !x || !x2 || !relu_bits || !dy || !gamma || !save_mean || !save_invstd || !gamma2 || !save_mean2 ||
-      !save_invstd2 || !dx || !dx2 || !dgamma || !dbeta || !dgamma2 || !dbeta2)
-    return fail(RIGL_EINVAL, "rigl_bn_add_bn_bwd: bad arguments");
-  if (c % 8) return fail(RIGL_EUNSUPPORTED, "rigl_bn_add_bn_bwd: channels %% 8 != 0");
+      !save_invstd2 || !dgamma || !dbeta || !dgamma2 || !dbeta2 || (reduce_only ? !coef2_out : (!dx || !dx2)))
+    return fail(RIGL_EINVAL, "%s: bad arguments", who);
+  if (c % 8) return fail(RIGL_EUNSUPPORTED, "%s: channels %% 8 != 0", who);
   const size_t lds = (size_t)10 * c * 4;
-  if (lds > 160 * 1024 - 1024) return fail(RIGL_EUNSUPPORTED, "rigl_bn_add_bn_bwd: too many channels for the LDS parameter cache");
+  if (lds > 160 * 1024 - 1024) return fail(RIGL_EUNSUPPORTED, "%s: too many channels for the LDS parameter cache", who);
   const size_t need = rigl_bn_add_bn_bwd_workspace_bytes(m, c);
-  if (!workspace || workspace_bytes < need) return fail(RIGL_EWORKSPACE, "rigl_bn_add_bn_bwd: workspace %zu < %zu", workspace_bytes, need);
-  static const bool big_lds = hipFuncSetAttribute(reinterpret_cast<const void*>(&k_bwd_apply_pair),
-                                                  hipFuncAttributeMaxDynamicSharedMemorySize, 159 * 1024) == hipSuccess;
-  if (lds > 65536 && !big_lds) return fail(RIGL_ELAUNCH, "rigl_bn_add_bn_bwd: cannot raise the dynamic LDS limit");
+  if (!workspace || workspace_bytes < need) return fail(RIGL_EWORKSPACE, "%s: workspace %zu < %zu", who, workspace_bytes, need);
+  if (!reduce_only) {
+    static const bool big_lds = hipFuncSetAttribute(reinterpret_cast<const void*>(&k_bwd_apply_pair),
+                                                    hipFuncAttributeMaxDynamicSharedMemorySize, 159 * 1024) == hipSuccess;
+    if (lds > 65536 && !big_lds) return fail(RIGL_ELAUNCH, "%s: cannot raise the dynamic LDS limit", who);
+  }
   hipStream_t st = as_stream(stream);
   Geom g = make_geom(m, c);
   const size_t half = rigl_bn_workspace_bytes(m, c);
   const size_t part_bytes = align_up((size_t)g.parts * 2 * c * 4, 256);
   char* w0 = static_cast<char*>(workspace);
   float* partial = reinterpret_cast<float*>(w0);
-  float* coef = reinterpret_cast<float*>(w0 + part_bytes);
+  float* coef = reduce_only ? coef_out : reinterpret_cast<float*>(w0 + part_bytes);
   float* partial2 = reinterpret_cast<float*>(w0 + half);
-  float* coef2 = reinterpret_cast<float*>(w0 + half + part_bytes);
+  float* coef2 = reduce_only ? coef2_out : reinterpret_cast<float*>(w0 + half + part_bytes);
   dim3 rgrid((unsigned)g.parts, (unsigned)((g.cg + g.tpr - 1) / g.tpr));
   hipLaunchKernelGGL(k_reduce_pair, rgrid, dim3(THREADS), 0, st, g, x, x2, relu_bits, dy, save_mean, save_invstd, save_mean2,
                      save_invstd2, partial, partial2);
   const FinSet f0 = {partial, gamma, save_invstd, dgamma, dbeta, coef};
   const FinSet f1 = {partial2, gamma2, save_invstd2, dgamma2, dbeta2, coef2};
   hipLaunchKernelGGL(k_bwd_finalize_pair<16>, dim3((unsigned)((c + 15) / 16), 2), dim3(THREADS), 0, st, g, f0, f1);
+  if (reduce_only) {
+    RIGL_CHECK_LAUNCH(who);
+    return RIGL_OK;
+  }
   const dim3 pgrid(apply_grid(g));
   hipLaunchKernelGGL(k_bwd_apply_pair, pgrid, dim3(THREADS), g.fixed ? 0 : lds, st, g, x, x2, relu_bits, dy, save_mean, save_invstd,
                      save_mean2, save_invstd2, coef, coef2, dx, dx2);
-  RIGL_CHECK_LAUNCH("rigl_bn_add_bn_bwd");
+  RIGL_CHECK_LAUNCH(who);
   return RIGL_OK;
+}
+
+int rigl_bn_add_bn_bwd(int64_t m, int32_t c, const rigl_bf16* x, const rigl_bf16* x2, const uint8_t* relu_bits,
+                       const rigl_bf16* dy, const float* gamma, const float* save_mean, const float* save_invstd,
+                       const float* gamma2, const float* save_mean2, const float* save_invstd2, rigl_bf16* dx,
+                       rigl_bf16* dx2, float* dgamma, float* dbeta, float* dgamma2, float* dbeta2, void* workspace,
+                       size_t workspace_bytes, rigl_stream_t stream) {
+  return bn_add_bn_bwd_impl("rigl_bn_add_bn_bwd", m, c, x, x2, relu_bits, dy, gamma, save_mean, save_invstd, gamma2, save_mean2,
+                            save_invstd2, dx, dx2, dgamma, dbeta, dgamma2, dbeta2, nullptr, nullptr, workspace, workspace_bytes,
+                            stream);
+}
+
+int rigl_bn_add_bn_bwd_reduce(int64_t m, int32_t c, const rigl_bf16* x, const rigl_bf16* x2, const uint8_t* relu_bits,
+                              const rigl_bf16* dy, const float* gamma, const float* save_mean, const float* save_invstd,
+                              const float* gamma2, const float* save_mean2, const float* save_invstd2, float* dgamma,
+                              float* dbeta, float* dgamma2, float* dbeta2, float* coef, float* coef2, void* workspace,
+                              size_t workspace_size, rigl_stream_t stream) {
+  if (!coef || !coef2) return rigl::fail(RIGL_EINVAL, "rigl_bn_add_bn_bwd_reduce: coef and coef2 are required");
+  return bn_add_bn_bwd_impl("rigl_bn_add_bn_bwd_reduce", m, c, x, x2, relu_bits, dy, gamma, save_mean, save_invstd, gamma2,
+                            save_mean2, save_invstd2, nullptr, nullptr, dgamma, dbeta, dgamma2, dbeta2, coef, coef2, workspace,
+                            workspace_size, stream);
 }
 
 static int bn_bwd_impl(int64_t m, int32_t c, const rigl_bf16* x, const rigl_bf16* y, const uint8_t* relu_bits,
diff --git a/rigl_amd/csrc/bwd1x1.hpp b/rigl_amd/csrc/bwd1x1.hpp
--- a/rigl_amd/csrc/bwd1x1.hpp
+++ b/rigl_amd/csrc/bwd1x1.hpp
@@ -24,11 +24,12 @@
 
 typedef __attribute__((ext_vector_type(4))) float f32x4;
 
-template <int CI, int CO, bool DO_W, int NST, bool BNA = false>
+template <int CI, int CO, bool DO_W, int NST, bool BNA = false, bool ADDL = false>
 struct Bwd1x1Smem {
-  static constexpr int BYTES = NST * (32 * ((DO_W ? CI : 0) + CO) * 2 + (BNA ? 32 * CO * 2 + 32 * (CO / 8) : 0)) + (CI <= 64 ? 2 : 1) * 32 * (CI * 2 + 16);
+  static constexpr int BYTES = NST * (32 * ((DO_W ? CI : 0) + CO) * 2 + (BNA ? 32 * CO * 2 + 32 * (CO / 8) : 0)) +
+                               (CI <= 64 ? 2 : 1) * 32 * (CI * 2 + (ADDL ? 0 : 16)) + (ADDL ? 32 * CI * 2 : 0);
 };
-template <int CI, int CO, bool DO_W, int NST, bool BNA = false>
+template <int CI, int CO, bool DO_W, int NST, bool BNA = false, bool ADDL = false>
 __global__ __launch_bounds__(THREADS) void k_bwd1x1(Bwd1x1Args P) {
   constexpr int PX = 32;
   constexpr int YROWB = CO * 2, XROWB = CI * 2;
@@ -48,10 +49,14 @@
   static_assert(CFW * KSD * 4 <= 96, "W fragments stay in registers");
   constexpr bool DXDB = CI <= 64;
   constexpr int NDX = DXDB ? 2 : 1;
-  constexpr int DXROWB = XROWB + 16, DX_BYTES = PX * DXROWB;
-  static_assert(NST * STAGE + NDX * DX_BYTES == Bwd1x1Smem<CI, CO, DO_W, NST, BNA>::BYTES, "host and device agree on the LDS size");
+  constexpr int DXROWB = XROWB + (ADDL ? 0 : 16), DX_BYTES = PX * DXROWB;
+  constexpr int A_BYTES = ADDL ? PX * XROWB : 0;
+  static_assert(NST * STAGE + NDX * DX_BYTES + A_BYTES == Bwd1x1Smem<CI, CO, DO_W, NST, BNA, ADDL>::BYTES, "host and device agree on the LDS size");
+  static_assert(!ADDL || (BNA && NST >= 3 && A_BYTES == THREADS * 16), "ADDL: one 16-byte addend piece per thread, written by its own wave's DMA");
   extern __shared__ __attribute__((aligned(1024))) unsigned char smem[];
   unsigned char* const dxs = smem + NST * STAGE;
+  unsigned char* const adds = dxs + NDX * DX_BYTES;
+  (void)adds;
 
   const int tid = threadIdx.x, lane = tid & 63;
   const int wave = __builtin_amdgcn_readfirstlane(tid >> 6);
@@ -66,7 +71,8 @@
   (void)rsrcY4; (void)rsrcX4; (void)rsrcY; (void)rsrcX;
   const u32x4 rsrcZ4 = make_rsrc4(BNA ? P.Y3 : P.DY, BNA ? P.dy_bytes : 0u);
   const u32x4 rsrcB4 = make_rsrc4(BNA ? (const void*)P.BITS : (const void*)P.DY, BNA ? P.dy_bytes >> 4 : 0u);
-  (void)rsrcZ4; (void)rsrcB4;
+  const u32x4 rsrcA4 = make_rsrc4(ADDL ? (const void*)P.ADD : (const void*)P.DY, ADDL ? P.x_bytes : 0u);
+  (void)rsrcZ4; (void)rsrcB4; (void)rsrcA4;
 
   int y_row[YPW], y_col[YPW], x_row[XPW], x_col[XPW];
 #pragma unroll
@@ -146,7 +152,7 @@
 
   constexpr int DXP = PX * (CI / 8) / THREADS;
   static_assert(PX * (CI / 8) % THREADS == 0, "whole pieces per thread");
-  constexpr int W_N = L * (NST - 2), W_A = W_N + DXP * (NST - 1);
+  constexpr int W_N = L * (NST - 2), W_A = W_N + DXP * (ADDL ? NST - 2 : NST - 1), A_FROM = ADDL ? NST - 2 : NST - 1;
   uint4 addv[DXP];
 #define B1_FLUSH(ktp_, second_barrier_)                                                                    \
   {                                                                                                        \
@@ -163,7 +169,7 @@
       if (p0_ + row < P.M) {                                                                               \
         uint4 v = v_[q];                                                                                   \
         if (P.ADD) {                                                                                       \
-          const uint4 a = addv[q];                                                                         \
+          const uint4 a = ADDL ? *reinterpret_cast<const uint4*>(adds + tid * 16) : addv[q];               \
           v.x = add_bf16x2(v.x, a.x); v.y = add_bf16x2(v.y, a.y); v.z = add_bf16x2(v.z, a.z); v.w = add_bf16x2(v.w, a.w); \
         }                                                                                                  \
         *reinterpret_cast<uint4*>(P.DX + (int64_t)(p0_ + row) * CI + ch * 8) = v;                          \
@@ -174,7 +180,7 @@
     if (t < KT) B1_ISSUE(t, t);
   for (int kt = 0; kt < KT; ++kt) {
     if (kt + NST - 1 <= KT) {
-      if (P.ADD && kt >= NST - 1) wait_vmcnt<W_A>();
+      if (P.ADD && kt >= A_FROM) wait_vmcnt<W_A>();
       else wait_vmcnt<W_N>();
     } else {
       wait_vmcnt<0>();
@@ -205,15 +211,30 @@
     asm volatile("s_waitcnt lgkmcnt(0)" ::: "memory");
     __builtin_amdgcn_s_barrier();
     asm volatile("" ::: "memory");
-    if (kt + NST - 1 < KT) B1_ISSUE(kt + NST - 1, (kt + NST - 1) % NST);
-    asm volatile("" ::: "memory");
-    __builtin_amdgcn_sched_barrier(0);
-    if (kt > 0) B1_FLUSH(kt - 1, !DXDB);
+    if constexpr (ADDL) {
+      if (kt > 0) {
+        if (kt + NST - 2 < KT) wait_vmcnt<L>(); else wait_vmcnt<0>();
+        B1_FLUSH(kt - 1, !DXDB);
+      }
+      asm volatile("s_waitcnt lgkmcnt(0)" ::: "memory");
+      __builtin_amdgcn_sched_barrier(0);
+      {
+        const int p0 = (kt_begin + kt * kt_step) * PX;
+        lds_dma16_nt(rsrcA4, adds + wave * 1024,
+                     p0 + tid / (CI / 8) < P.M ? (int)((uint32_t)p0 * (uint32_t)(CI * 2) + (uint32_t)tid * 16u) : (int)OOB);
+      }
+      if (kt + NST - 1 < KT) B1_ISSUE(kt + NST - 1, (kt + NST - 1) % NST);
+    } else {
+      if (kt + NST - 1 < KT) B1_ISSUE(kt + NST - 1, (kt + NST - 1) % NST);
+      asm volatile("" ::: "memory");
+      __builtin_amdgcn_sched_barrier(0);
+      if (kt > 0) B1_FLUSH(kt - 1, !DXDB);
+    }
     asm volatile("" ::: "memory");
     __builtin_amdgcn_sched_barrier(0);
     const unsigned char* Ys = smem + (kt % NST) * STAGE;
     const unsigned char* Xs = Ys + Y_BYTES;
-    if (P.ADD) {
+    if (!ADDL && P.ADD) {
       const int p0 = (kt_begin + kt * kt_step) * PX;
 #pragma unroll
       for (int q = 0; q < DXP; ++q) {
@@ -269,6 +290,7 @@
     }
   }
   if (KT > 0) {
+    if (ADDL) wait_vmcnt<0>();
     __syncthreads();
     B1_FLUSH(KT - 1, false);
   }
@@ -343,10 +365,18 @@
 }
 
 static bool bwd1x1_bna_ready(const RiglConvDesc* d) {
-  if (!RIGL_TUNE("bn_bwd_on_load", 1) || bwd1x1_kind(d) != 1 || !bwd1x1_ready(d)) return false;
+  if (!RIGL_TUNE("bn_bwd_on_load", 2) || bwd1x1_kind(d) != 1 || !bwd1x1_ready(d)) return false;
   constexpr int SMEM = Bwd1x1Smem<64, 256, true, 4, true>::BYTES;
   static_assert(SMEM <= 160 * 1024, "the ring fits a CU's LDS");
   static const bool ready = hipFuncSetAttribute(reinterpret_cast<const void*>(&k_bwd1x1<64, 256, true, 4, true>),
+                                                hipFuncAttributeMaxDynamicSharedMemorySize, SMEM) == hipSuccess;
+  return ready;
+}
+static bool bwd1x1_bna_addl_ready() {
+  if (!RIGL_TUNE("bwd1x1_add_lds", 1)) return false;
+  constexpr int SMEM = Bwd1x1Smem<64, 256, true, 4, true, true>::BYTES;
+  static_assert(SMEM <= 160 * 1024, "the ring fits a CU's LDS");
+  static const bool ready = hipFuncSetAttribute(reinterpret_cast<const void*>(&k_bwd1x1<64, 256, true, 4, true, true>),
                                                 hipFuncAttributeMaxDynamicSharedMemorySize, SMEM) == hipSuccess;
   return ready;
 }
@@ -359,7 +389,11 @@
   a.M = d->n * d->h * d->w; a.splits = bwd1x1_splits(); a.interleave = RIGL_TUNE("bwd1x1_il", 1);
   a.x_bytes = (uint32_t)((size_t)a.M * d->cin * 2); a.dy_bytes = (uint32_t)((size_t)a.M * d->cout * 2);
   a.Y3 = y3; a.BITS = bits; a.MEAN = mean; a.INVSTD = invstd; a.COEF = coef;
-  RIGL_K_LAUNCH((k_bwd1x1<64, 256, true, 4, true>), dim3((unsigned)a.splits), dim3(THREADS),
-                (Bwd1x1Smem<64, 256, true, 4, true>::BYTES), st, a);
+  if (addend && bwd1x1_bna_addl_ready())
+    RIGL_K_LAUNCH((k_bwd1x1<64, 256, true, 4, true, true>), dim3((unsigned)a.splits), dim3(THREADS),
+                  (Bwd1x1Smem<64, 256, true, 4, true, true>::BYTES), st, a);
+  else
+    RIGL_K_LAUNCH((k_bwd1x1<64, 256, true, 4, true>), dim3((unsigned)a.splits), dim3(THREADS),
+                  (Bwd1x1Smem<64, 256, true, 4, true>::BYTES), st, a);
   return true;
 }
diff --git a/rigl_amd/ops.py b/rigl_amd/ops.py
--- a/rigl_amd/ops.py
+++ b/rigl_amd/ops.py
@@ -544,6 +544,10 @@
   if not (mfma_supported(d) and mfma_dgrad_supported(d)):
     return False
   return bool(_plan_cached(d, 'bwd_bn_apply', lambda: int(_lib.load().rigl_conv2d_bwd_takes_bn_apply(C.byref(d)))))
+
+
+def bn_bwd_on_load():
+  return tune_get('bn_bwd_on_load', 2)
 
 
 def _conv_bwd(d, x, dy, w_hwio, dw, dx, on_dw_ready, launch, need_dx=True, dx_shape=None, dgrad_desc=None, f32=False):
@@ -1006,6 +1010,25 @@
   return dx, dx2
 
 
+def bn_add_bn_bwd_reduce(x, x2, relu_bits, dy, gamma, saved, gamma2, saved2, dgamma, dbeta, dgamma2, dbeta2):
+  _req(x, torch.bfloat16, 'x')
+  _req(x2, torch.bfloat16, 'x2')
+  _req(dy, torch.bfloat16, 'dy')
+  _req(relu_bits, torch.uint8, 'relu_bits')
+  c = x.shape[-1]
+  m = x.numel() // c
+  if x2.shape != x.shape or dy.numel() != x.numel() or relu_bits.numel() * 8 != x.numel():
+    raise ValueError('x2 and dy must have the shape of x and relu_bits one bit per element of it')
+  lib = _lib.load()
+  ws = workspace(lib.rigl_bn_add_bn_bwd_workspace_bytes(m, c), x.device)
+  coef = torch.empty((3, c), dtype=torch.float32, device=x.device)
+  coef2 = torch.empty((3, c), dtype=torch.float32, device=x.device)
+  check(lib.rigl_bn_add_bn_bwd_reduce(m, c, _ptr(x), _ptr(x2), _ptr(relu_bits), _ptr(dy), _ptr(gamma), _ptr(saved[0]),
+                                      _ptr(saved[1]), _ptr(gamma2), _ptr(saved2[0]), _ptr(saved2[1]), _ptr(dgamma), _ptr(dbeta),
+                                      _ptr(dgamma2), _ptr(dbeta2), _ptr(coef), _ptr(coef2), _ptr(ws), ws.numel(), _stream()))
+  return coef, coef2
+
+
 def bn_relu_maxpool_fwd(d, x, gamma, beta, running_mean, running_var, momentum, eps, partials=None):
   saved = bn_statistics(x, gamma, beta, running_mean, running_var, momentum, eps, partials=partials)
   lib = _lib.load()
diff --git a/rigl_amd/pruning_layers.py b/rigl_amd/pruning_layers.py
--- a/rigl_amd/pruning_layers.py
+++ b/rigl_amd/pruning_layers.py
@@ -164,9 +164,9 @@
 class _MaskedConvForkFn(torch.autograd.Function):
 
   @staticmethod
-  def forward(ctx, x, lv, desc, want_stats=False, bn_holder=None, addend_holder=None):
+  def forward(ctx, x, lv, desc, want_stats=False, bn_holder=None, addend_holder=None, apply_holder=None):
     ctx.lv, ctx.desc = lv, desc
-    ctx.bn_holder, ctx.addend_holder = bn_holder, addend_holder
+    ctx.bn_holder, ctx.addend_holder, ctx.apply_holder = bn_holder, addend_holder, apply_holder
     ctx.save_for_backward(x)
     y, part = _conv_forward(lv, desc, x, want_stats)
     return stats_outputs(ctx, want_stats, (y, x.view_as(x)), (part,), x.device)
@@ -181,16 +181,22 @@
     if x.dtype == torch.float32:
       dx = ops.conv_bwd_f32(d, x, dy, lv.weights.data.view(-1), _mask_bits(lv), lv.weights.grad.view(-1),
                             need_dx=True, addend=dalias, on_dw_ready=ready)
-      return (dx,) + (None,) * 5
+      return (dx,) + (None,) * 6
     got = ctx.addend_holder.take(dalias) if ctx.addend_holder is not None else None
+    applied = ctx.apply_holder.take(dy) if ctx.apply_holder is not None else None
+    if applied is not None:
+      if got is not None:
+        raise RuntimeError('bn_bwd_on_load: the fused backward takes its addend already masked')
+      dx = ops.conv_bwd_bnapply(d, x, dy, lv.hwio, lv.weights.grad.view(-1), *applied, addend=dalias, on_dw_ready=ready)
+      return (dx,) + (None,) * 6
     if got is not None:
       dx = ops.conv_bwd(d, x, dy, lv.hwio, lv.weights.grad.view(-1), need_dx=True, addend=dalias, addend_bits=got[0],
                         on_dw_ready=ready)
-      return (dx,) + (None,) * 5
+      return (dx,) + (None,) * 6
     req = _bn_fuse_request(ctx.bn_holder, True)
     dx = ops.conv_bwd(d, x, dy, lv.hwio, lv.weights.grad.view(-1), need_dx=True, addend=dalias, on_dw_ready=ready, bn_fuse=req)
     _bn_fuse_publish(ctx.bn_holder, req, dx)
-    return (dx,) + (None,) * 5
+    return (dx,) + (None,) * 6
 
 
 class _MaskedConvPairFn(torch.autograd.Function):
@@ -358,9 +364,13 @@
     n, h, w, _ = x.shape
     holder = _bn_source(x)
     addend_holder = MaskedAddendHolder() if self.takes_masked_addend(x) else None
-    y, alias, *part = _MaskedConvForkFn.apply(x.contiguous(), self.vars, self.desc_for(n, h, w), bn_stats, holder, addend_holder)
+    d = self.desc_for(n, h, w)
+    apply_holder = BnApplyHolder() if (x.dtype == torch.bfloat16 and x.is_cuda and ops.conv_bwd_takes_bn_apply(d)) else None
+    y, alias, *part = _MaskedConvForkFn.apply(x.contiguous(), self.vars, d, bn_stats, holder, addend_holder, apply_holder)
     if part and part[0].numel():
       y.bn_partials = part[0]
+    if apply_holder is not None and y.grad_fn is not None:
+      y.bn_apply = apply_holder
     if addend_holder is not None:
       alias.masked_addend = addend_holder
     return y, alias
diff --git a/rigl_amd/workloads/nn.py b/rigl_amd/workloads/nn.py
--- a/rigl_amd/workloads/nn.py
+++ b/rigl_amd/workloads/nn.py
@@ -113,9 +113,15 @@
 class _BnAddBnFn(torch.autograd.Function):
 
   @staticmethod
-  def forward(ctx, x, x2, bn, bn2, partials, partials2):
-    from rigl_amd import ops
+  def forward(ctx, x, x2, bn, bn2, partials, partials2, apply_holder=None, apply_holder2=None):
+    from rigl_amd import ops
+    x_in, x2_in = x, x2
     x, x2 = x.contiguous(), x2.contiguous()
+    ctx.apply_holders = None
+    if (apply_holder is not None and apply_holder2 is not None and ops.bn_bwd_on_load() >= 2 and x is x_in and x2 is x2_in
+        and ctx.needs_input_grad[0] and ctx.needs_input_grad[1]):
+      ctx.apply_holders = (apply_holder, apply_holder2)
+      apply_holder.armed = apply_holder2.armed = True
     saved2 = ops.bn_statistics(x2, bn2.gamma.data, bn2.beta.data, bn2.moving_mean, bn2.moving_variance,
                                1.0 - bn2.decay, bn2.eps, partials=partials2)
     y, saved, bits = ops.bn_add_bn_fwd(x, x2, saved2, bn.gamma.data, bn.beta.data, bn.moving_mean, bn.moving_variance,
@@ -129,9 +135,16 @@
     from rigl_amd import ops
     x, x2, saved, saved2, bits = ctx.saved_tensors
     bn, bn2 = ctx.bn, ctx.bn2
-    dx, dx2 = ops.bn_add_bn_bwd(x, x2, bits, dy.contiguous(), bn.gamma.data, saved, bn2.gamma.data, saved2,
+    dy = dy.contiguous()
+    if ctx.apply_holders is not None:
+      coef, coef2 = ops.bn_add_bn_bwd_reduce(x, x2, bits, dy, bn.gamma.data, saved, bn2.gamma.data, saved2,
+                                             bn.gamma.grad, bn.beta.grad, bn2.gamma.grad, bn2.beta.grad)
+      ctx.apply_holders[0].fill(dy, x, bits, saved, coef)
+      ctx.apply_holders[1].fill(dy, x2, bits, saved2, coef2)
+      return dy, dy, None, None, None, None, None, None
+    dx, dx2 = ops.bn_add_bn_bwd(x, x2, bits, dy, bn.gamma.data, saved, bn2.gamma.data, saved2,
                                 bn.gamma.grad, bn.beta.grad, bn2.gamma.grad, bn2.beta.grad)
-    return dx, dx2, None, None, None, None
+    return dx, dx2, None, None, None, None, None, None
 
 
 _BN_PAIR_FUSED = os.environ.get('RIGL_BN_PAIR', '1') != '0'
@@ -146,7 +159,7 @@
       x = x.detach().requires_grad_(True)
     if not x2.requires_grad:
       x2 = x2.detach().requires_grad_(True)
-    return _BnAddBnFn.apply(x, x2, bn, bn2, px, px2)
+    return _BnAddBnFn.apply(x, x2, bn, bn2, px, px2, getattr(x, 'bn_apply', None), getattr(x2, 'bn_apply', None))
   return bn(x, is_training, relu=True, residual=bn2(x2, is_training, relu=False))
 
 
```

New measurement: 13200 (median of 6 runs). About the same (+0.7%).
